# david-jk/BigGAN-Tensorflow

Measured on AMD Instinct MI355X. Metric: BigGAN-128 train-step images/sec, higher is better.
Workload: dtype bf16; 1 GPU; BigGAN-128 ch=96 bf16 (BASELINE config 3: global batch 256, 32/GPU over 8 GPUs); img_size=128, ch=96, per_gpu_batch=256, global_batch=256, da_policy=full, g_regularization=ortho_cosine, n_labels=0, gan_type=hinge, hip_graph=False, precision=bf16, parallelism=dp1

## Files before the change

### biggan-tensorflow_amd/csrc/elementwise.hip

```cpp
#include <stdlib.h>
#include <mutex>
#include "common.h"

namespace bg {

#define EW_BLOCK 256
#define EW_MAX_BLOCKS 2048

static inline int ew_grid(int64_t work_items) {
    int64_t b = (work_items + EW_BLOCK - 1) / EW_BLOCK;
    if (b > EW_MAX_BLOCKS) b = EW_MAX_BLOCKS;
    if (b < 1) b = 1;
    return (int)b;
}

__device__ __forceinline__ float4 ldg4(const float* p) { return *reinterpret_cast<const float4*>(p); }
__device__ __forceinline__ void stg4(float* p, const float4& v) { *reinterpret_cast<float4*>(p) = v; }

template <int NQ, int VEC, class Fn, class OutT>
__global__ __launch_bounds__(EW_BLOCK) void colreduce_kernel(Fn fn, OutT* out, float* part, int64_t qstride,
                                                             int64_t rows_per_seg, int C, int rows_per_block) {
    __shared__ float red[NQ * EW_BLOCK * VEC];
    const int CV = C / VEC;
    const int tx = CV < EW_BLOCK ? CV : EW_BLOCK;
    const int lanes = EW_BLOCK / tx;
    const int cq = threadIdx.x % tx, rl = threadIdx.x / tx;
    const int seg = blockIdx.y;
    const int64_t r0 = (int64_t)blockIdx.x * rows_per_block;
    int64_t r1 = r0 + rows_per_block;
    if (r1 > rows_per_seg) r1 = rows_per_seg;
    for (int cbase = 0; cbase < CV; cbase += tx) {
        const int cv = cbase + cq;
        float acc[NQ][VEC];
#pragma unroll
        for (int q = 0; q < NQ; ++q)
#pragma unroll
            for (int j = 0; j < VEC; ++j) acc[q][j] = 0.f;
        if (cv < CV && rl < lanes) {
            float acc4[4][NQ][VEC];
#pragma unroll
            for (int u = 0; u < 4; ++u)
#pragma unroll
                for (int q = 0; q < NQ; ++q)
#pragma unroll
                    for (int j = 0; j < VEC; ++j) acc4[u][q][j] = 0.f;
            int64_t r = r0 + rl;
            for (; r + 3 * (int64_t)lanes < r1; r += 4 * (int64_t)lanes) {
#pragma unroll
                for (int u = 0; u < 4; ++u) fn(seg, r + u * (int64_t)lanes, cv * VEC, acc4[u]);
            }
            for (; r < r1; r += lanes) fn(seg, r, cv * VEC, acc4[0]);
#pragma unroll
            for (int q = 0; q < NQ; ++q)
#pragma unroll
                for (int j = 0; j < VEC; ++j)
// ... 325 lines not shown
                                                                  const float* __restrict__ r, const float* __restrict__ cr,
                                                                  const float* __restrict__ c0, float* __restrict__ out,
                                                                  int64_t total, int C) {
    for (int64_t i = (int64_t)blockIdx.x * EW_BLOCK + threadIdx.x; i < total; i += (int64_t)gridDim.x * EW_BLOCK) {
        const int c = (int)(i % C);
        float v = cp[c] * p[i] + cq[c] * q[i] + c0[c];
        if (r) v += cr[c] * r[i];
        out[i] = v;
    }
}

__global__ __launch_bounds__(256) void renorm_coeffs_kernel(const double* __restrict__ sums, double count,
                                                            float* ref_mean, float* ref_scale, int scale_is_var,
                                                            float* weight, float eps, float rmin, float rmax, float dmax,
                                                            float decay, float fade, int update, float* __restrict__ r,
                                                            float* __restrict__ d, int C) {
    const float w = weight ? *weight : 1.f;
    __syncthreads();
    for (int c = threadIdx.x; c < C; c += blockDim.x) {
        const double m64 = sums[c] / count;
        double v64 = sums[C + c] / count - m64 * m64;
        if (v64 < 0) v64 = 0;
        const float m = (float)m64, var = (float)v64;
        const float sigma = sqrtf(var + eps);
        const float rm = ref_mean[c], rs = ref_scale[c];
        const float sigma_ref = scale_is_var ? sqrtf(rs + eps) : fmaxf(rs, sqrtf(eps));
        const float sigma_w = w * sigma_ref + (1.f - w) * sigma;
        const float mean_w = w * rm + (1.f - w) * m;
        r[c] = fminf(fmaxf(sigma / sigma_w, rmin), rmax);
        d[c] = fminf(fmaxf((m - mean_w) / sigma_w, -dmax), dmax);
        if (update) {
            ref_mean[c] = rm * decay + m * (1.f - decay);
            ref_scale[c] = rs * decay + (scale_is_var ? var : sigma) * (1.f - decay);
        }
    }
    if (update && weight && threadIdx.x == 0) *weight = w * fade + 1.0f * (1.f - fade);
}

__global__ __launch_bounds__(EW_BLOCK) void renorm_affine_kernel(const float* __restrict__ g, const float* __restrict__ b,
                                                                 const float* __restrict__ r, const float* __restrict__ d,
                                                                 float* __restrict__ oa, float* __restrict__ ob,
                                                                 int64_t total, int C, int dir) {
    for (int64_t i = (int64_t)blockIdx.x * blockDim.x + threadIdx.x; i < total; i += (int64_t)gridDim.x * blockDim.x) {
        const int c = (int)(i % C);
        if (dir == 0) {
            oa[i] = r[c] * g[i];
            ob[i] = b[i] + d[c] * g[i];
        } else {
            oa[i] = r[c] * g[i] + d[c] * b[i];
        }
    }
}

__device__ __forceinline__ float prelu_f(float v, float a) { return v > 0.f ? v : a * v; }
__device__ __forceinline__ float prelu_d(float v, float a) { return v > 0.f ? 1.f : (v < 0.f ? a : 0.5f * a); }

template <int VEC, class TX, class TY>
__global__ __launch_bounds__(EW_BLOCK) void bn_apply_act_fwd_t_kernel(const TX* __restrict__ x,
                                                                       const float* __restrict__ mean,
                                                                       const float* __restrict__ rstd,
                                                                       const float* __restrict__ gamma,
                                                                       const float* __restrict__ beta, int per_sample,
                                                                       const float* __restrict__ alpha,
                                                                       TY* __restrict__ y, int N, int HW, int C) {
    const int CV = C / VEC;
    const int64_t total = (int64_t)N * HW * CV;
    for (int64_t i = (int64_t)blockIdx.x * EW_BLOCK + threadIdx.x; i < total; i += (int64_t)gridDim.x * EW_BLOCK) {
        const int c = (int)(i % CV) * VEC;
        const int n = (int)(i / ((int64_t)HW * CV));
        const float* gp = gamma + (per_sample ? (int64_t)n * C : 0) + c;
        const float* bp = beta + (per_sample ? (int64_t)n * C : 0) + c;
        float xv[VEC], mu[VEC], rs[VEC], ga[VEC], be[VEC], al[VEC], out[VEC];
        loadv<VEC>(x + i * VEC, xv);
        loadv<VEC>(mean + c, mu);
        loadv<VEC>(rstd + c, rs);
        loadv<VEC>(gp, ga);
        loadv<VEC>(bp, be);
        if (alpha) loadv<VEC>(alpha + c, al);
#pragma unroll
        for (int j = 0; j < VEC; ++j) {
            const float inv = rs[j] * ga[j];
            float v = xv[j] * inv + (be[j] - mu[j] * inv);
            out[j] = alpha ? prelu_f(v, al[j]) : v;
        }
        storev<VEC>(y + i * VEC, out);
    }
}

template <class TX, class TY>
struct BnBwdReduceFnT {
    const TX* x;
    const TY* dy;
    const float *mean, *rstd, *gamma, *beta, *alpha;
    int per_sample, HW, C;
    template <int VEC>
    __device__ __forceinline__ void operator()(int n, int64_t r, int c, float (&acc)[3][VEC]) const {
        const int64_t off = ((int64_t)n * HW + r) * C + c;
        float xv[VEC], dv[VEC], mu[VEC], rs[VEC], ga[VEC], be[VEC], al[VEC];
        loadv<VEC>(x + off, xv);
        loadv<VEC>(dy + off, dv);
        loadv<VEC>(mean + c, mu);
        loadv<VEC>(rstd + c, rs);
        loadv<VEC>(gamma + (per_sample ? (int64_t)n * C : 0) + c, ga);
        loadv<VEC>(beta + (per_sample ? (int64_t)n * C : 0) + c, be);
        if (alpha) loadv<VEC>(alpha + c, al);
#pragma unroll
        for (int j = 0; j < VEC; ++j) {
// ... 179 lines not shown
        bf16x8_load(x + (int64_t)r * C + c, xv);
        bf16x8_load(dy + (int64_t)r * C + c, dv);
#pragma unroll
        for (int j = 0; j < 8; ++j) {
            const float xh = (xv[j] - mu[j]) * rs[j];
            const float pre = xh * ga[j] + be[j];
            const float g = alpha ? dv[j] * prelu_d(pre, al[j]) : dv[j];
            out[j] = rs[j] * (g * ga[j] - m1[j] - xh * m2[j]);
        }
        if (add) {
            float av[8];
            bf16x8_load(add + (int64_t)r * C + c, av);
#pragma unroll
            for (int j = 0; j < 8; ++j) out[j] += av[j];
        }
        bf16x8_store(dx + (int64_t)r * C + c, out);
    }
}

template <bool BWD>
__global__ __launch_bounds__(EW_BLOCK) void prelu_bf16x8_kernel(const __bf16* __restrict__ x, const __bf16* __restrict__ dy,
                                                                 const float* __restrict__ alpha, __bf16* out,
                                                                 const __bf16* add, int rows, int CV) {
    const int gtid = blockIdx.x * EW_BLOCK + threadIdx.x;
    const int c = (gtid % CV) * 8, C = CV * 8;
    const int rstep = (gridDim.x * EW_BLOCK) / CV;
    float al[8];
    f32x8_load(alpha + c, al);
    for (int r = gtid / CV; r < rows; r += rstep) {
        float xv[8], dv[8], o[8];
        bf16x8_load(x + (int64_t)r * C + c, xv);
        if (BWD) bf16x8_load(dy + (int64_t)r * C + c, dv);
#pragma unroll
        for (int j = 0; j < 8; ++j) o[j] = BWD ? dv[j] * prelu_d(xv[j], al[j]) : prelu_f(xv[j], al[j]);
        if (BWD && add) {
            float av[8];
            bf16x8_load(add + (int64_t)r * C + c, av);
#pragma unroll
            for (int j = 0; j < 8; ++j) o[j] += av[j];
        }
        bf16x8_store(out + (int64_t)r * C + c, o);
    }
}

__global__ __launch_bounds__(EW_BLOCK) void lincomb_bf16x8_kernel(const __bf16* __restrict__ a, const float* sa_dev, float sa,
                                                                   const __bf16* __restrict__ b, float sb,
                                                                   __bf16* __restrict__ y, int64_t n8) {
    const float s = sa_dev ? *sa_dev : sa;
    for (int64_t i = (int64_t)blockIdx.x * EW_BLOCK + threadIdx.x; i < n8; i += (int64_t)gridDim.x * EW_BLOCK) {
        float av[8], bv[8], o[8];
        bf16x8_load(a + i * 8, av);
        if (b) {
            bf16x8_load(b + i * 8, bv);
#pragma unroll
            for (int j = 0; j < 8; ++j) o[j] = s * av[j] + sb * bv[j];
        } else {
#pragma unroll
            for (int j = 0; j < 8; ++j) o[j] = s * av[j];
        }
        bf16x8_store(y + i * 8, o);
    }
}

static inline int bn_x8_grid(int64_t rows, int CV) {
    int a = CV, b = EW_BLOCK;
    while (b) { const int t = a % b; a = b; b = t; }
    const int unit = CV / a;
    int64_t want = (rows * CV + EW_BLOCK - 1) / EW_BLOCK;
    if (want > 4096) want = 4096;
    if (want < 1) want = 1;
    return (int)((want + unit - 1) / unit * unit);
}

template <int VEC, class TX, class TY>
__global__ __launch_bounds__(EW_BLOCK) void prelu_fwd_t_kernel(const TX* __restrict__ x, const float* __restrict__ alpha,
                                                                TY* __restrict__ y, int64_t total_v, int C) {
    const int CV = C / VEC;
    for (int64_t i = (int64_t)blockIdx.x * EW_BLOCK + threadIdx.x; i < total_v; i += (int64_t)gridDim.x * EW_BLOCK) {
        const int c = (int)(i % CV) * VEC;
        float xv[VEC], al[VEC], out[VEC];
        loadv<VEC>(x + i * VEC, xv);
        loadv<VEC>(alpha + c, al);
#pragma unroll
        for (int j = 0; j < VEC; ++j) out[j] = prelu_f(xv[j], al[j]);
        storev<VEC>(y + i * VEC, out);
    }
}

template <int VEC, class TX, class TY>
__global__ __launch_bounds__(EW_BLOCK) void prelu_bwd_dx_t_kernel(const TX* __restrict__ x, const TY* __restrict__ dy,
                                                                   const float* __restrict__ alpha, TX* dx, const TX* add,
                                                                   int64_t total_v, int C) {
    const int CV = C / VEC;
    for (int64_t i = (int64_t)blockIdx.x * EW_BLOCK + threadIdx.x; i < total_v; i += (int64_t)gridDim.x * EW_BLOCK) {
        const int c = (int)(i % CV) * VEC;
        float xv[VEC], dv[VEC], al[VEC], out[VEC];
        loadv<VEC>(x + i * VEC, xv);
        loadv<VEC>(dy + i * VEC, dv);
        loadv<VEC>(alpha + c, al);
#pragma unroll
        for (int j = 0; j < VEC; ++j) out[j] = dv[j] * prelu_d(xv[j], al[j]);
        if (add) {
            float av[VEC];
            loadv<VEC>(add + i * VEC, av);
#pragma unroll
            for (int j = 0; j < VEC; ++j) out[j] += av[j];
        }
        storev<VEC>(dx + i * VEC, out);
    }
}

// ... 387 lines not shown
}

__global__ __launch_bounds__(EW_BLOCK) void scale_add_kernel(const float* __restrict__ o,
                                                              const float* __restrict__ gamma,
                                                              const float* __restrict__ x, float* __restrict__ y,
                                                              int64_t n) {
    const float g = *gamma;
    const int64_t n4 = n / 4;
    for (int64_t i = (int64_t)blockIdx.x * EW_BLOCK + threadIdx.x; i < n4; i += (int64_t)gridDim.x * EW_BLOCK) {
        float4 ov = ldg4(o + i * 4), xv = ldg4(x + i * 4);
        stg4(y + i * 4, make_float4(g * ov.x + xv.x, g * ov.y + xv.y, g * ov.z + xv.z, g * ov.w + xv.w));
    }
    for (int64_t i = n4 * 4 + (int64_t)blockIdx.x * EW_BLOCK + threadIdx.x; i < n; i += (int64_t)gridDim.x * EW_BLOCK)
        y[i] = g * o[i] + x[i];
}

__global__ __launch_bounds__(EW_BLOCK) void scale_dev_kernel(const float* __restrict__ x, const float* __restrict__ sp,
                                                              float* __restrict__ y, int64_t n) {
    const float s = *sp;
    for (int64_t i = (int64_t)blockIdx.x * EW_BLOCK + threadIdx.x; i < n; i += (int64_t)gridDim.x * EW_BLOCK)
        y[i] = s * x[i];
}

template <class T>
__global__ __launch_bounds__(EW_BLOCK) void lincomb_t_kernel(const T* __restrict__ a, const float* sa_dev, float sa,
                                                              const T* __restrict__ b, float sb, T* __restrict__ y,
                                                              int64_t n4) {
    const float s = sa_dev ? *sa_dev : sa;
    for (int64_t i = (int64_t)blockIdx.x * EW_BLOCK + threadIdx.x; i < n4; i += (int64_t)gridDim.x * EW_BLOCK) {
        float av[4], bv[4], o[4];
        loadv<4>(a + i * 4, av);
        if (b) {
            loadv<4>(b + i * 4, bv);
#pragma unroll
            for (int j = 0; j < 4; ++j) o[j] = s * av[j] + sb * bv[j];
        } else {
#pragma unroll
            for (int j = 0; j < 4; ++j) o[j] = s * av[j];
        }
        storev<4>(y + i * 4, o);
    }
}

template <class T>
__global__ __launch_bounds__(EW_BLOCK) void dot_t_kernel(float* part, const T* __restrict__ a, const T* __restrict__ b, float* out,
                                                          int64_t n) {
    __shared__ float sh[4];
    float s = 0.f;
    const int64_t n4 = n / 4;
    for (int64_t i = (int64_t)blockIdx.x * EW_BLOCK + threadIdx.x; i < n4; i += (int64_t)gridDim.x * EW_BLOCK) {
        float av[4], bv[4];
        loadv<4>(a + i * 4, av);
        loadv<4>(b + i * 4, bv);
        s += av[0] * bv[0] + av[1] * bv[1] + av[2] * bv[2] + av[3] * bv[3];
    }
    for (int64_t i = n4 * 4 + (int64_t)blockIdx.x * EW_BLOCK + threadIdx.x; i < n; i += (int64_t)gridDim.x * EW_BLOCK)
        s += (float)a[i] * (float)b[i];
    s = block_sum_256(s, sh);
    if (threadIdx.x == 0) {
        if (part)
            part[blockIdx.x] = s;
        else
            *out += s;
    }
}

template <class T>
static int launch_dot(const T* a, const T* b, float* out, int64_t n, hipStream_t s) {
    int grid = ew_grid(n / 4 + 1);
    if (grid > 512) grid = 512;
    float* part = nullptr;
    if (!block_partials(grid, 1, s, &part)) return BG_ERR_LAUNCH;
    hipLaunchKernelGGL((dot_t_kernel<T>), dim3(grid), dim3(EW_BLOCK), 0, s, part, a, b, out, n);
    finalize_block_partials(part, out, grid, 1, s);
    BG_LAUNCH_CHECK();
    return BG_OK;
}

__global__ __launch_bounds__(EW_BLOCK) void tanh_fwd_kernel(const float* __restrict__ x, float* __restrict__ y,
                                                             int64_t n) {
    for (int64_t i = (int64_t)blockIdx.x * EW_BLOCK + threadIdx.x; i < n; i += (int64_t)gridDim.x * EW_BLOCK)
        y[i] = tanhf(x[i]);
}

__global__ __launch_bounds__(EW_BLOCK) void tanh_bwd_kernel(const float* __restrict__ y, const float* __restrict__ dy,
                                                             float* __restrict__ dx, int64_t n) {
    for (int64_t i = (int64_t)blockIdx.x * EW_BLOCK + threadIdx.x; i < n; i += (int64_t)gridDim.x * EW_BLOCK)
        dx[i] = dy[i] * (1.f - y[i] * y[i]);
}

template <class TS, class TD>
__global__ __launch_bounds__(EW_BLOCK) void pad_channels_kernel(const TS* __restrict__ src, TD* __restrict__ dst,
                                                                 int64_t total, int Cs, int Cd, int64_t inner, int mode) {
    for (int64_t idx = (int64_t)blockIdx.x * EW_BLOCK + threadIdx.x; idx < total; idx += (int64_t)gridDim.x * EW_BLOCK) {
        const int64_t i = idx % inner, t = idx / inner;
        const int c = (int)(t % Cd);
        const int64_t o = t / Cd;
        const TS* sp = src + o * Cs * inner + i;
        float v = 0.f;
        if (mode == 3) {
            v = (float)sp[(int64_t)c * inner] + (float)sp[(int64_t)(c + Cd) * inner];
        } else if (c < Cs) {
            v = (float)sp[(int64_t)c * inner];
            if (mode == 1) v = (float)(__bf16)v;
        } else if (mode != 0 && c < 2 * Cs) {
            v = (float)sp[(int64_t)(c - Cs) * inner];
            if (mode == 1) v -= (float)(__bf16)v;
        }
        dst[idx] = (TD)v;
    }
}

__global__ __launch_bounds__(EW_BLOCK) void pad_pixels_to8_kernel(const float* __restrict__ src, __bf16* __restrict__ dst,
                                                                  int64_t pixels, int Cs, int mode) {
    for (int64_t i = (int64_t)blockIdx.x * EW_BLOCK + threadIdx.x; i < pixels; i += (int64_t)gridDim.x * EW_BLOCK) {
        float v[8];
#pragma unroll
        for (int c = 0; c < 8; ++c) v[c] = 0.f;
        const float* sp = src + i * Cs;
#pragma unroll
        for (int c = 0; c < 4; ++c)
            if (c < Cs) {
                const float s = sp[c];
                if (mode == 1) {
                    const float hi = (float)(__bf16)s;
                    v[c] = hi;
// ... 1203 lines not shown
        BG_DISPATCH_T(dtype, hipLaunchKernelGGL((maxpool2_bwd_t_kernel<1, T>), dim3(ew_grid(total)), dim3(EW_BLOCK), 0,
                                                as_stream(stream), (const T*)x, (const T*)dy, (T*)dx, N, H, W, C));
    BG_LAUNCH_CHECK();
    return BG_OK;
}

int bg_sum_pool_fwd_t(const void* x, int x_dtype, float* y, int N, int HW, int C, void* stream) {
    BG_REQUIRE(x && y && N > 0 && HW > 0 && C > 0 && BG_DT_OK(x_dtype), "bg_sum_pool_fwd_t: bad argument");
    if (C % 4 == 0)
        BG_DISPATCH_T(x_dtype, hipLaunchKernelGGL((sum_pool_fwd_t_kernel<4, T>), dim3(ew_grid((int64_t)N * C / 4)),
                                                  dim3(EW_BLOCK), 0, as_stream(stream), (const T*)x, y, N, HW, C));
    else
        BG_DISPATCH_T(x_dtype, hipLaunchKernelGGL((sum_pool_fwd_t_kernel<1, T>), dim3(ew_grid((int64_t)N * C)),
                                                  dim3(EW_BLOCK), 0, as_stream(stream), (const T*)x, y, N, HW, C));
    BG_LAUNCH_CHECK();
    return BG_OK;
}

int bg_sum_pool_bwd_t(const float* dy, void* dx, int x_dtype, int N, int HW, int C, void* stream) {
    BG_REQUIRE(dy && dx && N > 0 && HW > 0 && C > 0 && BG_DT_OK(x_dtype), "bg_sum_pool_bwd_t: bad argument");
    if (C % 4 == 0)
        BG_DISPATCH_T(x_dtype, hipLaunchKernelGGL((sum_pool_bwd_t_kernel<4, T>), dim3(ew_grid((int64_t)N * HW * C / 4)),
                                                  dim3(EW_BLOCK), 0, as_stream(stream), dy, (T*)dx, N, HW, C));
    else
        BG_DISPATCH_T(x_dtype, hipLaunchKernelGGL((sum_pool_bwd_t_kernel<1, T>), dim3(ew_grid((int64_t)N * HW * C)),
                                                  dim3(EW_BLOCK), 0, as_stream(stream), dy, (T*)dx, N, HW, C));
    BG_LAUNCH_CHECK();
    return BG_OK;
}

int bg_lincomb_t(const void* a, const float* sa_dev, float sa, const void* b, float sb, void* y, int dtype, int64_t n,
                 void* stream) {
    BG_REQUIRE(a && y && n > 0 && n % 4 == 0 && BG_DT_OK(dtype), "bg_lincomb_t: bad argument (n %% 4 == 0)");
    if (dtype == BG_BF16 && n % 8 == 0 && ((uintptr_t)a & 15) == 0 && ((uintptr_t)y & 15) == 0 &&
        (!b || ((uintptr_t)b & 15) == 0)) {
        hipLaunchKernelGGL(lincomb_bf16x8_kernel, dim3(ew_grid(n / 8)), dim3(EW_BLOCK), 0, as_stream(stream),
                           (const __bf16*)a, sa_dev, sa, (const __bf16*)b, sb, (__bf16*)y, n / 8);
        BG_LAUNCH_CHECK();
        return BG_OK;
    }
    BG_DISPATCH_T(dtype, hipLaunchKernelGGL((lincomb_t_kernel<T>), dim3(ew_grid(n / 4)), dim3(EW_BLOCK), 0, as_stream(stream),
                                            (const T*)a, sa_dev, sa, (const T*)b, sb, (T*)y, n / 4));
    BG_LAUNCH_CHECK();
    return BG_OK;
}

int bg_dot_t(const void* a, const void* b, int dtype, float* out_accum, int64_t n, void* stream) {
    BG_REQUIRE(a && b && out_accum && n > 0 && n % 4 == 0 && BG_DT_OK(dtype), "bg_dot_t: bad argument (n %% 4 == 0)");
    int rc = BG_OK;
    BG_DISPATCH_T(dtype, rc = launch_dot((const T*)a, (const T*)b, out_accum, n, as_stream(stream)));
    return rc;
}

int bg_bn_stats(const float* x, double* sums, int64_t rows, int C, void* stream) {
    return bg_bn_stats_t(x, BG_F32, sums, rows, C, stream);
}

int bg_bn_apply_act_fwd(const float* x, const float* mean, const float* rstd, const float* gamma, const float* beta,
                        int per_sample, const float* alpha, float* y, int N, int HW, int C, void* stream) {
    return bg_bn_apply_act_fwd_t(x, BG_F32, mean, rstd, gamma, beta, per_sample, alpha, y, BG_F32, N, HW, C, stream);
}

int bg_bn_apply_act_bwd_reduce(const float* x, const float* dy, const float* mean, const float* rstd,
                               const float* gamma, const float* beta, int per_sample, const float* alpha, float* part,
                               int N, int HW, int C, void* stream) {
    return bg_bn_apply_act_bwd_reduce_t(x, BG_F32, dy, BG_F32, mean, rstd, gamma, beta, per_sample, alpha, part, N, HW, C,
                                        stream);
}

int bg_bn_apply_act_bwd_dx(const float* x, const float* dy, const float* mean, const float* rstd, const float* gamma,
                           const float* beta, int per_sample, const float* alpha, const float* cm, float* dx, int N,
                           int HW, int C, void* stream) {
    return bg_bn_apply_act_bwd_dx_t(x, BG_F32, dy, BG_F32, mean, rstd, gamma, beta, per_sample, alpha, cm, dx, NULL, N, HW,
                                    C, stream);
}

int bg_prelu_fwd(const float* x, const float* alpha, float* y, int64_t rows, int C, void* stream) {
    return bg_prelu_fwd_t(x, BG_F32, alpha, y, BG_F32, rows, C, stream);
}

int bg_prelu_bwd(const float* x, const float* dy, const float* alpha, float* dx, float* dalpha, int64_t rows, int C,
                 void* stream) {
    return bg_prelu_bwd_t(x, BG_F32, dy, BG_F32, alpha, dx, dalpha, NULL, rows, C, stream);
}

int bg_bias_grad(const float* dy, float* db, int64_t rows, int C, void* stream) {
    return bg_bias_grad_t(dy, BG_F32, db, rows, C, stream);
}

int bg_maxpool2_fwd(const float* x, float* y, int N, int H, int W, int C, void* stream) {
    return bg_maxpool2_fwd_t(x, y, BG_F32, N, H, W, C, stream);
}

int bg_maxpool2_bwd(const float* x, const float* dy, float* dx, int N, int H, int W, int C, void* stream) {
    return bg_maxpool2_bwd_t(x, dy, dx, BG_F32, N, H, W, C, stream);
}

int bg_sum_pool_fwd(const float* x, float* y, int N, int HW, int C, void* stream) {
    return bg_sum_pool_fwd_t(x, BG_F32, y, N, HW, C, stream);
}

int bg_sum_pool_bwd(const float* dy, float* dx, int N, int HW, int C, void* stream) {
    return bg_sum_pool_bwd_t(dy, dx, BG_F32, N, HW, C, stream);
}

int bg_dot(const float* a, const float* b, float* out_accum, int64_t n, void* stream) {
// ... 7 lines not shown
```

### biggan-tensorflow_amd/csrc/igemm.hip

```cpp
#include <stdlib.h>
#include "common.h"
#include "igemm.h"
#include "igemm_dev.h"
#include "igemm_bf16.h"
#include "igemm16.h"


namespace bg {

typedef float floatx16 __attribute__((ext_vector_type(16)));

#define BKT 16

template <int TM, int TN, int LDA, int LDB>
__device__ __forceinline__ void mma_tile(const float* __restrict__ as, const float* __restrict__ bs, int a_rd, int b_rd,
                                         floatx16 (&acc)[TM][TN]) {
    float a[2][TM], b[2][TN];
#pragma unroll
    for (int i = 0; i < TM; ++i) a[0][i] = as[a_rd + 32 * i];
#pragma unroll
    for (int j = 0; j < TN; ++j) b[0][j] = bs[b_rd + 32 * j];
#pragma unroll
    for (int kk = 0; kk < BKT / 2; ++kk) {
        const int cur = kk & 1, nxt = cur ^ 1;
        if (kk + 1 < BKT / 2) {
#pragma unroll
            for (int i = 0; i < TM; ++i) a[nxt][i] = as[a_rd + 2 * (kk + 1) * LDA + 32 * i];
#pragma unroll
            for (int j = 0; j < TN; ++j) b[nxt][j] = bs[b_rd + 2 * (kk + 1) * LDB + 32 * j];
        }
#pragma unroll
        for (int i = 0; i < TM; ++i)
#pragma unroll
            for (int j = 0; j < TN; ++j)
                acc[i][j] = __builtin_amdgcn_mfma_f32_32x32x2f32(a[cur][i], b[cur][j], acc[i][j], 0, 0, 0);
    }
}

template <int TM, int TN, int WM, int WN, bool BT, int MODE, bool MIRROR, bool VEC>
__global__ __launch_bounds__(256, (TM * TN == 4 && !MIRROR) ? 4 : 1) void nn_kernel(const NNParams p) {
    constexpr int BM = 32 * TM * WM, BN = 32 * TN * WN;
    constexpr int LDA = BM + 2;
    constexpr int LDB = BT ? BN + 2 : BN + 4;
    constexpr int AROWS = BM / 64;
    constexpr int NSRC = MIRROR ? 4 : 1;
    static_assert(WM * WN == 4, "4 waves");
    __shared__ __attribute__((aligned(16))) float As[2][BKT * LDA];
    __shared__ __attribute__((aligned(16))) float Bs[2][BKT * LDB];

    const int t = threadIdx.x;
    const int lane = t & 63, wave = t >> 6;
    const int wm = wave / WN, wn = wave % WN;

// ... 1028 lines not shown
    const int batch = d->batch > 0 ? d->batch : 1;
    Gather g{};
    g.Nb = d->transA ? d->K : d->M; g.Hs = 1; g.Ws = 1; g.Ho = 1; g.Wo = 1; g.Hq = 1; g.Wq = 1; g.pstep = 1;
    g.k = 1; g.stride = 1; g.ld = d->lda;
    if (d->transA) {
        pl.route = TN_F32;
        TNParams& p = pl.tn;
        p.g = g;
        p.Ca = d->M; p.Cb = d->N; p.Mf = d->M; p.b_ld = d->ldb; p.M = d->K;
        p.out_ld = d->ldc; p.batch = batch;
        p.strideA = d->strideA; p.strideB = d->strideB; p.strideC = d->strideC;
        return pl;
    }
    pl.route = F32_TAP;
    NNParams& p = pl.nn;
    p.g = g;
    p.C = d->K; p.M = d->M; p.N = d->N;
    if (d->transB) { p.ldk = 1; p.ldn = d->ldb; } else { p.ldk = d->ldb; p.ldn = 1; }
    p.out_ld = d->ldc; p.batch = batch;
    p.strideA = d->strideA; p.strideB = d->strideB; p.strideC = d->strideC;
    pl.bt = d->transB != 0;
    pl.dense = d->ldc == d->N && batch == 1;
    pl.zdim = batch;
    pl.niter_min = kc_of(d->K);
    pl.out_elems = (int64_t)d->M * d->N;
    return pl;
}

static ConvPlan plan_gram16(int rows, int cols, int ld) {
    ConvPlan pl{};
    pl.route = TN_BF16;
    pl.mode = GATHER_PLAIN;
    TN16Params& p = pl.tn16;
    p.g.ld = ld; p.b_ld = ld;
    p.Ca = cols; p.Cb = cols; p.Mf = cols; p.M = rows; p.out_ld = cols;
    return pl;
}

static size_t plan_workspace_bytes(const ConvPlan& pl) {
    if (pl.route == TN_F32) return tn_workspace_bytes(pl.tn.Mf, pl.tn.Cb, pl.tn.batch, pl.tn.M);
    if (pl.route == TN_BF16) return tn16_workspace_bytes(pl.tn16);
    const size_t slabs = route_f32(pl.route) ? nn_workspace_bytes(pl)
                                             : nn16_workspace_bytes(pl.nn16, pl.mode, pl.zdim, pl.out_elems);
    return pl.grid_bytes ? align256(slabs) + pl.grid_bytes : slabs;
}

static size_t plan_stats_bytes(const BgConvDesc* d, const ConvPlan& pl) {
    if (pl.route != BF16_PLAIN || d->y_dtype != BG_BF16) return 0;
    return (size_t)nn16_stats_rows(pl.nn16, pl.mode, pl.zdim) * 2 * (size_t)d->Cout * sizeof(float);
}

static int run_nn(ConvPlan& pl, const BgConvDesc* d, const char* op, bool deconv, const void* src, const void* w,
                  const float* bias, const float* alpha_dev, void* out, int accumulate, void* ws, size_t ws_bytes,
                  void* stream) {
    hipStream_t s = as_stream(stream);
    Tag tag(op, d);
    void* const grid = ws;
    void* target = out;
    int acc = accumulate;
    if (pl.grid_bytes) {
        BG_REQUIRE(ws && ws_bytes >= pl.grid_bytes, "bg_conv2d_dgrad: workspace too small for the padded gradient");
        target = ws; acc = 0;
        ws = ws_bytes > pl.grid_bytes ? reinterpret_cast<char*>(ws) + pl.grid_bytes : nullptr;
        ws_bytes -= pl.grid_bytes;
    }
    ProfScope prof(s, conv_flops(d, deconv), tag.s, tag.bytes);
    int rc;
    if (route_f32(pl.route)) {
        NNParams& p = pl.nn;
        p.A = (const float*)src; p.B = (const float*)w; p.bias = bias; p.alpha = alpha_dev; p.out = (float*)target;
        p.accumulate = acc;
        const bool vec = (p.C % 4 == 0) && (pl.bt || p.N % 4 == 0) && aligned16(src) && aligned16(w);
        rc = launch_nn(pl, vec, ws, ws_bytes, s, d->compute == BG_COMPUTE_BF16);
    } else {
        NN16Params& r = pl.nn16;
        r.A = src; r.B = w; r.bias = bias; r.alpha = alpha_dev; r.out = target; r.accumulate = acc;
        NN16Params q = r;
        if (pl.route == BF16_THIN_D2S || pl.route == BF16_THIN_D2S_RING)
            rc = launch_nn16h_d2s(r, s);
        else
            rc = launch_nn16(r, pl.mode, pl.zdim, pl.out_elems, ws, ws_bytes, s);
        if (!rc && route_ring(pl.route)) {
            q.ring = 1;
            q.ring_lines = d->stride == 1 ? 2 : 1;
            q.accumulate = 1;
            rc = launch_nn16_ring(q, s);
        }
    }
    if (rc || !pl.grid_bytes) return rc;
    return launch_reflect_fold(grid, out, route_f32(pl.route) ? 1 : pl.nn16.out_f32, d->N, d->H, d->W, d->Cin, pl.nn.g.Ho,
                               pl.nn.g.Wo, d->pad_lo, accumulate, s);
}

static int run_tn(ConvPlan& pl, const BgConvDesc* d, const char* op, bool deconv, const void* a, const void* b, float* dw,
                  void* ws, size_t ws_bytes, void* stream) {
    Tag tag(op, d);
    ProfScope prof(as_stream(stream), conv_flops(d, deconv), tag.s, tag.bytes);
    if (pl.route == TN_BF16) {
        pl.tn16.A = a; pl.tn16.Bv = b;
        return launch_tn16(pl.tn16, pl.mode, dw, ws, ws_bytes, as_stream(stream));
    }
    pl.tn.A = (const float*)a; pl.tn.Bv = (const float*)b;
    const bool vec = (d->Cin % 4 == 0) && (d->Cout % 4 == 0) && aligned16(a) && aligned16(b);
    return launch_tn(pl.tn, pl.mode, vec, dw, ws, ws_bytes, as_stream(stream), d->compute == BG_COMPUTE_BF16);
}

}

using namespace bg;

extern "C" {

size_t bg_conv2d_fwd_workspace_bytes(const BgConvDesc* d) { return d ? plan_workspace_bytes(plan_conv_fwd(d)) : 0; }
size_t bg_conv2d_dgrad_workspace_bytes(const BgConvDesc* d) { return d ? plan_workspace_bytes(plan_conv_dgrad(d)) : 0; }
size_t bg_conv2d_wgrad_workspace_bytes(const BgConvDesc* d) { return d ? plan_workspace_bytes(plan_conv_wgrad(d)) : 0; }
size_t bg_deconv2d_fwd_workspace_bytes(const BgConvDesc* d) { return d ? plan_workspace_bytes(plan_deconv_fwd(d)) : 0; }
size_t bg_deconv2d_dgrad_workspace_bytes(const BgConvDesc* d) { return d ? plan_workspace_bytes(plan_deconv_dgrad(d)) : 0; }
size_t bg_deconv2d_wgrad_workspace_bytes(const BgConvDesc* d) { return d ? plan_workspace_bytes(plan_deconv_wgrad(d)) : 0; }
size_t bg_deconv2d_fwd_stats_workspace_bytes(const BgConvDesc* d) { return d ? plan_stats_bytes(d, plan_deconv_fwd(d)) : 0; }
size_t bg_gemm_workspace_bytes(const BgGemmDesc* d) { return d ? plan_workspace_bytes(plan_gemm(d)) : 0; }
size_t bg_gram16_workspace_bytes(int rows, int cols) {
    return rows > 0 && cols > 0 ? plan_workspace_bytes(plan_gram16(rows, cols, cols)) : 0;
}

int bg_conv2d_fwd(const BgConvDesc* d, const void* x, const void* w, const float* bias, const float* alpha_dev,
                  void* y, int accumulate, void* ws, size_t ws_bytes, void* stream) {
    int rc = check_conv(d);
    if (rc) return rc;
    BG_REQUIRE(x && w && y, "bg_conv2d_fwd: null tensor pointer");
    ConvPlan pl = plan_conv_fwd(d);
    if (pl.route == BF16_PLAIN)
        BG_REQUIRE(d->w_packed, "bg_conv2d_fwd: bf16 input needs the packed bf16 weights (w_packed)");
    else
        BG_REQUIRE(d->y_dtype == BG_F32 && !d->w_packed, "bg_conv2d_fwd: fp32 input needs fp32 weights and output");
    return run_nn(pl, d, "conv2d_fwd", false, x, w, bias, alpha_dev, y, accumulate, ws, ws_bytes, stream);
}

int bg_conv2d_fwd_d2s_supported(const BgConvDesc* d, int block) {
    if (!d) return 0;
    const ConvPlan pl = plan_conv_fwd(d, block);
    if (!pl.nn16.d2s_c || check_conv(d) != BG_OK) return 0;
    return nn16_d2s_ok(pl.nn16, pl.mode, pl.zdim) ? 1 : 0;
}

int bg_conv2d_fwd_d2s(const BgConvDesc* d, const void* x, const void* w, const float* bias, const float* alpha_dev,
                      void* y, int block, void* ws, size_t ws_bytes, void* stream) {
    int rc = check_conv(d);
    if (rc) return rc;
    BG_REQUIRE(x && w && y, "bg_conv2d_fwd_d2s: null tensor pointer");
    ConvPlan pl = plan_conv_fwd(d, block);
    BG_REQUIRE(pl.nn16.d2s_c && nn16_d2s_ok(pl.nn16, pl.mode, pl.zdim),
               "bg_conv2d_fwd_d2s: this launch has no fused depth-to-space store (query bg_conv2d_fwd_d2s_supported)");
    (void)ws; (void)ws_bytes;
    return run_nn(pl, d, "conv2d_fwd_d2s", false, x, w, bias, alpha_dev, y, 0, nullptr, 0, stream);
}

int bg_conv2d_dgrad(const BgConvDesc* d, const void* dy, const void* w, const float* alpha_dev, void* dx,
                    int accumulate, void* ws, size_t ws_bytes, void* stream) {
    int rc = check_conv(d);
    if (rc) return rc;
    BG_REQUIRE(dy && w && dx, "bg_conv2d_dgrad: null tensor pointer");
    BG_REQUIRE(d->H % d->stride == 0 && d->W % d->stride == 0, "conv dgrad: H,W must be multiples of stride");
    ConvPlan pl = plan_conv_dgrad(d);
    if (route_f32(pl.route))
        BG_REQUIRE(d->x_dtype == BG_F32 && d->y_dtype == BG_F32 && !d->w_packed, "bg_conv2d_dgrad: unsupported dtype mix");
    return run_nn(pl, d, "conv2d_dgrad", false, dy, w, nullptr, alpha_dev, dx, accumulate, ws, ws_bytes, stream);
}

int bg_conv2d_wgrad(const BgConvDesc* d, const void* x, const void* dy, float* dw, void* ws, size_t ws_bytes,
                    void* stream) {
    int rc = check_conv(d);
    if (rc) return rc;
    BG_REQUIRE(x && dy && dw, "bg_conv2d_wgrad: null tensor pointer");
    ConvPlan pl = plan_conv_wgrad(d);
    if (pl.route == TN_F32)
        BG_REQUIRE(d->x_dtype == BG_F32 && d->y_dtype == BG_F32, "bg_conv2d_wgrad: x and dy must both be fp32 or both bf16");
    return run_tn(pl, d, "conv2d_wgrad", false, x, dy, dw, ws, ws_bytes, stream);
}

int bg_deconv2d_fwd(const BgConvDesc* d, const void* x, const void* w, const float* bias, const float* alpha_dev,
                    void* y, int accumulate, void* ws, size_t ws_bytes, void* stream) {
    int rc = check_deconv(d);
    if (rc) return rc;
    BG_REQUIRE(x && w && y, "bg_deconv2d_fwd: null tensor pointer");
    ConvPlan pl = plan_deconv_fwd(d);
    if (pl.route == BF16_PLAIN)
        BG_REQUIRE(d->w_packed, "bg_deconv2d_fwd: bf16 input needs the packed bf16 weights (w_packed)");
    else
        BG_REQUIRE(d->y_dtype == BG_F32 && !d->w_packed, "bg_deconv2d_fwd: fp32 input needs fp32 weights and output");
    return run_nn(pl, d, "deconv2d_fwd", true, x, w, bias, alpha_dev, y, accumulate, ws, ws_bytes, stream);
// ... 80 lines not shown
```

### biggan-tensorflow_amd/csrc/igemm16.h

```cpp
#pragma once
#include <stdint.h>

#include "igemm.h"

namespace bg {

struct NN16Params {
    const void* A;
    const void* B;
    const float* bias;
    const float* alpha;
    void* out;
    float* slabs;
    float* stats_part;
    Gather g;
    int32_t C;
    int32_t M, N;
    int64_t tap_stride;
    int32_t out_ld;
    int32_t out_f32;
    int32_t accumulate;
    int32_t splitk;
    int64_t slab_stride;
    int32_t tiles_m, tiles_n;
    int32_t zfold;
    int32_t mfast;
    int32_t pow2;
    int32_t wq_shift, hq_shift;
    int32_t posmajor;
    int32_t ring;
    int32_t ring_lines;
    int32_t d2s_c;
};

struct TN16Params {
    const void* A;
    const void* Bv;
    float* out;
    Gather g;
    int32_t Ca, Cb;
    int32_t Mf;
    int32_t b_ld;
    int32_t M;
    int32_t splitk, rows_per_split;
    int64_t slab_stride;
    int32_t out_ld;
    int32_t tiles_m, tiles_n;
    int32_t pow2;
    int32_t wq_shift, hq_shift;
};

size_t nn16_workspace_bytes(const NN16Params& p, int mode, int zdim, int64_t out_elems);
int launch_nn16(NN16Params& p, int mode, int zdim, int64_t out_elems, void* ws, size_t ws_bytes, hipStream_t s);
int64_t nn16_stats_rows(const NN16Params& p, int mode, int zdim);
int launch_nn16_ring(NN16Params& p, hipStream_t s);
bool nn16_d2s_ok(const NN16Params& p, int mode, int zdim);
bool nn16h_d2s_ok(const NN16Params& p);
int launch_nn16h_d2s(const NN16Params& plain, hipStream_t s);
size_t tn16_workspace_bytes(const TN16Params& p);
int launch_tn16(TN16Params& p, int mode, float* final_out, void* ws, size_t ws_bytes, hipStream_t s);
int launch_reflect_fold(const void* dxp, void* dx, int f32, int N, int H, int W, int C, int Hp, int Wp, int pad_lo,
                        int accumulate, hipStream_t s);

}
```

### biggan-tensorflow_amd/csrc/igemm16.hip

```cpp
#include <stdlib.h>

#include "common.h"
#include "igemm.h"
#include "igemm16.h"
#include <type_traits>
#include "igemm_dev.h"

namespace bg {

typedef float f32x4_t __attribute__((ext_vector_type(4)));
typedef float f32x16_t __attribute__((ext_vector_type(16)));
typedef __bf16 bf16x8_t __attribute__((ext_vector_type(8)));
typedef short s16x4v __attribute__((ext_vector_type(4)));
typedef short s16x8v __attribute__((ext_vector_type(8)));
typedef __attribute__((address_space(3))) void lds_void_t;
typedef __attribute__((address_space(1))) const void gbl_void_t;
typedef __attribute__((address_space(3))) s16x4v lds_s16x4v;

__device__ uint4 g_zero_page[1024];

__device__ __forceinline__ void glds16(const void* src, unsigned char* lds_wave_base) {
    __builtin_amdgcn_global_load_lds((gbl_void_t*)src, (lds_void_t*)lds_wave_base, 16, 0, 0);
}

__device__ __forceinline__ void glds16_asm(const void* src, uint32_t lds_byte_addr) {
    unsigned keep;
    const uint32_t dst = __builtin_amdgcn_readfirstlane(lds_byte_addr);
    asm volatile("s_mov_b32 %0, m0\n\ts_mov_b32 m0, %2\n\ts_nop 0\n\tglobal_load_lds_dwordx4 %1, off\n\ts_mov_b32 m0, %0"
                 : "=&s"(keep)
                 : "v"(src), "s"(dst)
                 : "memory");
}

__device__ __forceinline__ uint32_t pack_bf16x2(float a, float b) {
    typedef __bf16 bf16x2_t __attribute__((ext_vector_type(2)));
    bf16x2_t v;
    v[0] = (__bf16)a;
    v[1] = (__bf16)b;
    return __builtin_bit_cast(uint32_t, v);
}
__device__ __forceinline__ float bf16_lo(uint32_t u) { return __builtin_bit_cast(float, u << 16); }
__device__ __forceinline__ float bf16_hi(uint32_t u) { return __builtin_bit_cast(float, u & 0xffff0000u); }

constexpr int NN16_BM = 128;
constexpr int NN16_TAPS = 4;
constexpr int NN16_RING_TAPS = 8;
constexpr int nn16_lds_bytes(int TN, int TAPS = NN16_TAPS) {
    const int stage = (NN16_BM + 32 * TN) * 128;
    const int epi = NN16_BM * (32 * TN + 4) * 4;
    const int tab = 2 * TAPS * NN16_BM * 4;
    return (2 * stage + tab > epi ? 2 * stage + tab : epi) + NN16_BM * 4 + 16;
}
constexpr int nn16_pipe_lds_bytes(int TN, int WM, int TAPS = NN16_TAPS) {
    const int bm = 64 * WM;
    return 3 * (bm + 32 * TN) * 64 + TAPS * bm * (4 + 2) + bm * 4 + 16;
}
constexpr int nn16x_lds_bytes(int TN) {
    return 2 * (256 + 32 * TN) * 128 + 2 * NN16_TAPS * 256 * 4 + 256 * 4 + 16;
}
constexpr int NN16_NOSRC = -(1 << 30);

template <int MODE>
__device__ __forceinline__ int64_t nn16_src_off(const Gather& g, const RowPos& r, int kh, int kw) {
    int h, w;
    if (MODE == GATHER_CONV) {
        h = conv_src(r.ho, kh, g.stride, g.pad, g.reflect, g.Hs);
        w = conv_src(r.wo, kw, g.stride, g.pad, g.reflect, g.Ws);
    } else {
        h = tconv_src_from_num(r.ho + g.pad - kh, g.stride, g.Hs);
        w = tconv_src_from_num(r.wo + g.pad - kw, g.stride, g.Ws);
    }
    const bool ok = r.valid && h >= 0 && w >= 0;
    const int pix = (r.b * g.Hs + h) * g.Ws + w;
    return ok ? (int64_t)pix * g.ld : (int64_t)-1;
}

constexpr int NN16_NOMIRROR = -(1 << 20);
__device__ __forceinline__ int nn16_mirror_pos(int o, int n, bool hi) {
    return o == 1 ? -1 : ((hi && o == n - 2) ? n : NN16_NOMIRROR);
}

template <int MODE, bool PM, bool RING = false>
__device__ __forceinline__ RowPos nn16_row(const NN16Params& p, int m, int ph, int pw) {
    RowPos r;
    if (PM) {
        r.valid = m < p.M;
        const int pos = m / p.g.Nb;
        r.b = m - pos * p.g.Nb;
        if (RING) {
            const int L = p.ring_lines, first = L * p.g.Wo;
            if (pos < first) {
                const int line = pos / p.g.Wo;
                r.ho = line == 0 ? 1 : p.g.Ho - 2;
                r.wo = pos - line * p.g.Wo;
            } else {
// ... 463 lines not shown
#pragma unroll
                for (int j = 0; j < TN; ++j)
                    acc[i][j] = __builtin_amdgcn_mfma_f32_16x16x32_bf16(b[s2][j], a[s2][i], acc[i][j], 0, 0, 0);
        asm volatile("s_waitcnt vmcnt(0) lgkmcnt(0)" ::: "memory");
        __builtin_amdgcn_s_barrier();
    }
    }

    constexpr int PARTS = PIPE ? WM : (PHASED ? 2 : 1), PR = BM / PARTS;
    constexpr int ELD = BN + 4;
    float* est = reinterpret_cast<float*>(smem);
    const bool partial = p.splitk > 1;
    const float alpha = (!partial && p.alpha) ? *p.alpha : 1.0f;
    constexpr int CPR = BN / 8;
    float* slab = partial ? p.slabs + (int64_t)zs * p.slab_stride : nullptr;
#pragma unroll
    for (int part = 0; part < PARTS; ++part) {
    if (part > 0) __syncthreads();
    if constexpr (PHASED) {
        constexpr int WNX = TN == 8 ? 4 : 2;
        const int wmx = w / WNX, wnx = w % WNX;
#pragma unroll
        for (int i = 0; i < XMI; ++i)
#pragma unroll
            for (int hj = 0; hj < 2 * XNJ; ++hj) {
                const int row = wmx * 16 * XMI + 16 * i + (lane & 15);
                const int col = (BN / 2) * (hj / XNJ) + wnx * 16 * XNJ + 16 * (hj % XNJ) + 4 * (lane >> 4);
                f32x4_t v = accx[part][i][hj / XNJ][hj % XNJ];
                v[0] *= alpha; v[1] *= alpha; v[2] *= alpha; v[3] *= alpha;
                *reinterpret_cast<f32x4_t*>(est + row * ELD + col) = v;
            }
    } else if (!PIPE || wm == part) {
#pragma unroll
        for (int i = 0; i < 4; ++i)
#pragma unroll
            for (int j = 0; j < TN; ++j) {
                const int row = (PIPE ? 0 : wm * 64) + 16 * i + (lane & 15);
                const int col = wn * 16 * TN + 16 * j + 4 * (lane >> 4);
                f32x4_t v = acc[i][j];
                v[0] *= alpha; v[1] *= alpha; v[2] *= alpha; v[3] *= alpha;
                *reinterpret_cast<f32x4_t*>(est + row * ELD + col) = v;
            }
    }
    __syncthreads();
#pragma unroll
    for (int q = 0; q < (PR * CPR + NTHR - 1) / NTHR; ++q) {
        const int idx = t + NTHR * q;
        if ((PR * CPR) % NTHR != 0 && idx >= PR * CPR) continue;
        const int erow = idx / CPR, cc = idx - erow * CPR;
        const int row = part * PR + erow;
        const int m = m0 + row, col = n0 + cc * 8;
        if (m >= p.M || col >= p.N) continue;
        int64_t ooff;
        if (use_tabo) {
            const unsigned op = tabo[row];
            if (op == 0xffffffffu) continue;
            ooff = (int64_t)op * p.out_ld + col;
        } else if (p.d2s_c) {
            int b, ho, wo;
            if (p.pow2) {
                wo = m & (g.Wo - 1);
                const int t2 = m >> p.wq_shift;
                ho = t2 & (g.Ho - 1);
                b = t2 >> p.hq_shift;
            } else {
                const int t2 = m / g.Wo;
                wo = m - t2 * g.Wo;
                b = t2 / g.Ho;
                ho = t2 - b * g.Ho;
            }
            const int sub = col / p.d2s_c, c = col - sub * p.d2s_c;
            ooff = (((int64_t)b * (2 * g.Ho) + 2 * ho + (sub >> 1)) * (2 * g.Wo) + 2 * wo + (sub & 1)) * p.d2s_c + c;
        } else {
            ooff = (int64_t)m * p.out_ld + col;
        }
        f32x4_t v0 = *reinterpret_cast<const f32x4_t*>(est + erow * ELD + cc * 8);
        f32x4_t v1 = *reinterpret_cast<const f32x4_t*>(est + erow * ELD + cc * 8 + 4);
        if (partial) {
            *reinterpret_cast<f32x4_t*>(slab + ooff) = v0;
            *reinterpret_cast<f32x4_t*>(slab + ooff + 4) = v1;
            continue;
        }
        if (p.bias) {
            const f32x4_t b0 = *reinterpret_cast<const f32x4_t*>(p.bias + col);
            const f32x4_t b1 = *reinterpret_cast<const f32x4_t*>(p.bias + col + 4);
            v0 += b0;
            v1 += b1;
        }
        if (p.out_f32) {
            float* o = reinterpret_cast<float*>(p.out) + ooff;
            if (p.accumulate) {
                v0 += *reinterpret_cast<const f32x4_t*>(o);
                v1 += *reinterpret_cast<const f32x4_t*>(o + 4);
            }
            *reinterpret_cast<f32x4_t*>(o) = v0;
            *reinterpret_cast<f32x4_t*>(o + 4) = v1;
        } else {
            __bf16* o = reinterpret_cast<__bf16*>(p.out) + ooff;
            if (p.accumulate) {
                const uint4 r = *reinterpret_cast<const uint4*>(o);
                v0[0] += bf16_lo(r.x); v0[1] += bf16_hi(r.x); v0[2] += bf16_lo(r.y); v0[3] += bf16_hi(r.y);
                v1[0] += bf16_lo(r.z); v1[1] += bf16_hi(r.z); v1[2] += bf16_lo(r.w); v1[3] += bf16_hi(r.w);
            }
            uint4 r;
            r.x = pack_bf16x2(v0[0], v0[1]);
            r.y = pack_bf16x2(v0[2], v0[3]);
            r.z = pack_bf16x2(v1[0], v1[1]);
            r.w = pack_bf16x2(v1[2], v1[3]);
            *reinterpret_cast<uint4*>(o) = r;
        }
    }
    }
}

__global__ __launch_bounds__(256) void nn16_slab_reduce_kernel(const float* __restrict__ slabs, void* __restrict__ out,
                                                               const float* __restrict__ bias,
                                                               const float* __restrict__ alpha_dev, int64_t n8, int N,
                                                               int splitk, int64_t slab_stride, int accumulate,
                                                               int out_f32) {
    const float alpha = alpha_dev ? *alpha_dev : 1.0f;
    for (int64_t i = (int64_t)blockIdx.x * 256 + threadIdx.x; i < n8; i += (int64_t)gridDim.x * 256) {
        f32x4_t s0 = {0.f, 0.f, 0.f, 0.f}, s1 = s0;
        for (int z = 0; z < splitk; ++z) {
            const float* sp = slabs + (int64_t)z * slab_stride + i * 8;
            s0 += *reinterpret_cast<const f32x4_t*>(sp);
            s1 += *reinterpret_cast<const f32x4_t*>(sp + 4);
        }
        s0 *= alpha;
        s1 *= alpha;
        if (bias) {
            const int col = (int)((i * 8) % N);
            s0 += *reinterpret_cast<const f32x4_t*>(bias + col);
            s1 += *reinterpret_cast<const f32x4_t*>(bias + col + 4);
        }
        if (out_f32) {
            float* o = reinterpret_cast<float*>(out) + i * 8;
            if (accumulate) {
                s0 += *reinterpret_cast<const f32x4_t*>(o);
                s1 += *reinterpret_cast<const f32x4_t*>(o + 4);
            }
            *reinterpret_cast<f32x4_t*>(o) = s0;
            *reinterpret_cast<f32x4_t*>(o + 4) = s1;
        } else {
            __bf16* o = reinterpret_cast<__bf16*>(out) + i * 8;
            if (accumulate) {
                const uint4 r = *reinterpret_cast<const uint4*>(o);
                s0[0] += bf16_lo(r.x); s0[1] += bf16_hi(r.x); s0[2] += bf16_lo(r.y); s0[3] += bf16_hi(r.y);
                s1[0] += bf16_lo(r.z); s1[1] += bf16_hi(r.z); s1[2] += bf16_lo(r.w); s1[3] += bf16_hi(r.w);
            }
            uint4 r;
            r.x = pack_bf16x2(s0[0], s0[1]);
            r.y = pack_bf16x2(s0[2], s0[3]);
            r.z = pack_bf16x2(s1[0], s1[1]);
            r.w = pack_bf16x2(s1[2], s1[3]);
            *reinterpret_cast<uint4*>(o) = r;
        }
    }
}

constexpr int NH_T = 16;
constexpr int NH_LDS_MAX = 81920;
template <int NT> struct NHGeom {
// ... 33 lines not shown
    for (int half = 0; half < 2; ++half) {
        if ((wm >> 1) == half) {
#pragma unroll
            for (int i = 0; i < 4; ++i)
#pragma unroll
                for (int j = 0; j < NF; ++j) {
                    const int row = ((wm & 1) * 4 + i) * 16 + px;
                    const int col = wn * 16 * NF + 16 * j + 4 * kb;
                    f32x4_t v = acc[i][j];
                    v[0] *= alpha; v[1] *= alpha; v[2] *= alpha; v[3] *= alpha;
                    *reinterpret_cast<f32x4_t*>(est + row * ELD + col) = v;
                }
        }
        __syncthreads();
        for (int idx = t; idx < 128 * CPR; idx += 512) {
            const int row = idx / CPR, cc = idx - row * CPR;
            const int gy = y0 + 8 * half + (row >> 4), gx = x0 + (row & 15);
            const int col = THIN == 1 ? 0 : n0 + cc * 8;
            const int oy = THIN == 1 ? 2 * gy + (cc >> 1) : gy * g.pstep + ph;
            const int ox = THIN == 1 ? 2 * gx + (cc & 1) : gx * g.pstep + pw;
            f32x4_t v0 = *reinterpret_cast<const f32x4_t*>(est + row * ELD + cc * 8);
            f32x4_t v1 = *reinterpret_cast<const f32x4_t*>(est + row * ELD + cc * 8 + 4);
            const bool live = gy < g.Hq && gx < g.Wq && col < p.N && oy < g.Ho && ox < g.Wo;
            if (live) {
                int64_t ooff = ((int64_t)(b * g.Ho + oy) * g.Wo + ox) * p.out_ld + col;
                if (THIN == 0 && p.d2s_c) {
                    const int sub = col / p.d2s_c, c = col - sub * p.d2s_c;
                    ooff = (((int64_t)b * (2 * g.Ho) + 2 * oy + (sub >> 1)) * (2 * g.Wo) + 2 * ox + (sub & 1)) * p.d2s_c + c;
                }
                if (p.bias) {
                    v0 += *reinterpret_cast<const f32x4_t*>(p.bias + col);
                    v1 += *reinterpret_cast<const f32x4_t*>(p.bias + col + 4);
                }
                if (p.out_f32) {
                    float* o = reinterpret_cast<float*>(p.out) + ooff;
                    if (p.accumulate) {
                        v0 += *reinterpret_cast<const f32x4_t*>(o);
                        v1 += *reinterpret_cast<const f32x4_t*>(o + 4);
                    }
                    *reinterpret_cast<f32x4_t*>(o) = v0;
                    *reinterpret_cast<f32x4_t*>(o + 4) = v1;
                } else {
                    __bf16* o = reinterpret_cast<__bf16*>(p.out) + ooff;
                    if (p.accumulate) {
                        const uint4 rr = *reinterpret_cast<const uint4*>(o);
                        v0[0] += bf16_lo(rr.x); v0[1] += bf16_hi(rr.x); v0[2] += bf16_lo(rr.y); v0[3] += bf16_hi(rr.y);
                        v1[0] += bf16_lo(rr.z); v1[1] += bf16_hi(rr.z); v1[2] += bf16_lo(rr.w); v1[3] += bf16_hi(rr.w);
                    }
                    uint4 rr;
                    rr.x = pack_bf16x2(v0[0], v0[1]);
                    rr.y = pack_bf16x2(v0[2], v0[3]);
                    rr.z = pack_bf16x2(v1[0], v1[1]);
                    rr.w = pack_bf16x2(v1[2], v1[3]);
                    *reinterpret_cast<uint4*>(o) = rr;
                    if (p.stats_part) {
                        v0[0] = bf16_lo(rr.x); v0[1] = bf16_hi(rr.x); v0[2] = bf16_lo(rr.y); v0[3] = bf16_hi(rr.y);
                        v1[0] = bf16_lo(rr.z); v1[1] = bf16_hi(rr.z); v1[2] = bf16_lo(rr.w); v1[3] = bf16_hi(rr.w);
                    }
                }
            } else if (p.stats_part) {
                v0 = f32x4_t{0.f, 0.f, 0.f, 0.f};
                v1 = v0;
            }
            if (p.stats_part) {
                *reinterpret_cast<f32x4_t*>(est + row * ELD + cc * 8) = v0;
                *reinterpret_cast<f32x4_t*>(est + row * ELD + cc * 8 + 4) = v1;
            }
        }
        __syncthreads();
        if (p.stats_part) {
            float st_s = 0.f, st_q = 0.f;
            if (t < RG * BN) {
                const int colr = t % BN;
                for (int row = t / BN; row < 128; row += RG) {
                    const float v = est[row * ELD + colr];
                    st_s += v;
                    st_q = fmaf(v, v, st_q);
                }
            }
            __syncthreads();
            if (t < RG * BN) {
                est[t] = st_s;
                est[RG * BN + t] = st_q;
            }
            __syncthreads();
            if (t < BN && n0 + t < p.N) {
                float s = 0.f, q = 0.f;
#pragma unroll
                for (int r2 = 0; r2 < RG; ++r2) {
                    s += est[r2 * BN + t];
                    q += est[RG * BN + r2 * BN + t];
                }
                const int64_t prow = 2 * ((((int64_t)b * tiles_y + ty) * tiles_x + tx) * nph + phase) + half;
                p.stats_part[prow * (2 * (int64_t)p.N) + n0 + t] = s;
                p.stats_part[prow * (2 * (int64_t)p.N) + p.N + n0 + t] = q;
            }
            __syncthreads();
        }
    }
}

template <int NT, int NF, int MODE, int THIN = 0>
__global__ __launch_bounds__(512, 4) void nn16h_kernel(const NN16Params p) {
    using G = NHGeom<NT>;
    constexpr int WW = G::HW, NPIX = G::NPIX, A_ROUNDS = G::A_ROUNDS, A_INSTR = G::A_INSTR, A_BYTES = G::A_BYTES;
    constexpr int BN = 32 * NF, W_ROUNDS = nh_w_rounds(NF), W_INSTR = nh_w_instr(NF), W_BYTES = W_ROUNDS * 1024;
    constexpr int NTAPS = NT * NT;
// ... 1084 lines not shown
    p.N = 32;
    p.splitk = 1; p.mfast = 0; p.ring = 0;
    const int64_t blocks = (int64_t)g.Nb * (g.Hq / NH_T) * (g.Wq / NH_T);
    BG_REQUIRE(blocks > 0 && blocks < (int64_t(1) << 31), "nn16h: grid out of range");
    if (const int rc = launch_nn16h_inst<2, 1, GATHER_CONV, 1>(p, (int)blocks, s)) return rc;
    BG_LAUNCH_CHECK();
    return BG_OK;
}

static int nn16_mfast(const NN16Params& p, int tiles_m, int tiles_n) {
    const char* e = getenv("BG_NN16_MFAST");
    if (!e) return 0;
    if (strcmp(e, "auto") != 0) return atoi(e) != 0;
    const double l2 = 3.0e6;
    const double a_bytes = 2.0 * p.g.Nb * (double)p.g.Hs * p.g.Ws * p.g.ld;
    const double w_bytes = 2.0 * p.g.k * p.g.k * (double)p.N * p.C;
    const double nfast = a_bytes + (w_bytes > l2 ? w_bytes * tiles_m : w_bytes);
    const double mfast = w_bytes + (a_bytes > l2 ? a_bytes * tiles_n : a_bytes);
    return mfast < nfast;
}

static int launch_nn16h(NN16Params& p, int mode, int ntaps, hipStream_t s) {
    int nf = 4, best = 1 << 30;
    for (int c = 4; c >= 1; --c) {
        const int padded = (p.N + 32 * c - 1) / (32 * c) * (32 * c);
        if (padded < best) { best = padded; nf = c; }
    }
    const Gather& g = p.g;
    const int64_t blocks = (int64_t)g.Nb * (g.Hq / NH_T) * (g.Wq / NH_T) * ((p.N + 32 * nf - 1) / (32 * nf)) *
                           (g.pstep * g.pstep);
    BG_REQUIRE(blocks > 0 && blocks < (int64_t(1) << 31), "nn16h: grid out of range");
    p.splitk = 1;
    p.mfast = nn16_mfast(p, g.Nb * (g.Hq / NH_T) * (g.Wq / NH_T), (p.N + 32 * nf - 1) / (32 * nf));
    int rc;
    if (mode == GATHER_CONV) rc = launch_nn16h_nf<3, GATHER_CONV>(p, nf, (int)blocks, s);
    else if (ntaps == 3) rc = launch_nn16h_nf<3, GATHER_TCONV>(p, nf, (int)blocks, s);
    else rc = launch_nn16h_nf<2, GATHER_TCONV>(p, nf, (int)blocks, s);
    if (rc) return rc;
    BG_LAUNCH_CHECK();
    return BG_OK;
}

bool nn16_d2s_ok(const NN16Params& p, int mode, int zdim) {
    const Gather& g = p.g;
    if (p.d2s_c <= 0 || p.d2s_c % 8 || p.N != 4 * p.d2s_c || p.C % 8 || mode != GATHER_CONV || zdim != 1 || g.stride != 1 ||
        g.pstep != 1 || g.Hq != g.Ho || g.Wq != g.Wo || p.stats_part || p.ring)
        return false;
    if ((int64_t)g.Nb * g.Ho * g.Wo * 4 >= (int64_t(1) << 31)) return false;
    if (nn16h_taps(p, mode, zdim)) return true;
    if (nn16_posmajor_fraction(p, mode) < 1.0) return false;
    return plan_nn16(p, mode, zdim, true).splitk == 1;
}

int64_t nn16_stats_rows(const NN16Params& p, int mode, int zdim) {
    if (p.C % 8 || p.N % 8 || !nn16h_taps(p, mode, zdim)) return 0;
    return 2 * (int64_t)p.g.Nb * (p.g.Hq / NH_T) * (p.g.Wq / NH_T) * (p.g.pstep * p.g.pstep);
}

int launch_nn16(NN16Params& p, int mode, int zdim, int64_t out_elems, void* ws, size_t ws_bytes, hipStream_t s) {
    BG_REQUIRE(p.C % 8 == 0 && p.N % 8 == 0 && p.g.ld % 8 == 0 && p.out_ld % 8 == 0,
               "bf16-resident conv: channel counts must be multiples of 8 (C=%d N=%d)", p.C, p.N);
    BG_REQUIRE((reinterpret_cast<uintptr_t>(p.A) & 15) == 0 && (reinterpret_cast<uintptr_t>(p.B) & 15) == 0 &&
                   (reinterpret_cast<uintptr_t>(p.out) & 15) == 0,
               "bf16-resident conv: tensors must be 16-byte aligned");
    BG_REQUIRE(p.g.k >= 1 && p.g.k <= NN16_TAPS && p.C <= 8192 && p.g.stride >= 1 && p.g.stride <= 2,
               "bf16-resident conv: kernel size %d / stride %d / %d channels not supported", p.g.k, p.g.stride, p.C);
    BG_REQUIRE((int64_t)p.g.Nb * p.g.Hs * p.g.Ws < (int64_t(1) << 30) && (int64_t)p.g.Nb * p.g.Ho * p.g.Wo < (int64_t(1) << 31),
               "bf16-resident conv: more than 2^30 source / 2^31 output pixels");
    BG_REQUIRE(p.d2s_c == 0 || (nn16_d2s_ok(p, mode, zdim) && ws == nullptr),
               "bf16-resident conv: this launch has no depth-to-space store (bg_conv2d_fwd_d2s_supported)");
    if (const int ntaps = nn16h_taps(p, mode, zdim)) return launch_nn16h(p, mode, ntaps, s);
    BG_REQUIRE(p.stats_part == nullptr, "bf16-resident conv: fused statistics need the halo-tile form (nn16_stats_rows)");
    NN16Plan pl = plan_nn16(p, mode, zdim, ws != nullptr);
    if (pl.splitk > 1 && ws_bytes < (size_t)pl.splitk * out_elems * sizeof(float)) pl.splitk = 1;
    p.splitk = pl.splitk;
    p.slabs = reinterpret_cast<float*>(ws);
    p.slab_stride = out_elems;
    p.posmajor = nn16_posmajor_fraction(p, mode) < 1.0;
    int xtn;
    const int form = nn16_form(p, pl.tn, (int64_t)((p.M + 255) / 256) * zdim * pl.splitk,
                               zdim == 1 || p.g.k % p.g.stride == 0, false, &xtn);
    const int ltn = form == NN16_FORM_PHASED ? xtn : pl.tn;
    const int bn = 32 * ltn;
    p.tiles_n = (p.N + bn - 1) / bn;
    const int bm = (form == NN16_FORM_WIDE || form == NN16_FORM_PHASED) ? 256 : NN16_BM;
    p.tiles_m = (p.M + bm - 1) / bm;
    p.pow2 = 0;
    if (p.g.Wq > 0 && p.g.Hq > 0 && (p.g.Wq & (p.g.Wq - 1)) == 0 && (p.g.Hq & (p.g.Hq - 1)) == 0) {
        p.pow2 = 1;
        p.wq_shift = __builtin_ctz(p.g.Wq);
        p.hq_shift = __builtin_ctz(p.g.Hq);
    }
    p.mfast = nn16_mfast(p, p.tiles_m, p.tiles_n);
    dim3 grid(p.tiles_m * p.tiles_n, 1, zdim * p.splitk);
    p.zfold = 0;
    if (mode == GATHER_TCONV && zdim > 1 && p.splitk == 1 && p.g.k % p.g.stride == 0) {
        p.zfold = zdim;
        grid = dim3(p.tiles_m * p.tiles_n * zdim, 1, 1);
    }
    int rc;
    if (mode == GATHER_CONV)
        rc = launch_nn16_mode<GATHER_CONV>(p, ltn, form, grid, s);
    else
        rc = launch_nn16_mode<GATHER_TCONV>(p, ltn, form, grid, s);
    if (rc) return rc;
    BG_LAUNCH_CHECK();
    if (pl.splitk > 1) {
        const int64_t n8 = out_elems / 8;
        int blocks = (int)((n8 + 255) / 256);
        if (blocks > 2048) blocks = 2048;
        hipLaunchKernelGGL(nn16_slab_reduce_kernel, dim3(blocks), dim3(256), 0, s, p.slabs, p.out, p.bias, p.alpha, n8,
                           p.N, pl.splitk, out_elems, p.accumulate, p.out_f32);
        BG_LAUNCH_CHECK();
    }
    return BG_OK;
}

static void plan_tn16(TN16Params& p) {
    const int64_t tiles = (int64_t)((p.Mf + 127) / 128) * ((p.Cb + 127) / 128);
    static const int want = getenv("BG_TN16_WANT") ? atoi(getenv("BG_TN16_WANT")) : 1024;
    int sk = (int)(want / tiles);
    const int max_sk = (p.M + 4 * TN16_BK - 1) / (4 * TN16_BK);
    if (sk > max_sk) sk = max_sk;
// ... 187 lines not shown
```

### biggan-tensorflow_amd/functional.py

```python
import math
import os

import torch
from torch.autograd import Function

from . import hip
from .hip import f32, i32, act, dt, stream, check, lib, workspace

BF16 = torch.bfloat16


class Precision:
    compute = hip.COMPUTE_F32
    gemm_bf16 = False
    resident = False
    name = "fp32"


def set_precision(mode):
    if mode in (None, "", "fp32", "f32"):
        Precision.compute, Precision.gemm_bf16, Precision.resident, Precision.name = hip.COMPUTE_F32, False, False, "fp32"
    elif mode == "bf16-staged":
        Precision.compute, Precision.gemm_bf16, Precision.resident, Precision.name = hip.COMPUTE_BF16, True, False, mode
    elif mode == "bf16":
        Precision.compute, Precision.gemm_bf16, Precision.resident, Precision.name = hip.COMPUTE_BF16, True, True, mode
    else:
        raise ValueError("precision %r: expected fp32, bf16-staged or bf16" % (mode,))


class precision_scope:

    def __init__(self, mode):
        self.mode = mode

    def __enter__(self):
        self.prev = Precision.name
        set_precision(self.mode)

    def __exit__(self, *exc):
        set_precision(self.prev)


def cast(x, dtype):
    if x.dtype == dtype:
        return x
    x = _c(x)
    y = torch.empty(x.shape, dtype=dtype, device=x.device)
    check(lib().bg_cast(act(x), dt(x), act(y), dt(y), x.numel(), stream()))
    return y


def image_tiles_u8(x, grid, gh, gw, tile0=0):
# ... 518 lines not shown

def new_run_stamp():
    _run_stamp[0] = object()
    return _run_stamp[0]


def current_run_stamp():
    return _run_stamp[0]



def set_zero_pool(pool):
    global _pool
    _pool = pool


def zeros(n, dtype, device):
    if _pool is not None and _pool.device == device and os.environ.get("BG_ZERO_POOL", "1") != "0":
        return _pool.zeros(n, dtype)
    return torch.zeros(n, dtype=dtype, device=device)


def _bias_grad(dy2d, out):
    check(lib().bg_bias_grad_t(act(dy2d), dt(dy2d), f32(out), dy2d.shape[0], dy2d.shape[1], stream()))


def _resident_ok(x, cin, cout, k=1):
    return x.dtype == BF16 and cin % 8 == 0 and cout % 8 == 0 and k <= 4


def pad_channels(x, C, dtype, axis=-1, mode=hip.PAD_ZERO_FILL):
    x = _c(x)
    axis = axis % x.dim()
    shape = list(x.shape)
    outer = int(math.prod(shape[:axis])) if axis else 1
    inner = int(math.prod(shape[axis + 1:])) if axis + 1 < len(shape) else 1
    Cs = shape[axis]
    shape[axis] = C
    y = torch.empty(shape, dtype=dtype, device=x.device)
    check(lib().bg_pad_channels(act(x), dt(x), act(y), dt(y), outer, Cs, C, inner, mode, stream()))
    return y


def _thin_plan(x, cin, cout):
    if not Precision.resident or x.dtype not in (BF16, torch.float32) or os.environ.get("BG_IMAGE_LAYERS", "") == "fp32":
        return None
    if cin <= 4 and cout % 8 == 0:
        return "in"
    if cout <= 4 and cin % 8 == 0 and x.dtype == BF16:
        return "out"
    return None


class Conv2dFn(Function):

    @staticmethod
    def forward(ctx, x, w, bias, stride, pad_lo, Ho, Wo, pad_mode, out_dtype=None, accumulate_into=None):
        ctx.fork = getattr(x, "bg_fork", None)
        x = _c(x)
        N, H, W_, Cin = x.shape
        k, _, cin2, Cout = w.shape
        assert cin2 == Cin, (x.shape, w.shape)
        L = lib()
        ctx.resident = _resident_ok(x, Cin, Cout, k)
        ctx.in_dtype = x.dtype
        ctx.pad8 = None if ctx.resident or k > 4 else _thin_plan(x, Cin, Cout)
        ctx.acc = accumulate_into is not None
        if ctx.acc:
            assert ctx.pad8 is None and tuple(accumulate_into.shape) == (N, Ho, Wo, Cout), "accumulate_into: shape"
        if ctx.pad8 == "in":
            x8 = pad_channels(x, 8, BF16, mode=hip.PAD_SPLIT)
            ydt = out_dtype or BF16
            d = hip.conv_desc(N, H, W_, 8, Ho, Wo, Cout, k, stride, pad_lo, pad_mode, hip.COMPUTE_BF16, hip.BF16,
                              hip.BF16 if ydt == BF16 else hip.F32, 1)
            y = torch.empty((N, Ho, Wo, Cout), dtype=ydt, device=x.device)
            ws, nb = hip.scratch(L.bg_conv2d_fwd_workspace_bytes, d, x.device)
            pt = weight_packs(pad_channels(w, 8, torch.float32, axis=2, mode=hip.PAD_DUP))[1]
            check(L.bg_conv2d_fwd(d, act(x8), act(pt), f32(bias), None, act(y), 0, f32(ws), nb, stream()))
            ctx.desc, ctx.rgb = d, False
            ctx.x, ctx.w, ctx.bias = x8, w, bias
            return y
        if ctx.pad8 == "out":
            b8 = None if bias is None else pad_channels(bias, 8, torch.float32)
            ydt = out_dtype or torch.float32
            d = hip.conv_desc(N, H, W_, Cin, Ho, Wo, 8, k, stride, pad_lo, pad_mode, hip.COMPUTE_BF16, hip.BF16,
                              hip.F32, 1)
            y8 = torch.empty((N, Ho, Wo, 8), dtype=torch.float32, device=x.device)
            ws, nb = hip.scratch(L.bg_conv2d_fwd_workspace_bytes, d, x.device)
            pt = weight_packs(pad_channels(w, 8, torch.float32, axis=3, mode=hip.PAD_SPLIT))[1]
            check(L.bg_conv2d_fwd(d, act(x), act(pt), f32(b8), None, act(y8), 0, f32(ws), nb, stream()))
            ctx.desc, ctx.rgb = d, False
            ctx.x, ctx.w, ctx.bias = x, w, bias
            return pad_channels(y8, Cout, ydt, mode=hip.PAD_FOLD)
        if x.dtype == BF16 and not ctx.resident:
            x = cast(x, torch.float32)
        if ctx.resident:
            ydt = out_dtype or BF16
            d = hip.conv_desc(N, H, W_, Cin, Ho, Wo, Cout, k, stride, pad_lo, pad_mode, hip.COMPUTE_BF16, hip.BF16,
                              hip.BF16 if ydt == BF16 else hip.F32, 1)
            if ctx.acc:
                y = accumulate_into
                assert y.dtype == ydt and y.is_contiguous(), (y.dtype, ydt)
                ctx.mark_dirty(y)
            else:
                y = torch.empty((N, Ho, Wo, Cout), dtype=ydt, device=x.device)
            ws, nb = hip.scratch(L.bg_conv2d_fwd_workspace_bytes, d, x.device)
            check(L.bg_conv2d_fwd(d, act(x), act(weight_packs(w)[1]), f32(bias), None, act(y), int(ctx.acc), f32(ws), nb,
                                  stream()))
            ctx.desc, ctx.rgb = d, False
            ctx.x, ctx.w, ctx.bias = x, w, bias
            return y
        w = _c(w)
        d = hip.conv_desc(N, H, W_, Cin, Ho, Wo, Cout, k, stride, pad_lo, pad_mode, Precision.compute)
        if ctx.acc:
            y = accumulate_into
            assert y.dtype == torch.float32 and y.is_contiguous()
            ctx.mark_dirty(y)
        else:
            y = torch.empty((N, Ho, Wo, Cout), dtype=torch.float32, device=x.device)
        ctx.rgb = bool(L.bg_rgbconv_supported(d))
        if ctx.rgb:
            check(L.bg_rgbconv_fwd(d, f32(x), f32(w), f32(bias), f32(y), int(ctx.acc), stream()))
        else:
            ws, nb = hip.scratch(L.bg_conv2d_fwd_workspace_bytes, d, x.device)
            check(L.bg_conv2d_fwd(d, f32(x), f32(w), f32(bias), None, f32(y), int(ctx.acc), f32(ws), nb, stream()))
        ctx.desc = d
        ctx.x, ctx.w, ctx.bias = x, w, bias
        return y

    @staticmethod
    def backward(ctx, dy):
        dy = _c(dy)
        d, x, w, bias = ctx.desc, ctx.x, ctx.w, ctx.bias
        L = lib()
        dx = None
        db = None
        if ctx.pad8:
            Cin, Cout = w.shape[2], w.shape[3]
            thin_in = ctx.pad8 == "in"
            if bias is not None:
                db = param_grad(bias, ctx.needs_input_grad[2], lambda out: _bias_grad(dy.view(-1, Cout), out))
            dy8 = cast(dy, BF16) if thin_in else pad_channels(dy, 8, BF16, mode=hip.PAD_SPLIT)
            db16 = hip.conv_desc(d.N, d.H, d.W, d.Cin, d.Ho, d.Wo, d.Cout, d.k, d.stride, d.pad_lo, d.pad_mode,
                                 hip.COMPUTE_BF16, hip.BF16, hip.BF16, 1)
            if ctx.needs_input_grad[0]:
                if thin_in:
                    pp = weight_packs(pad_channels(w, 8, torch.float32, axis=2, mode=hip.PAD_SPLIT))[0]
                    dd = hip.conv_desc(d.N, d.H, d.W, d.Cin, d.Ho, d.Wo, d.Cout, d.k, d.stride, d.pad_lo, d.pad_mode,
                                       hip.COMPUTE_BF16, hip.F32, hip.BF16, 1)
                    dx8 = torch.empty(x.shape, dtype=torch.float32, device=x.device)
                else:
                    pp = weight_packs(pad_channels(w, 8, torch.float32, axis=3, mode=hip.PAD_DUP))[0]
                    dd = db16
                    dx8 = torch.empty_like(x)
                ws, nb = hip.scratch(L.bg_conv2d_dgrad_workspace_bytes, dd, x.device)
                check(L.bg_conv2d_dgrad(dd, act(dy8), act(pp), None, act(dx8), 0, f32(ws), nb, stream()))
                dx = pad_channels(dx8, Cin, ctx.in_dtype, mode=hip.PAD_FOLD) if thin_in else dx8

            def wg8(out):
                nb = L.bg_conv2d_wgrad_workspace_bytes(db16)
                ws = workspace(nb, x.device)
                dw8 = torch.empty((d.k, d.k, d.Cin, d.Cout), dtype=torch.float32, device=x.device)
                check(L.bg_conv2d_wgrad(db16, act(x), act(dy8), f32(dw8), f32(ws), nb, stream()))
                if thin_in:
                    check(L.bg_pad_channels(act(dw8), hip.F32, act(out), hip.F32, d.k * d.k, 8, Cin, d.Cout,
                                            hip.PAD_FOLD, stream()))
                else:
                    check(L.bg_pad_channels(act(dw8), hip.F32, act(out), hip.F32, d.k * d.k * d.Cin, 8, Cout, 1,
                                            hip.PAD_FOLD, stream()))
            dw = param_grad(w, ctx.needs_input_grad[1], wg8)
            ctx.x = ctx.w = ctx.bias = None
            return dx, dw, db, None, None, None, None, None, None, None
        if bias is not None:
            db = param_grad(bias, ctx.needs_input_grad[2], lambda out: _bias_grad(dy.view(-1, d.Cout), out))
        if ctx.resident:
            dyb = cast(dy, BF16)
            db16 = hip.conv_desc(d.N, d.H, d.W, d.Cin, d.Ho, d.Wo, d.Cout, d.k, d.stride, d.pad_lo, d.pad_mode,
                                 hip.COMPUTE_BF16, hip.BF16, hip.BF16, 1)
            if ctx.needs_input_grad[0]:
                dx, add = _fork_target(ctx.fork, x)
                ws, nb = hip.scratch(L.bg_conv2d_dgrad_workspace_bytes, db16, x.device)
                check(L.bg_conv2d_dgrad(db16, act(dyb), act(weight_packs(w)[0]), None, act(dx), int(add), f32(ws), nb,
                                        stream()))
                _fork_done(ctx.fork, dx)

            def wg16(out):
                nb = L.bg_conv2d_wgrad_workspace_bytes(db16)
                ws = workspace(nb, x.device)
                check(L.bg_conv2d_wgrad(db16, act(x), act(dyb), f32(out), f32(ws), nb, stream()))
            dw = param_grad(w, ctx.needs_input_grad[1], wg16)
            ctx.x = ctx.w = ctx.bias = None
            return dx, dw, db, None, None, None, None, None, None, (dy if ctx.acc else None)
        if ctx.needs_input_grad[0]:
            dx = torch.empty_like(x)
            if ctx.rgb:
                check(L.bg_rgbconv_dgrad(d, f32(dy), f32(w), f32(dx), 0, stream()))
            else:
                ws, nb = hip.scratch(L.bg_conv2d_dgrad_workspace_bytes, d, x.device)
                check(L.bg_conv2d_dgrad(d, f32(dy), f32(w), None, f32(dx), 0, f32(ws), nb, stream()))

        def wg(out):
            if ctx.rgb:
                nb = L.bg_rgbconv_wgrad_workspace_bytes(d)
                ws = workspace(nb, x.device)
                check(L.bg_rgbconv_wgrad(d, f32(x), f32(dy), f32(out), f32(ws), nb, stream()))
                return
            nb = L.bg_conv2d_wgrad_workspace_bytes(d)
            ws = workspace(nb, x.device)
            check(L.bg_conv2d_wgrad(d, f32(x), f32(dy), f32(out), f32(ws), nb, stream()))
        dw = param_grad(w, ctx.needs_input_grad[1], wg)
        ctx.x = ctx.w = ctx.bias = None
        if dx is not None:
            dx = cast(dx, ctx.in_dtype)
        return dx, dw, db, None, None, None, None, None, None, (dy if ctx.acc else None)


def _shuffle_ok(t, C):
    return C % (8 if t.dtype == BF16 else 4) == 0


def depth_to_space(x, r=2):
    x = _c(x)
    N, H, W_, C4 = x.shape
    C = C4 // (r * r)
    assert C * r * r == C4, (x.shape, r)
    if not _shuffle_ok(x, C):
        raise NotImplementedError("depth_to_space: %d channels of %s are not a multiple of 16 bytes" % (C, x.dtype))
    y = torch.empty((N, H * r, W_ * r, C), dtype=x.dtype, device=x.device)
    check(lib().bg_depth_to_space(act(x), act(y), dt(x), N, H, W_, C, r, stream()))
    return y


def space_to_depth(y, r=2):
    y = _c(y)
    N, Hr, Wr, C = y.shape
    assert Hr % r == 0 and Wr % r == 0, (y.shape, r)
    if not _shuffle_ok(y, C):
        raise NotImplementedError("space_to_depth: %d channels of %s are not a multiple of 16 bytes" % (C, y.dtype))
    x = torch.empty((N, Hr // r, Wr // r, r * r * C), dtype=y.dtype, device=y.device)
    check(lib().bg_space_to_depth(act(y), act(x), dt(y), N, Hr // r, Wr // r, C, r, stream()))
    return x


def _fuse_d2s():
    return os.environ.get("BG_FUSE_D2S", "1") != "0"


class SubpixelConvFn(Function):

    @staticmethod
    def forward(ctx, x, w, bias, pad_lo, pad_mode, r=2, out_dtype=None):
        N, H, W_, Cin = x.shape
        k, _, cin2, C4 = w.shape
        assert cin2 == Cin and C4 % (r * r) == 0, (x.shape, w.shape, r)
        C = C4 // (r * r)
        ctx.r = r
        L = lib()
        if _fuse_d2s() and r == 2 and out_dtype is None and _resident_ok(x, Cin, C4) and C % 8 == 0:
            d = hip.conv_desc(N, H, W_, Cin, H, W_, C4, k, 1, pad_lo, pad_mode, hip.COMPUTE_BF16, hip.BF16, hip.BF16, 1)
            if L.bg_conv2d_fwd_d2s_supported(d, r):
                ctx.fork = getattr(x, "bg_fork", None)
                x = _c(x)
                ctx.resident, ctx.in_dtype, ctx.pad8, ctx.acc, ctx.rgb = True, x.dtype, None, False, False
                y = torch.empty((N, H * r, W_ * r, C), dtype=BF16, device=x.device)
                check(L.bg_conv2d_fwd_d2s(d, act(x), act(weight_packs(w)[1]), f32(bias), None, act(y), r, None, 0,
                                          stream()))
                ctx.desc = d
# ... 805 lines not shown
        x, mean, rstd = ctx.x, ctx.mean, ctx.rstd
        gamma, beta, alpha = ctx.gamma, ctx.beta, ctx.alpha
        N, H, W_, C = x.shape
        HW = H * W_
        L = lib()
        dev = x.device
        ps = ctx.per_sample
        part = torch.empty((3, N, C), dtype=torch.float32, device=dev)
        check(L.bg_bn_apply_act_bwd_reduce_t(act(x), dt(x), act(dy), dt(dy), f32(mean), f32(rstd), f32(ctx.gamma_c),
                                             f32(ctx.beta_c), ps, f32(alpha), f32(part), N, HW, C, stream()))
        gshape = (N, C) if ps else (C,)
        dgamma = torch.empty(gshape, dtype=torch.float32, device=dev)
        dbeta = torch.empty(gshape, dtype=torch.float32, device=dev)
        dalpha = torch.empty(C, dtype=torch.float32, device=dev) if alpha is not None else None
        cm = torch.empty(2 * C, dtype=torch.float32, device=dev)
        check(L.bg_bn_bwd_finalize(f32(part), f32(ctx.gamma_c), ps, ctx.count, f32(dgamma), f32(dbeta), f32(dalpha),
                                   f32(cm), N, C, stream()))
        if ctx.renorm_rd is not None:
            r_, d_ = ctx.renorm_rd
            dg_eff = dgamma
            dgamma = torch.empty_like(dg_eff)
            check(L.bg_renorm_affine_bwd(f32(dg_eff), f32(dbeta), f32(r_), f32(d_), f32(dgamma), dg_eff.numel() // C, C,
                                         stream()))
        if not ctx.is_training:
            cm.zero_()
        elif ctx.reduce_fn is not None:
            ctx.reduce_fn(cm)
        dx = None
        if ctx.needs_input_grad[0]:
            fork = _fused_fork(ctx.fork, x, dy)
            dx, add = _fork_target(fork, x)
            check(L.bg_bn_apply_act_bwd_dx_t(act(x), dt(x), act(dy), dt(dy), f32(mean), f32(rstd), f32(ctx.gamma_c),
                                             f32(ctx.beta_c), ps, f32(alpha), f32(cm), act(dx), act(dx) if add else None,
                                             N, HW, C, stream()))
            _fork_done(fork, dx)

        def deliver(t, needed, g):
            if not needed:
                return None
            if is_variable(t):
                emit_grad(t, lambda out: out.copy_(g))
                return None
            return g
        dg = deliver(gamma, ctx.needs_input_grad[1], dgamma)
        db = deliver(beta, ctx.needs_input_grad[2], dbeta)
        da = deliver(alpha, ctx.needs_input_grad[3], dalpha) if alpha is not None else None
        ctx.x = None
        return dx, dg, db, da, None, None, None, None, None, None, None, None, None, None


class PReluFn(Function):

    @staticmethod
    def forward(ctx, x, alpha):
        ctx.fork = getattr(x, "bg_fork", None)
        x = _c(x)
        C = x.shape[-1]
        if KinkProbe.sites is not None:
            KinkProbe.sites.append((getattr(alpha, "bg_name", None), "act", x.detach().float().clone()))
        y = torch.empty_like(x)
        check(lib().bg_prelu_fwd_t(act(x), dt(x), f32(alpha), act(y), dt(y), x.numel() // C, C, stream()))
        ctx.x, ctx.alpha = x, alpha
        return y

    @staticmethod
    def backward(ctx, dy):
        dy = _c(dy)
        x, alpha = ctx.x, ctx.alpha
        C = x.shape[-1]
        rows = x.numel() // C
        L = lib()
        dx = None
        if ctx.needs_input_grad[0]:
            fork = _fused_fork(ctx.fork, x, dy)
            dx, add = _fork_target(fork, x)
            check(L.bg_prelu_bwd_t(act(x), dt(x), act(dy), dt(dy), f32(alpha), act(dx), None, act(dx) if add else None,
                                   rows, C, stream()))
            _fork_done(fork, dx)

        def prod(out):
            out.zero_()
            check(L.bg_prelu_bwd_t(act(x), dt(x), act(dy), dt(dy), f32(alpha), None, f32(out), None, rows, C, stream()))
        da = param_grad(alpha, ctx.needs_input_grad[1], prod)
        ctx.x = None
        return dx, da


class MaxPool2Fn(Function):
    @staticmethod
    def forward(ctx, x):
        x = _c(x)
        N, H, W_, C = x.shape
        y = torch.empty((N, H // 2, W_ // 2, C), dtype=x.dtype, device=x.device)
        check(lib().bg_maxpool2_fwd_t(act(x), act(y), dt(x), N, H, W_, C, stream()))
        ctx.x = x
        return y

    @staticmethod
    def backward(ctx, dy):
        dy = _c(dy)
        x = ctx.x
        N, H, W_, C = x.shape
        dx = torch.empty_like(x)
        check(lib().bg_maxpool2_bwd_t(act(x), act(cast(dy, x.dtype)), act(dx), dt(x), N, H, W_, C, stream()))
        ctx.x = None
        return dx


class AvgPool2Fn(Function):

    @staticmethod
    def forward(ctx, x):
        x = _c(x)
        N, H, W_, C = x.shape
        y = torch.empty((N, H // 2, W_ // 2, C), dtype=torch.float32, device=x.device)
        check(lib().bg_box2_down(f32(x), f32(y), N, H, W_, C, 0.25, stream()))
        ctx.shape = (N, H, W_, C)
        return y

    @staticmethod
    def backward(ctx, dy):
        dy = _c(dy)
        N, H, W_, C = ctx.shape
        dx = torch.empty(ctx.shape, dtype=torch.float32, device=dy.device)
        check(lib().bg_box2_up(f32(dy), f32(dx), N, H // 2, W_ // 2, C, 0.25, stream()))
        return dx


class UpSample2Fn(Function):

    @staticmethod
    def forward(ctx, x):
        x = _c(x)
        N, H, W_, C = x.shape
        y = torch.empty((N, 2 * H, 2 * W_, C), dtype=x.dtype, device=x.device)
        if x.dtype == torch.float32:
            check(lib().bg_box2_up(f32(x), f32(y), N, H, W_, C, 1.0, stream()))
        else:
# ... 318 lines not shown
class GradMarkFn(Function):

    @staticmethod
    def forward(ctx, x, callback, tag):
        ctx.cb, ctx.tag = callback, tag
        return x.view_as(x)

    @staticmethod
    def backward(ctx, dy):
        ctx.cb(ctx.tag)
        return dy, None, None


class CastFn(Function):

    @staticmethod
    def forward(ctx, x, dtype):
        ctx.src = x.dtype
        return cast(x, dtype)

    @staticmethod
    def backward(ctx, dy):
        return cast(_c(dy), ctx.src), None


class ForkFn(Function):

    @staticmethod
    def forward(ctx, x, n, state=None):
        ctx.state = state
        return tuple(x.detach().view_as(x) for _ in range(n))

    @staticmethod
    def backward(ctx, *gs):
        if ctx.state is not None:
            ctx.state.buf = None
        uniq = []
        for g in gs:
            if g is not None and not any(g.data_ptr() == u.data_ptr() and g.shape == u.shape for u in uniq):
                uniq.append(_c(g))
        if not uniq:
            return None, None, None
        if len(uniq) == 1:
            return uniq[0], None, None
        out = add(uniq[0], uniq[1])
        for g in uniq[2:]:
            out = add(out, g, out=out)
        return out, None, None


class ScaleAddFn(Function):

    @staticmethod
    def forward(ctx, o, gamma, x):
        ctx.fork = getattr(x, "bg_fork", None)
        o, x = _c(o), _c(x)
        ctx.o_dtype = o.dtype
        if o.dtype != x.dtype:
            o = cast(o, x.dtype)
        y = torch.empty_like(x)
        if x.dtype == torch.float32:
            check(lib().bg_scale_add(f32(o), f32(gamma), f32(x), f32(y), x.numel(), stream()))
        else:
            check(lib().bg_lincomb_t(act(o), f32(gamma), 0.0, act(x), 1.0, act(y), dt(x), x.numel(), stream()))
        ctx.o, ctx.gamma = o, gamma
        return y

    @staticmethod
    def backward(ctx, dy):
        dy = _c(dy)
        o, gamma = ctx.o, ctx.gamma
        L = lib()
        do = None
        if ctx.needs_input_grad[0]:
            do = torch.empty_like(o)
            if dy.dtype == torch.float32:
                check(L.bg_scale_dev(f32(dy), f32(gamma), f32(do), dy.numel(), stream()))
            else:
                check(L.bg_lincomb_t(act(dy), f32(gamma), 0.0, None, 0.0, act(do), dt(dy), dy.numel(), stream()))

        def prod(out):
            out.zero_()
            if dy.numel() % 4:
                check(L.bg_dot(f32(dy), f32(o), f32(out), dy.numel(), stream()))
            else:
                check(L.bg_dot_t(act(dy), act(o), dt(dy), f32(out), dy.numel(), stream()))
        dg = param_grad(gamma, ctx.needs_input_grad[1], prod)
        ctx.o = None
        if do is not None:
            do = cast(do, ctx.o_dtype)
        if ctx.needs_input_grad[2] and dy.dtype == ctx.o_dtype:
            _fork_done(ctx.fork, dy)
        return do, dg, dy


class BnTangentFn(Function):

    @staticmethod
    def forward(ctx, xdot, x, gamma, mean, rstd, count, reduce_fn):
        xdot, x = _c(xdot), _c(x)
        C = x.shape[-1]
        rows = x.numel() // C
        L = lib()
        dev = x.device
        sums = torch.empty(3 * C, dtype=torch.float64, device=dev)
        check(L.bg_chan_dots3(f32(xdot), f32(x), None, hip.ptr(sums), rows, C, stream()))
        if reduce_fn is not None:
            reduce_fn(sums)
        cf = torch.empty(3 * C, dtype=torch.float32, device=dev)
        m12 = torch.empty(2 * C, dtype=torch.float32, device=dev)
        check(L.bg_bn_tangent_fwd_coefs(hip.ptr(sums), float(count), f32(mean), f32(rstd), f32(gamma), f32(cf), f32(m12), C,
                                        stream()))
        y = torch.empty_like(x)
        check(L.bg_chan_lincomb3(f32(xdot), f32(cf[:C]), f32(x), f32(cf[C:2 * C]), None, None, f32(cf[2 * C:]), f32(y),
                                 rows, C, stream()))
        ctx.saved = (xdot, x, gamma, mean, rstd, m12, float(count), reduce_fn)
        return y

    @staticmethod
    def backward(ctx, s_):
        s_ = _c(s_)
        xdot, x, gamma, mean, rstd, m12, count, reduce_fn = ctx.saved
        C = x.shape[-1]
        rows = x.numel() // C
        L = lib()
        dev = x.device
        sums = torch.empty(3 * C, dtype=torch.float64, device=dev)
        check(L.bg_chan_dots3(f32(s_), f32(x), f32(xdot), hip.ptr(sums), rows, C, stream()))
        if reduce_fn is not None:
            reduce_fn(sums)
        cd = torch.empty(3 * C, dtype=torch.float32, device=dev)
        cx = torch.empty(4 * C, dtype=torch.float32, device=dev)
        dg = torch.empty(C, dtype=torch.float32, device=dev)
        check(L.bg_bn_tangent_bwd_coefs(hip.ptr(sums), count, f32(mean), f32(rstd), f32(gamma), f32(m12), f32(cd), f32(cx),
                                        f32(dg), C, stream()))
        dxdot = dx = None
        if ctx.needs_input_grad[0]:
            dxdot = torch.empty_like(x)
            check(L.bg_chan_lincomb3(f32(s_), f32(cd[:C]), f32(x), f32(cd[C:2 * C]), None, None, f32(cd[2 * C:]),
                                     f32(dxdot), rows, C, stream()))
        if ctx.needs_input_grad[1]:
            dx = torch.empty_like(x)
            check(L.bg_chan_lincomb3(f32(s_), f32(cx[:C]), f32(x), f32(cx[C:2 * C]), f32(xdot), f32(cx[2 * C:3 * C]),
                                     f32(cx[3 * C:]), f32(dx), rows, C, stream()))
        dgam = param_grad(gamma, ctx.needs_input_grad[2], lambda out: out.copy_(dg))
        ctx.saved = None
# ... 465 lines not shown
```

### biggan-tensorflow_amd/hip.py

```python
import ctypes
import os
from ctypes import (POINTER, Structure, byref, c_char_p, c_double, c_float, c_int, c_int32, c_int64, c_size_t, c_uint16,
                    c_uint32, c_void_p)

import torch

_LIB = None
LIB_NAME = "libbiggan_hip.so"
ABI_VERSION = 10
LIB_PATH = os.path.join(os.path.dirname(os.path.abspath(__file__)), LIB_NAME)

PAD_REFLECT, PAD_ZERO = 0, 1
PAD_ZERO_FILL, PAD_SPLIT, PAD_DUP, PAD_FOLD = 0, 1, 2, 3
F32, BF16 = 0, 1
COMPUTE_F32, COMPUTE_BF16 = 0, 1
SN_ALL, SN_POWER, SN_NORMALIZE = 0, 1, 2


class BgConvDesc(Structure):
    _fields_ = [(n, c_int32) for n in
                ("N", "H", "W", "Cin", "Ho", "Wo", "Cout", "k", "stride", "pad_lo", "pad_mode",
                 "compute", "x_dtype", "y_dtype", "w_packed")]


class BgGemmDesc(Structure):
    _fields_ = [("M", c_int32), ("N", c_int32), ("K", c_int32), ("transA", c_int32), ("transB", c_int32),
                ("lda", c_int32), ("ldb", c_int32), ("ldc", c_int32), ("batch", c_int32),
                ("strideA", c_int64), ("strideB", c_int64), ("strideC", c_int64),
                ("compute", c_int32), ("reserved", c_int32)]


class BgSnItem(Structure):
    _fields_ = [("w", c_void_p), ("u", c_void_p), ("v", c_void_p), ("sigma", c_void_p), ("w_norm", c_void_p),
                ("g_wnorm", c_void_p), ("dw", c_void_p), ("ws_offset", c_int64), ("rows", c_int32), ("cols", c_int32),
                ("pack_p", c_void_p), ("pack_t", c_void_p), ("taps", c_int32), ("pack_p_ld", c_int32)]


class BgDenseItem(Structure):
    _fields_ = [("x", c_void_p), ("ldx", c_int64), ("w", c_void_p), ("bias", c_void_p), ("y", c_void_p), ("dw", c_void_p),
                ("db", c_void_p), ("K", c_int32), ("N", c_int32), ("acc_w", c_int32), ("acc_b", c_int32)]


DENSE_GROUP_MAX = 8


class BgLatentTarget(Structure):
    _fields_ = [("dst", c_void_p), ("ldd", c_int64), ("width", c_int32), ("accumulate", c_int32)]


class BgLatentSeg(Structure):
    _fields_ = [("src", c_void_p), ("lds", c_int64), ("src_col", c_int32), ("dst_col", c_int32), ("width", c_int32),
                ("target", c_int32)]


LATENT_MAX_TARGETS = 8
LATENT_MAX_SEGS = 48


class BgMixBranch(Structure):
    _fields_ = [("c_off", c_int32), ("cb", c_int32), ("k", c_int32), ("dil", c_int32), ("lo", c_int32),
                ("pad_mode", c_int32), ("transposed", c_int32), ("acc_w", c_int32),
                ("w", c_void_p), ("bias", c_void_p), ("dw", c_void_p)]


MIX_MAX_BRANCHES = 8


class BgAttn16Desc(Structure):
    _fields_ = [(n, c_int32) for n in ("B", "N", "Nk", "d", "dv", "reserved")] + \
               [(n, c_int64) for n in ("ldq", "sq", "ldk", "sk", "ldv", "sv", "ldo", "so",
                                       "ldg", "sg", "lddq", "sdq", "lddk", "sdk", "lddv", "sdv")]


class BgHistItem(Structure):
    _fields_ = [("x", c_void_p), ("n", c_int64)]


class BgPlaceEntry(Structure):
    _fields_ = [("offset", c_int64), ("pitch", c_int32), ("skip", c_int32)]


class BgJpegInfo(Structure):
    _fields_ = [(n, c_int32) for n in ("width", "height", "ncomp", "hs", "vs", "restart")] + \
               [("bw", c_int32 * 3), ("bh", c_int32 * 3), ("blocks", c_int64), ("q", (c_uint16 * 64) * 3)]


_P = c_void_p
_AD = POINTER(BgAttn16Desc)
_CD = POINTER(BgConvDesc)
_GD = POINTER(BgGemmDesc)

SIGNATURES = {
    "bg_abi_version": (c_int, []),
    "bg_last_error": (c_char_p, []),
    "bg_target_arch": (c_char_p, []),
    "bg_png_unfilter": (c_int, [c_char_p, c_int, c_int, c_int, _P]),
    "bg_jpeg_info": (c_int, [c_char_p, c_size_t, _P]),
    "bg_jpeg_coefficients": (c_int, [c_char_p, c_size_t, _P, c_size_t]),
    "bg_conv2d_fwd_workspace_bytes": (c_size_t, [_CD]),
    "bg_conv2d_fwd": (c_int, [_CD, _P, _P, _P, _P, _P, c_int, _P, c_size_t, _P]),
    "bg_conv2d_fwd_d2s_supported": (c_int, [_CD, c_int]),
    "bg_conv2d_fwd_d2s": (c_int, [_CD, _P, _P, _P, _P, _P, c_int, _P, c_size_t, _P]),
    "bg_conv2d_dgrad_workspace_bytes": (c_size_t, [_CD]),
    "bg_conv2d_dgrad": (c_int, [_CD, _P, _P, _P, _P, c_int, _P, c_size_t, _P]),
    "bg_conv2d_wgrad_workspace_bytes": (c_size_t, [_CD]),
    "bg_conv2d_wgrad": (c_int, [_CD, _P, _P, _P, _P, c_size_t, _P]),
    "bg_deconv2d_fwd_workspace_bytes": (c_size_t, [_CD]),
    "bg_deconv2d_fwd": (c_int, [_CD, _P, _P, _P, _P, _P, c_int, _P, c_size_t, _P]),
    "bg_deconv2d_fwd_stats_workspace_bytes": (c_size_t, [_CD]),
    "bg_deconv2d_fwd_stats": (c_int, [_CD, _P, _P, _P, _P, _P, c_int, _P, _P, c_size_t, _P, c_size_t, _P]),
    "bg_deconv2d_dgrad_workspace_bytes": (c_size_t, [_CD]),
    "bg_deconv2d_dgrad": (c_int, [_CD, _P, _P, _P, _P, c_int, _P, c_size_t, _P]),
    "bg_deconv2d_wgrad_workspace_bytes": (c_size_t, [_CD]),
    "bg_deconv2d_wgrad": (c_int, [_CD, _P, _P, _P, _P, c_size_t, _P]),
    "bg_rgbconv_supported": (c_int, [_CD]),
    "bg_rgbconv_fwd": (c_int, [_CD, _P, _P, _P, _P, c_int, _P]),
    "bg_rgbconv_dgrad": (c_int, [_CD, _P, _P, _P, c_int, _P]),
    "bg_rgbconv_wgrad_workspace_bytes": (c_size_t, [_CD]),
    "bg_rgbconv_wgrad": (c_int, [_CD, _P, _P, _P, _P, c_size_t, _P]),
    "bg_dense_group_fwd": (c_int, [POINTER(BgDenseItem), c_int, c_int, _P]),
    "bg_dense_group_wgrad": (c_int, [POINTER(BgDenseItem), c_int, c_int, _P]),
    "bg_dense_group_dgrad": (c_int, [POINTER(BgDenseItem), c_int, c_int, _P, c_int, c_int, _P]),
    "bg_latent_fanout": (c_int, [_P, c_int, _P, c_int, c_int, _P]),
    "bg_latent_fanin": (c_int, [_P, c_int, _P, c_int, c_int, _P]),
    "bg_mixconv_fwd": (c_int, [_CD, _P, c_int, _P, _P, c_int, _P]),
    "bg_mixconv_dgrad": (c_int, [_CD, _P, c_int, _P, c_int, _P, c_int, _P]),
    "bg_mixconv_wgrad_workspace_bytes": (c_size_t, [_CD, _P, c_int]),
    "bg_mixconv_wgrad": (c_int, [_CD, _P, c_int, _P, _P, c_int, _P, c_size_t, _P]),
    "bg_gemm_workspace_bytes": (c_size_t, [_GD]),
    "bg_gemm": (c_int, [_GD, _P, _P, _P, _P, _P, c_int, _P, c_size_t, _P]),
    "bg_attention2_supported": (c_int, [c_int, c_int, c_int, c_int]),
    "bg_attention2_fwd": (c_int, [_P, _P, _P, _P, _P, c_int, c_int, c_int, c_int, c_int, _P]),
    "bg_attention2_bwd": (c_int, [_P, _P, _P, _P, _P, _P, _P, _P, _P, _P, c_int, c_int, c_int, c_int, c_int, _P]),
    "bg_attention16_supported": (c_int, [c_int, c_int, c_int, c_int]),
    "bg_attention16_fwd": (c_int, [_AD, _P, _P, _P, _P, _P, _P]),
    "bg_attention16_bwd": (c_int, [_AD, _P, _P, _P, _P, _P, _P, _P, _P, _P, _P, _P]),
    "bg_spectral_norm_workspace_bytes": (c_size_t, [c_int, c_int]),
    "bg_spectral_norm_fwd": (c_int, [_P, _P, _P, _P, _P, _P, c_int, c_int, _P, c_size_t, _P]),
    "bg_spectral_norm_bwd": (c_int, [_P, _P, _P, _P, _P, _P, c_int, c_int, _P, c_size_t, _P]),
    "bg_spectral_norm_batch_fwd": (c_int, [_P, c_int, _P, c_size_t, _P]),
    "bg_spectral_norm_batch_phase": (c_int, [_P, c_int, _P, c_size_t, c_int, _P]),
    "bg_spectral_norm_batch_bwd": (c_int, [_P, c_int, _P, _P, _P, c_size_t, _P]),
    "bg_bn_stats": (c_int, [_P, _P, c_int64, c_int, _P]),
    "bg_bn_finalize": (c_int, [_P, c_double, c_float, c_float, c_int, _P, _P, _P, _P, c_int, _P]),
    "bg_bn_apply_act_fwd": (c_int, [_P, _P, _P, _P, _P, c_int, _P, _P, c_int, c_int, c_int, _P]),
    "bg_bn_apply_act_bwd_reduce": (c_int, [_P, _P, _P, _P, _P, _P, c_int, _P, _P, c_int, c_int, c_int, _P]),
    "bg_bn_apply_act_bwd_dx": (c_int, [_P, _P, _P, _P, _P, _P, c_int, _P, _P, _P, c_int, c_int, c_int, _P]),
    "bg_bn_bwd_finalize": (c_int, [_P, _P, c_int, c_double, _P, _P, _P, _P, c_int, c_int, _P]),
    "bg_bn_population": (c_int, [_P, _P, c_float, _P, _P, c_int, _P]),
    "bg_renorm_coeffs": (c_int, [_P, c_double, _P, _P, c_int, _P, c_float, c_float, c_float, c_float, c_float, c_float,
                                 c_int, _P, _P, c_int, _P]),
    "bg_renorm_affine_fwd": (c_int, [_P, _P, _P, _P, _P, _P, c_int64, c_int, _P]),
    "bg_renorm_affine_bwd": (c_int, [_P, _P, _P, _P, _P, c_int64, c_int, _P]),
    "bg_symmetrize": (c_int, [_P, _P, c_int, _P]),
    "bg_gp_interpolate": (c_int, [_P, _P, _P, _P, c_double, _P, c_int, c_int64, _P]),
# ... 23 lines not shown
    "bg_alpha_head_bwd": (c_int, [_P, _P, _P, _P, _P, c_int64, _P]),
    "bg_alpha_mask_fwd": (c_int, [_P, _P, c_int64, _P]),
    "bg_alpha_mask_bwd": (c_int, [_P, _P, _P, c_int64, _P]),
    "bg_alpha_mask_tangent": (c_int, [_P, _P, _P, c_int64, _P]),
    "bg_diffaugment_fwd": (c_int, [_P, _P, _P, _P, _P, _P, _P, _P, _P, c_int, c_int, c_int, c_int, _P, _P]),
    "bg_diffaugment_bwd": (c_int, [_P, _P, _P, _P, _P, _P, _P, _P, c_int, c_int, c_int, c_int, _P, _P]),
    "bg_hinge_d_sums": (c_int, [_P, _P, _P, c_int, _P]),
    "bg_hinge_d_grad": (c_int, [_P, _P, _P, c_double, c_float, _P, _P, _P, c_int, _P]),
    "bg_hinge_g_sums": (c_int, [_P, _P, c_int, _P]),
    "bg_hinge_g_grad": (c_int, [_P, c_double, c_float, _P, _P, c_int, _P]),
    "bg_gan_loss_means": (c_int, [_P, _P, _P, c_int, c_int, _P]),
    "bg_gan_loss_terms": (c_int, [c_int, c_int, _P, _P, _P, c_double, c_double, _P, c_int, c_int, _P]),
    "bg_gan_loss_grad": (c_int, [c_int, c_int, _P, _P, _P, _P, c_double, c_double, c_float, _P, _P, _P, c_int, c_int,
                                 _P]),
    "bg_sigmoid_ce": (c_int, [_P, _P, _P, c_float, _P, _P, c_int, c_int, _P]),
    "bg_label_loss_sums": (c_int, [_P, _P, _P, _P, _P, _P, c_int, c_int, c_int, _P]),
    "bg_label_loss_finish": (c_int, [_P, _P, _P, _P, _P, _P, c_double, c_float, _P, _P, c_int, c_int, c_int, _P]),
    "bg_gather_rows": (c_int, [_P, _P, _P, c_int, c_int, c_int, _P]),
    "bg_ortho_cosine_fwd_bwd": (c_int, [_P, c_float, _P, _P, c_int, _P]),
    "bg_ortho_identity_fwd_bwd": (c_int, [_P, c_float, _P, _P, c_int, _P]),
    "bg_gemv_rows": (c_int, [_P, _P, _P, c_int, c_int, _P]),
    "bg_ortho_lowrank_cols": (c_int, [_P, _P, _P, c_float, _P, _P, _P, c_int, c_int, _P]),
    "bg_ortho_lowrank_finish": (c_int, [_P, _P, _P, _P, _P, c_int, c_int, _P]),
    "bg_adam_tf_ema_step": (c_int, [_P, _P, _P, _P, _P, c_float, c_float, c_float, c_float, c_float, c_float,
                                    c_int64, _P]),
    "bg_adam_tf_ema_step_dev": (c_int, [_P, _P, _P, _P, _P, _P, c_float, c_float, c_float, c_float, c_float, c_int64,
                                        _P]),
    "bg_chan_dots3": (c_int, [_P, _P, _P, _P, c_int64, c_int, _P]),
    "bg_bn_tangent_fwd_coefs": (c_int, [_P, c_double, _P, _P, _P, _P, _P, c_int, _P]),
    "bg_bn_tangent_bwd_coefs": (c_int, [_P, c_double, _P, _P, _P, _P, _P, _P, _P, c_int, _P]),
    "bg_chan_lincomb3": (c_int, [_P, _P, _P, _P, _P, _P, _P, _P, c_int64, c_int, _P]),
    "bg_gram16_workspace_bytes": (c_size_t, [c_int, c_int]),
    "bg_gram16": (c_int, [_P, c_int, c_int, c_int, _P, _P, c_size_t, _P]),
    "bg_cast": (c_int, [_P, c_int, _P, c_int, c_int64, _P]),
    "bg_depth_to_space": (c_int, [_P, _P, c_int, c_int, c_int, c_int, c_int, c_int, _P]),
    "bg_space_to_depth": (c_int, [_P, _P, c_int, c_int, c_int, c_int, c_int, c_int, _P]),
    "bg_pad_channels": (c_int, [_P, c_int, _P, c_int, c_int64, c_int, c_int, c_int64, c_int, _P]),
    "bg_weight_pack": (c_int, [_P, c_int, c_int, c_int, _P, _P, _P]),
    "bg_bn_stats_t": (c_int, [_P, c_int, _P, c_int64, c_int, _P]),
    "bg_bn_apply_act_fwd_t": (c_int, [_P, c_int, _P, _P, _P, _P, c_int, _P, _P, c_int, c_int, c_int, c_int, _P]),
    "bg_bn_apply_act_bwd_reduce_t": (c_int, [_P, c_int, _P, c_int, _P, _P, _P, _P, c_int, _P, _P, c_int, c_int, c_int,
                                             _P]),
    "bg_bn_apply_act_bwd_dx_t": (c_int, [_P, c_int, _P, c_int, _P, _P, _P, _P, c_int, _P, _P, _P, _P, c_int, c_int, c_int,
                                         _P]),
    "bg_prelu_fwd_t": (c_int, [_P, c_int, _P, _P, c_int, c_int64, c_int, _P]),
    "bg_prelu_bwd_t": (c_int, [_P, c_int, _P, c_int, _P, _P, _P, _P, c_int64, c_int, _P]),
    "bg_bias_grad_t": (c_int, [_P, c_int, _P, c_int64, c_int, _P]),
    "bg_maxpool2_fwd_t": (c_int, [_P, _P, c_int, c_int, c_int, c_int, c_int, _P]),
    "bg_maxpool2_bwd_t": (c_int, [_P, _P, _P, c_int, c_int, c_int, c_int, c_int, _P]),
    "bg_sum_pool_fwd_t": (c_int, [_P, c_int, _P, c_int, c_int, c_int, _P]),
    "bg_sum_pool_bwd_t": (c_int, [_P, _P, c_int, c_int, c_int, c_int, _P]),
    "bg_lincomb_t": (c_int, [_P, _P, c_float, _P, c_float, _P, c_int, c_int64, _P]),
    "bg_dot_t": (c_int, [_P, _P, c_int, _P, c_int64, _P]),
    "bg_bn_glu_fwd": (c_int, [_P, _P, _P, _P, _P, _P, c_int, c_int64, c_int, _P]),
    "bg_bn_glu_bwd_reduce": (c_int, [_P, _P, _P, _P, _P, _P, _P, c_int, c_int64, c_int, c_int, _P]),
    "bg_bn_glu_bwd_dx": (c_int, [_P, _P, _P, _P, _P, _P, _P, _P, c_int, c_int64, c_int, _P]),
    "bg_glu_fwd": (c_int, [_P, _P, c_int, c_int64, c_int, _P]),
    "bg_glu_bwd": (c_int, [_P, _P, _P, c_int, c_int64, c_int, _P]),
    "bg_upsample2_fwd_t": (c_int, [_P, _P, c_int, c_int, c_int, c_int, c_int, _P]),
    "bg_upsample2_bwd_t": (c_int, [_P, _P, c_int, c_int, c_int, c_int, c_int, _P]),
    "bg_crop_at_fwd": (c_int, [_P, _P, c_int, _P, _P, c_int, c_int, c_int, c_int, c_int, _P]),
    "bg_crop_at_bwd": (c_int, [_P, _P, c_int, _P, _P, c_int, c_int, c_int, c_int, c_int, _P]),
    "bg_recon_loss_sums": (c_int, [_P, _P, _P, _P, _P, c_int, c_int, _P, c_int, c_int, c_int, c_int, c_int, _P]),
    "bg_recon_loss_finalize": (c_int, [_P, c_double, _P, _P]),
    "bg_recon_loss_bwd": (c_int, [_P, _P, _P, _P, c_int, c_int, _P, c_double, _P, _P, c_int, c_int, c_int, c_int, c_int,
                                  _P]),
    "bg_image_tiles_u8": (c_int, [_P, c_int, c_int, c_int, c_int, c_int, _P, c_int, c_int, c_int, _P]),
    "bg_image_place_u8": (c_int, [_P, c_int, c_int, c_int, c_int, c_int, _P, _P, c_int64, _P]),
    "bg_deflate_bound": (c_size_t, [c_int]),
    "bg_png_filter": (c_int, [_P, c_int64, _P, c_int, c_int, c_int, _P, c_int64, _P]),
    "bg_deflate_segments": (c_int, [_P, c_int64, _P, c_int, c_int, _P, c_int64, _P, _P]),
    "bg_deflate_compact": (c_int, [_P, c_int64, _P, _P, c_int, _P, c_int64, _P, _P, c_int, _P]),
    "bg_image_batch_u8": (c_int, [_P, c_int64, _P, c_int, c_int, c_int, _P, _P]),
    "bg_jpeg_batch_workspace_bytes": (c_size_t, [c_int, c_int64]),
    "bg_jpeg_batch_u8": (c_int, [_P, c_int64, _P, c_int, c_int64, c_int, _P, c_int64, _P, c_int, _P, c_size_t, _P]),
    "bg_dataset_store": (c_int, [_P, c_int64, _P, c_int, _P, c_int64, _P]),
    "bg_dataset_batch": (c_int, [_P, c_int64, _P, c_int, _P, c_int, c_int, c_int, _P, _P]),
    "bg_crc32c": (c_uint32, [c_char_p, c_size_t, c_uint32]),
    "bg_var_hist_plan_chunks": (c_int, [_P, c_int, _P]),
    "bg_var_hist_plan_bytes": (c_size_t, [c_int, c_int]),
    "bg_var_hist_plan": (c_int, [_P, c_int, _P, c_size_t]),
    "bg_var_hist_workspace_bytes": (c_size_t, [c_int, c_int]),
    "bg_var_hist": (c_int, [_P, c_int, c_int, _P, c_int, _P, _P, _P, c_size_t, _P]),
    "bg_swd_pyr_down": (c_int, [_P, c_int, _P, c_int, c_int, c_int, _P]),
    "bg_swd_pyr_lap": (c_int, [_P, c_int, _P, _P, c_int, c_int, c_int, _P]),
    "bg_swd_stats_workspace_bytes": (c_size_t, [c_int, c_int]),
    "bg_swd_descriptors": (c_int, [_P, _P, c_int, c_int, c_int, _P, c_int64, c_int64, _P, c_size_t, _P]),
    "bg_swd_stats_finish": (c_int, [_P, c_size_t, c_int, c_int, _P, _P]),
    "bg_swd_project": (c_int, [_P, _P, _P, _P, _P, _P, c_int64, c_int, c_int, _P]),
    "bg_swd_sort_tile": (c_size_t, []),
    "bg_swd_sort_segments": (c_int, [_P, c_int, c_int, _P]),
    "bg_swd_l1_workspace_bytes": (c_size_t, [c_int64, c_int]),
    "bg_swd_l1": (c_int, [_P, _P, c_int64, c_int, _P, _P, c_size_t, _P]),
    "bg_nn_pack": (c_int, [_P, c_int, c_int, c_int, c_int, c_int, c_int, _P, _P]),
    "bg_nn_distances": (c_int, [_P, _P, c_int, c_int64, c_int, _P, _P]),
    "bg_nn_topk_workspace_bytes": (c_size_t, [c_int, c_int64, c_int]),
    "bg_nn_topk": (c_int, [_P, c_int, c_int64, c_int, _P, _P, _P, c_size_t, _P]),
    "bg_msssim_workspace_bytes": (c_size_t, [c_int, c_int, c_int]),
    "bg_msssim_level": (c_int, [_P, _P, c_int, c_int64, c_int, c_int, c_int, c_int, _P, _P, _P, c_size_t, _P]),
    "bg_msssim_finish": (c_int, [_P, c_size_t, c_int, c_int, c_int, _P, c_int64, c_int64, _P]),
    "bg_prof_enable": (None, [c_int]),
    "bg_prof_reset": (None, []),
    "bg_prof_collect": (c_int, [POINTER(c_double), POINTER(c_double), POINTER(c_int64)]),
    "bg_prof_dump": (c_int, [c_char_p]),
}

# ... 88 lines not shown
```

### biggan-tensorflow_amd/ops.py

```python
import os

import torch

from . import functional as Fn
from . import hip
from . import scope as S
from .scope import variable_scope, get_variable
from .utils import round_up

weight_init = S.truncated_normal_initializer(mean=0.0, stddev=0.02)
gan_dtype = torch.float32


class _Run:
    def __init__(self):
        self.sn_cache = {}
        self.sn_prefetched = set()
        self.reg_losses = []
        self.reg_seen = set()
        self.reduce_fn = None
        self.world = 1
        self.rank = 0
        self.reg_owner = None
        self.dense_cache = {}
# ... 85 lines not shown
    c4 = channels * r * r
    with variable_scope(scope) as full_scope:
        N, H, W, Cin = x.shape
        pad = (kernel - 1) / 2.0
        pad_mode, pad_lo, pad_hi = hip.PAD_REFLECT, 0, 0
        if pad > 0:
            pad_type = opt.get("conv", {}).get("padding_type", 'reflect')
            tot = pad * 2
            pad_lo = int(tot // 2)
            pad_hi = int(tot - pad_lo)
            if pad_type == 'zero':
                pad_mode = hip.PAD_ZERO
            elif pad_type != 'reflect':
                raise ValueError("Unsupported padding type: " + str(pad_type))
        if pad_lo + pad_hi != kernel - 1:
            raise NotImplementedError("subpixel_conv: kernel %d does not keep the map size" % kernel)
        sn = opt.get("conv", {}).get("sn", True)
        reg = opt.get("conv", {}).get("regularizer", None) if 'generator' in full_scope else None
        w = get_variable("kernel", shape=[kernel, kernel, Cin, c4], initializer=weight_init, regularizer=reg)
        _regularize(w, reg)
        wk = spectral_norm(w, _shape_only=_is_meta(x)) if sn else w
        bias = get_variable("bias", [c4], initializer=S.constant_initializer(0.0)) if use_bias else None
        if _is_meta(x):
            return _meta((N, H * r, W * r, channels))
        if pad_mode == hip.PAD_REFLECT and max(pad_lo, pad_hi) > min(H, W) - 1:
            raise ValueError("tf.pad REFLECT: padding %d does not fit a %dx%d map" % (max(pad_lo, pad_hi), H, W))
        return _resident_out(Fn.SubpixelConvFn.apply(x, wk, bias, pad_lo, pad_mode, r))


def decode_kernel_sizes(str):
    entries = [tuple(int(v) for v in item.split('x')) for item in str.split(',')]
    slices = [{"size": width, "kernel": k} for width, k in entries]
    return {"slices": slices, "total_channels": sum(width for width, _ in entries)}


def encode_kernel_sizes(slices, ch_mul=1.0):
    return ",".join("%dx%d" % (int(float(sl["size"]) * ch_mul + 1e-8), sl["kernel"]) for sl in slices)


def _to(x, dtype):
    if _is_meta(x) or x.dtype == dtype:
        return x
    return Fn.CastFn.apply(x, dtype)


def _resident_out(y):
    if _is_meta(y):
        return y
    if Fn.Precision.resident and y.dtype == torch.float32 and y.dim() == 4 and y.shape[-1] % 8 == 0:
        return Fn.CastFn.apply(y, torch.bfloat16)
    return y


def conv(x, channels, opt, kernel=4, stride=2, pad=0, dilation=1, use_bias=True, scope='conv_0', _out_dtype=None,
         _accumulate_into=None):
    with variable_scope(scope) as full_scope:
        if isinstance(kernel, str):
            slices = decode_kernel_sizes(kernel)["slices"]
            branches = [_MixBranch('conv' + str(sl["kernel"]) + "_slice", False, sl["size"], sl["kernel"],
                                   (sl["kernel"] - 1) // 2, dilation) for sl in slices]
            y = _mixconv(x, branches, opt, stride, use_bias)
            return _mix_epilogue(y, _out_dtype, _accumulate_into)
        if dilation != 1:
            y = _mixconv(x, [_MixBranch(None, False, channels, kernel, pad, dilation)], opt, stride, use_bias)
            return _mix_epilogue(y, _out_dtype, _accumulate_into)
        N, H, W, Cin = x.shape
        pad_mode = hip.PAD_REFLECT
        pad_lo = pad_hi = 0
        if pad > 0:
            pad_type = opt.get("conv", {}).get("padding_type", 'reflect')
            if H % stride == 0:
                tot = pad * 2
            else:
                tot = max(kernel - (H % stride), 0)
            pad_lo = int(tot // 2)
            pad_hi = int(tot - pad_lo)
            if pad_type == 'zero':
                pad_mode = hip.PAD_ZERO
                out = -(-H // stride)
                tot = max((out - 1) * stride + kernel - H, 0)
                pad_lo, pad_hi = tot // 2, tot - tot // 2
            elif pad_type == 'reflect':
                pad_mode = hip.PAD_REFLECT
            else:
                raise ValueError("Unsupported padding type: " + str(pad_type))
        Ho = (H + pad_lo + pad_hi - kernel) // stride + 1
        Wo = (W + pad_lo + pad_hi - kernel) // stride + 1

        sn = opt.get("conv", {}).get("sn", True)
        reg = opt.get("conv", {}).get("regularizer", None) if 'generator' in full_scope else None
        w = get_variable("kernel", shape=[kernel, kernel, Cin, channels], initializer=weight_init, regularizer=reg)
        _regularize(w, reg)
        bias = None
        if sn:
            wk = spectral_norm(w, _shape_only=_is_meta(x))
            if use_bias:
                bias = get_variable("bias", [channels], initializer=S.constant_initializer(0.0))
        else:
            wk = w
            if use_bias:
                bias = get_variable("bias", [channels], initializer=S.constant_initializer(0.0))
        if _is_meta(x):
            return _meta((N, Ho, Wo, channels))
        if _is_dual(x):
            y = Dual(Fn.Conv2dFn.apply(x.p, wk, bias, stride, pad_lo, Ho, Wo, pad_mode),
                     Fn.Conv2dFn.apply(x.t, wk, None, stride, pad_lo, Ho, Wo, pad_mode))
            return y if _accumulate_into is None else _add(y, _accumulate_into)
        acc = _accumulate_into
        if acc is not None and os.environ.get("BG_FUSE_RESIDUAL", "1") == "0":
            y = Fn.Conv2dFn.apply(x, wk, bias, stride, pad_lo, Ho, Wo, pad_mode, _out_dtype)
            return _add(y if _out_dtype is not None else _resident_out(y), acc)
        if acc is not None:
            want = (_out_dtype or (torch.bfloat16 if Fn._resident_ok(x, Cin, channels, kernel) else torch.float32))
            if (acc.dtype != want or not acc.is_contiguous() or Fn._thin_plan(x, Cin, channels) is not None
                    or (x.dtype == torch.bfloat16 and not Fn._resident_ok(x, Cin, channels, kernel))):
                y = Fn.Conv2dFn.apply(x, wk, bias, stride, pad_lo, Ho, Wo, pad_mode, _out_dtype)
                return _add(y if _out_dtype is not None else _resident_out(y), acc)
        y = Fn.Conv2dFn.apply(x, wk, bias, stride, pad_lo, Ho, Wo, pad_mode, _out_dtype, acc)
        return y if _out_dtype is not None else _resident_out(y)


def deconv(x, channels, opt, kernel=4, stride=2, padding='SAME', use_bias=True, scope='deconv_0', _accumulate_into=None,
           _stats=False):
    with variable_scope(scope):
        N, H, W, Cin = x.shape
        if padding != 'SAME':
            raise NotImplementedError("deconv padding != 'SAME'")
        tot = max((H - 1) * stride + kernel - stride * H, 0)
        pad_lo = tot // 2
        reg = opt.get("conv", {}).get("regularizer", None)
        w = get_variable("kernel", shape=[kernel, kernel, channels, Cin], initializer=weight_init, regularizer=reg)
        _regularize(w, reg)
        wk = spectral_norm(w, _shape_only=_is_meta(x)) if opt.get("conv", {}).get("sn", True) else w
        bias = None
        if use_bias:
            bias = get_variable("bias", [channels], initializer=S.constant_initializer(0.0))
        if _is_meta(x):
            return _meta((N, H * stride, W * stride, channels))
        if _accumulate_into is not None and _accumulate_into.dtype != x.dtype and x.dtype == torch.bfloat16:
            _accumulate_into = _to(_accumulate_into, x.dtype)
        box = [None] if (_stats and opt.get("is_training", True) and x.dtype == torch.bfloat16
                         and os.environ.get("BG_FUSE_BNSTATS", "1") != "0") else None
        y = _resident_out(Fn.Deconv2dFn.apply(x, wk, bias, stride, pad_lo, _accumulate_into, box))
        if box is not None and box[0] is not None:
            y.bg_bn_sums = box[0]
        return y


def get_variable_with_custom_lr(name, shape, regularizer, lrmul):
    if lrmul != 1.0:
        raise NotImplementedError("lrmul != 1.0")
    return get_variable(name, shape, initializer=S.truncated_normal_initializer(mean=0.0, stddev=0.02 / lrmul),
                        regularizer=regularizer)


def fully_connected(x, units, opt, use_bias=True, lrmul=1.0, scope='fully_0'):
    with variable_scope(scope) as full_scope:
        x = flatten(x)
        channels = x.shape[-1]
        reg = opt.get("fc_regularizer") if 'generator' in full_scope else None
        w = get_variable_with_custom_lr("kernel", shape=[channels, units], regularizer=reg, lrmul=lrmul)
        _regularize(w, reg)
        bias = get_variable("bias", [units], initializer=S.constant_initializer(0.0)) if use_bias else None
        wk = spectral_norm(w, _shape_only=_is_meta(x)) if opt.get("conv", {}).get("sn", True) else w
        if _is_meta(x):
            return _meta((x.shape[0], units))
        if _is_dual(x):
            return Dual(Fn.DenseFn.apply(x.p, wk, bias), Fn.DenseFn.apply(x.t, wk, None))
        hit = _run.dense_cache.pop(w.bg_name, None)
        if hit is not None and hit[0].data_ptr() == x.data_ptr() and hit[0].shape == x.shape and hit[0].stride() == x.stride():
            return hit[1]
        return Fn.DenseFn.apply(x, wk, bias)


def flatten(x):
    if _is_dual(x):
        return Dual(flatten(x.p), flatten(x.t))
    if x.dim() == 2:
        return x
    if x.dim() == 4 and x.shape[1] == 1 and x.shape[2] == 1:
        return x[:, 0, 0, :]
    return x.reshape(x.shape[0], -1)


def hw_flatten(x):
    return x.reshape(x.shape[0], -1, x.shape[-1])


def _add(a, b):
    if _is_meta(a):
        return _meta(a.shape)
    if _is_dual(a):
        return Dual(Fn.AddFn.apply(a.p, b.p), Fn.AddFn.apply(a.t, b.t))
    return Fn.AddFn.apply(a, b)


def _fork(x, n=2):
    if _is_dual(x):
        return tuple(Dual(a, b) for a, b in zip(_fork(x.p, n), _fork(x.t, n)))
    if _is_meta(x) or not (torch.is_grad_enabled() and x.requires_grad):
        return (x,) * n
    state = Fn.ForkState()
    outs = Fn.ForkFn.apply(x, n, state)
    sums = getattr(x, "bg_bn_sums", None)
    for t in outs:
        t.bg_fork = state
        if sums is not None:
            t.bg_bn_sums = sums
    return outs


def resblock(x_init, channels, opt, use_bias=True, scope='resblock'):
    with variable_scope(scope):
        x_main, x_skip = _fork(x_init)
        with variable_scope('res1'):
            x = conv(x_main, channels, kernel=3, stride=1, pad=1, use_bias=use_bias, opt=opt)
            if opt["bn_in_d"]:
                x = bn(x, opt=opt)
            x = opt["act"](x)
        with variable_scope('res2'):
            x = conv(x, channels, kernel=3, stride=1, pad=1, use_bias=use_bias, opt=opt)
            if opt["bn_in_d"]:
                x = bn(x, opt=opt)
        return _add(x, x_skip)


def upconv(x, channels, opt, use_bias=True, _accumulate_into=None, _stats=False):
    m = opt["upsampling_method"]
    if m == 'deconv3':
        return deconv(x, channels, kernel=3, stride=2, use_bias=use_bias, opt=opt, _accumulate_into=_accumulate_into,
                      _stats=_stats)
    elif m == 'deconv4':
        return deconv(x, channels, kernel=4, stride=2, use_bias=use_bias, opt=opt, _accumulate_into=_accumulate_into,
                      _stats=_stats)
    elif m == 'deconv6':
        return deconv(x, channels, kernel=6, stride=2, use_bias=use_bias, opt=opt, _accumulate_into=_accumulate_into,
                      _stats=_stats)
    elif m == 'resize_conv':
        x = up_sample(x, 2)
        y = conv(x, channels, kernel=3, stride=1, pad=1, use_bias=use_bias, opt=opt)
        return y if _accumulate_into is None else _add(y, _accumulate_into)
    elif m == 'nn':
        y = up_sample(x, 2)
        return y if _accumulate_into is None else _add(y, _accumulate_into)
    elif m == 'subpixel2':
        y = subpixel_conv(x, channels, kernel=2, scale=2, use_bias=use_bias, opt=opt)
        return y if _accumulate_into is None else _add(y, _accumulate_into)
    elif m == 'subpixel3':
        y = subpixel_conv(x, channels, kernel=3, scale=2, use_bias=use_bias, opt=opt)
        return y if _accumulate_into is None else _add(y, _accumulate_into)
    else:
        raise ValueError("Invalid upsampling method specified: " + str(m))


def g_conv(x, channels, opt, use_bias=True, _accumulate_into=None, _stats=False):
    m = opt["g_conv"]
    if m == 'deconv3':
        return deconv(x, channels, kernel=3, stride=1, use_bias=use_bias, opt=opt, _accumulate_into=_accumulate_into,
                      _stats=_stats)
    elif m == 'deconv4':
        return deconv(x, channels, kernel=4, stride=1, use_bias=use_bias, opt=opt, _accumulate_into=_accumulate_into,
                      _stats=_stats)
    elif m == 'conv3':
        y = conv(x, channels, kernel=3, stride=1, pad=1, use_bias=use_bias, opt=opt)
        return y if _accumulate_into is None else _add(y, _accumulate_into)
    elif m == 'conv5':
        y = conv(x, channels, kernel=5, stride=1, pad=2, use_bias=use_bias, opt=opt)
        return y if _accumulate_into is None else _add(y, _accumulate_into)
    else:
        raise ValueError("Invalid generator convolution type specified: " + str(m))


# ... 16 lines not shown
    args, names = [], []
    for sub in subscopes:
        for which in ('beta', 'gamma'):
            name = "%s/%s/%s/%s" % (base, sub, bscope, which)
            w, b = store.vars.get(name + "/kernel"), store.vars.get(name + "/bias")
            if w is None or w.shape[0] != x.shape[1]:
                return
            wk = w
            if sn:
                cached = _run.sn_cache.get(w.bg_name)
                if cached is None or cached[1] != (torch.is_grad_enabled() and w.requires_grad):
                    return
                wk = cached[0]
            args += [x, wk, b]
            names.append(w.bg_name)
    if not names or len(names) > hip.DENSE_GROUP_MAX:
        return
    ys = Fn.GroupedDenseFn.apply(len(names), *args)
    for nm, y in zip(names, ys):
        _run.dense_cache[nm] = (x, y)


def resblock_up(x_init, channels, opt, use_bias=True, scope='resblock_up'):
    with variable_scope(scope):
        x_main, x_skip = _fork(x_init)
        with variable_scope('res1'):
            x = _bn_act(x_main, None, opt)
            x = upconv(x, channels, use_bias=use_bias, opt=opt)
        with variable_scope('res2'):
            x = _bn_act(x, None, opt)
        with variable_scope('skip'):
            skip = upconv(x_skip, channels, use_bias=use_bias, opt=opt)
        with variable_scope('res2'):
            x = g_conv(x, channels, use_bias=use_bias, opt=opt, _accumulate_into=skip)
    return x


def resblock_up_condition(x_init, z, channels, opt, use_bias=True, scope='resblock_up'):
    with variable_scope(scope):
        _cbn_prefetch(z, ('res1', 'res2'), opt)
        x_main, x_skip = _fork(x_init)
        with variable_scope('res1'):
            x = _bn_act(x_main, z, opt)
            x = upconv(x, channels, use_bias=use_bias, opt=opt, _stats=True)
        with variable_scope('res2'):
            x = _bn_act(x, z, opt)
        with variable_scope('skip'):
            skip = upconv(x_skip, channels, use_bias=use_bias, opt=opt)
        with variable_scope('res2'):
            x = g_conv(x, channels, use_bias=use_bias, opt=opt, _accumulate_into=skip, _stats=True)
    return x


def downconv(x, channels, opt, use_bias=True, method=None):
    if method is None:
        method = opt["downsampling_method"]
    if method == 'strided_conv3':
        return conv(x, channels, kernel=3, stride=2, pad=1, use_bias=use_bias, opt=opt)
    elif method == 'resize_conv1':
        x = conv(x, channels, kernel=1, stride=1, pad=0, use_bias=use_bias, opt=opt)
        return avg_pooling(x)
    elif method == 'resize_conv3':
        x = conv(x, channels, kernel=3, stride=1, pad=1, use_bias=use_bias, opt=opt)
        return avg_pooling(x)
    elif method == 'pool_only':
        return avg_pooling(x)
    elif method == 'max_pool_only':
        return max_pooling(x)
    elif method == 'resize_conv35':
        channels5 = int(channels * 0.333333333334)
        channels3 = channels - channels5
        x = _conv35(x, channels3, channels5, use_bias, opt)
        return avg_pooling(x)
    else:
        raise ValueError("Invalid downsampling method specified: " + str(method))


def _conv35(x, channels3, channels5, use_bias, opt):
    kernel = "%dx3,%dx5" % (channels3, channels5)
    if _is_meta(x) or _is_dual(x) or not (Fn.Precision.resident and x.shape[-1] % 8):
        return conv(x, channels3 + channels5, kernel=kernel, stride=1, pad=1, use_bias=use_bias, opt=opt)
    x3, x5 = _fork(_to(x, torch.float32))
    with variable_scope('conv_0'), Fn.precision_scope("bf16-staged"):
        y3 = conv(x3, channels3, kernel=3, stride=1, pad=1, use_bias=use_bias, opt=opt, scope='conv3_slice')
        y5 = conv(x5, channels5, kernel=5, stride=1, pad=2, use_bias=use_bias, opt=opt, scope='conv5_slice')
    return _channel_concat(y3, y5)


def resblock_down(x_init, channels, opt, use_bias=True, scope='resblock_down'):
    with variable_scope(scope):
        x_main, x_init = _fork(x_init)
        with variable_scope('res1'):
            if opt["bn_in_d"]:
                x = bn(x_main, opt=opt)
            else:
                x = x_main
            x = opt["act"](x)
            res_method = opt["downsampling_method"]
            if res_method != 'strided_conv3':
                res_method = 'resize_conv3'
            x = downconv(x, channels, use_bias=use_bias, opt=opt, method=res_method)
        with variable_scope('res2'):
            if opt["bn_in_d"]:
                x = bn(x, opt=opt)
            x = opt["act"](x)
        with variable_scope('skip'):
            x_init = downconv(x_init, channels, use_bias=use_bias, opt=opt, method=opt["downsampling_method"])
        with variable_scope('res2'):
            x = conv(x, channels, kernel=3, stride=1, pad=1, use_bias=use_bias, opt=opt,
                     _accumulate_into=None if _is_meta(x) else x_init)
    return x


def _channel_slice(x, lo, hi):
    if _is_meta(x):
        return _meta(tuple(x.shape[:-1]) + (hi - lo,))
    return x[..., lo:hi]


def _channel_concat(a, b):
    if _is_meta(a):
        return _meta(tuple(a.shape[:-1]) + (a.shape[-1] + b.shape[-1],))
    return torch.cat([a, b], dim=-1)


def resblock_up_cond_deep(x_init, z, channels_out, opt, upscale=True, use_bias=True, scope='deep_resblock'):
    channels_in = int(x_init.shape[-1])
    inner_channels = round_up((channels_in + channels_out) // 6, 8)
    with variable_scope(scope):
        x_main, x_skip = _fork(x_init)
        with variable_scope('bottleneck'):
            x = _bn_act(x_main, z, opt)
            x = conv(x, inner_channels, kernel=1, stride=1, use_bias=False, opt=opt)
        with variable_scope('upscale'):
            x = _bn_act(x, z, opt)
            if upscale:
                x = upconv(x, inner_channels, use_bias=False, opt=opt)
        with variable_scope('inner1'):
            x = g_conv(x, inner_channels, use_bias=False, opt=opt)
            x = _bn_act(x, z, opt)
        with variable_scope('inner2'):
            x = g_conv(x, inner_channels, use_bias=False, opt=opt)
            x = _bn_act(x, None, opt)
        with variable_scope('proj'):
            x = conv(x, channels_out, kernel=1, stride=1, use_bias=use_bias, opt=opt)
        with variable_scope('skip'):
            if upscale:
                kept = _channel_slice(x_skip, 0, channels_out) if channels_in != channels_out else x_skip
                x_skip = upconv(kept, channels_out, use_bias=use_bias, opt=opt)
    return _add(x, x_skip)


def resblock_down_deep(x_init, channels_out, opt, downscale=True, use_bias=True, scope='deep_resblock'):
    channels_in = int(x_init.shape[-1])
    inner_channels = round_up((channels_in + channels_out) // 6, 8)
    with variable_scope(scope):
        x_main, x_skip = _fork(x_init)
        with variable_scope('bottleneck'):
# ... 114 lines not shown
    conv5_ch = split_ch
    no_deconv2 = opt.get("mixed_conv_no_deconv2", False)
    if no_deconv2:
        deconv4_ch += half_split_ch
        conv5_ch += other_half_split_ch
    with variable_scope(scope):
        branches = [_MixBranch("deconv4", True, deconv4_ch, 4), _MixBranch("deconv3", True, split_ch * 2, 3)]
        if not no_deconv2:
            branches.append(_MixBranch("deconv2", True, split_ch, 2))
        branches += [_MixBranch("conv3", False, split_ch, 3, pad=1), _MixBranch("conv5", False, conv5_ch, 5, pad=2),
                     _MixBranch("dilconv5", False, split_ch, 5, pad=4, dilation=2)]
        concat = _mixconv(x, branches, opt, 1, use_bias)
        return _bn_act(concat, z, dict(opt, act=prelu))


def mixed_resblock(x, inner_channels, out_channels, opt, use_bias=False, z=None, scope='res_mixed'):
    with variable_scope(scope):
        x_main, x_skip = _fork(x)
        res = clown_conv(x_main, inner_channels, scope="clown", opt=opt, z=z)
        if _is_meta(x) or torch.is_grad_enabled():
            res = conv(res, channels=out_channels, kernel=1, stride=1, pad=0, use_bias=False, opt=opt, scope='proj')
            return _add(res, x_skip)
        return conv(res, channels=out_channels, kernel=1, stride=1, pad=0, use_bias=False, opt=opt, scope='proj',
                    _accumulate_into=x_skip)


def self_attention(x, channels, opt, scope='self_attention'):
    raise NotImplementedError("self_attention (ops.py:445) is never called by the reference; use self_attention_2")


def _conv1x1_vars(name, cin, cout, opt, use_bias):
    with variable_scope(name) as full_scope:
        reg = opt.get("conv", {}).get("regularizer", None) if 'generator' in full_scope else None
        w = get_variable("kernel", shape=[1, 1, cin, cout], initializer=weight_init, regularizer=reg)
        _regularize(w, reg)
        wk = spectral_norm(w) if opt.get("conv", {}).get("sn", True) else w
        bias = get_variable("bias", [cout], initializer=S.constant_initializer(0.0)) if use_bias else None
    return wk, bias


def self_attention_2(x, channels, opt, scope='self_attention'):
    with variable_scope(scope):
        use_bias = opt.get("self_attention_bias", False)
        if (Fn.Precision.resident and not _is_meta(x) and not _is_dual(x) and x.dtype == torch.bfloat16
                and channels % 8 == 0 and (channels // 2) % 8 == 0):
            C = x.shape[-1]
            wf, b_f = _conv1x1_vars('f_conv', C, channels // 8, opt, use_bias)
            wg, b_g = _conv1x1_vars('g_conv', C, channels // 8, opt, use_bias)
            wh, b_h = _conv1x1_vars('h_conv', C, channels // 2, opt, use_bias)
            if Fn.SaFrontFn.supported(x, wf, wg, wh):
                x_qkv, x_res = _fork(x, 2)
                gamma = get_variable("gamma", [1], initializer=S.constant_initializer(0.0))
                o = Fn.SaFrontFn.apply(x_qkv, wf, wg, wh, b_f, b_g, b_h)
                o = conv(o, channels, kernel=1, stride=1, opt=opt, scope='attn_conv', use_bias=use_bias)
                return Fn.ScaleAddFn.apply(o, gamma, x_res)
        x_f, x_g, x_h, x = _fork(x, 4)
        f32o = None if _is_meta(x) or _is_dual(x) or x.dtype == torch.float32 else torch.float32
        f = conv(x_f, channels // 8, kernel=1, stride=1, opt=opt, scope='f_conv', use_bias=use_bias, _out_dtype=f32o)
        f = max_pooling(f)
        g = conv(x_g, channels // 8, kernel=1, stride=1, opt=opt, scope='g_conv', use_bias=use_bias, _out_dtype=f32o)
        h = conv(x_h, channels // 2, kernel=1, stride=1, opt=opt, scope='h_conv', use_bias=use_bias, _out_dtype=f32o)
        h = max_pooling(h)
        gamma = get_variable("gamma", [1], initializer=S.constant_initializer(0.0))
        if _is_meta(x):
            o = _meta((x.shape[0], x.shape[1], x.shape[2], channels // 2))
        elif _is_dual(x):
            o = _attention_dual(hw_flatten(g), hw_flatten(f), hw_flatten(h))
            o = o.reshape(x.shape[0], x.shape[1], x.shape[2], channels // 2)
        else:
            o = Fn.AttentionFn.apply(hw_flatten(_to(g, torch.float32)), hw_flatten(_to(f, torch.float32)),
                                     hw_flatten(_to(h, torch.float32)))
            o = o.reshape(x.shape[0], x.shape[1], x.shape[2], channels // 2)
            if x.dtype == torch.bfloat16 and (channels // 2) % 8 == 0 and channels % 8 == 0:
                o = _to(o, torch.bfloat16)
        o = conv(o, channels, kernel=1, stride=1, opt=opt, scope='attn_conv', use_bias=use_bias)
        if _is_meta(x):
            return _meta(x.shape)
        if _is_dual(x):
            return Dual(Fn.ScaleAddFn.apply(o.p, gamma, x.p), Fn.ScaleAddFn.apply(o.t, gamma, x.t))
        return Fn.ScaleAddFn.apply(o, gamma, x)


def _attention_dual(q, k, v):
    q1, q2 = _fork(q.p)
    k1, k2 = _fork(k.p)
    v1, v2 = _fork(v.p)
    p = Fn.SoftmaxFn.apply(Fn.BmmFn.apply(q1, k1, True))
    p1, p2, p3 = _fork(p, 3)
    o = Fn.BmmFn.apply(p1, v1, False)
    sdot = Fn.AddFn.apply(Fn.BmmFn.apply(q.t, k2, True), Fn.BmmFn.apply(q2, k.t, True))
    pdot = Fn.SoftmaxTangentFn.apply(p2, sdot)
    odot = Fn.AddFn.apply(Fn.BmmFn.apply(pdot, v2, False), Fn.BmmFn.apply(p3, v.t, False))
    return Dual(o, odot)


def global_avg_pooling(x):
    if _is_meta(x):
        return _meta((x.shape[0], x.shape[-1]))
    inv = 1.0 / float(x.shape[1] * x.shape[2])
    if _is_dual(x):
        return Dual(Fn.ScaleFn.apply(Fn.SumPoolFn.apply(x.p), inv), Fn.ScaleFn.apply(Fn.SumPoolFn.apply(x.t), inv))
    return Fn.ScaleFn.apply(Fn.SumPoolFn.apply(x), inv)


def global_sum_pooling(x):
    if _is_meta(x):
        return _meta((x.shape[0], x.shape[-1]))
    if _is_dual(x):
# ... 328 lines not shown
```

### include/biggan_hip.h

```cpp
#ifndef BIGGAN_HIP_H
#define BIGGAN_HIP_H

#include <stddef.h>
#include <stdint.h>

#ifdef __cplusplus
extern "C" {
#endif

#define BG_ABI_VERSION 10

enum { BG_OK = 0, BG_ERR_ARG = 1, BG_ERR_LAUNCH = 2, BG_ERR_UNSUPPORTED = 3 };
enum { BG_PAD_REFLECT = 0, BG_PAD_ZERO = 1 };
enum { BG_F32 = 0, BG_BF16 = 1 };
enum { BG_COMPUTE_F32 = 0, BG_COMPUTE_BF16 = 1 };

int         bg_abi_version(void);
const char* bg_last_error(void);
const char* bg_target_arch(void);

int bg_png_unfilter(const unsigned char* raw, int h, int stride, int bpp, unsigned char* out);

typedef struct BgJpegInfo {
    int32_t  width, height, ncomp, hs, vs, restart;
    int32_t  bw[3], bh[3];
    int64_t  blocks;
    uint16_t q[3][64];
} BgJpegInfo;
int bg_jpeg_info(const unsigned char* data, size_t n, BgJpegInfo* info);
int bg_jpeg_coefficients(const unsigned char* data, size_t n, int16_t* coef, size_t coef_count);

uint32_t bg_crc32c(const void* data, size_t n, uint32_t crc);

typedef struct BgConvDesc {
    int32_t N, H, W, Cin;
    int32_t Ho, Wo, Cout;
    int32_t k, stride;
    int32_t pad_lo;
    int32_t pad_mode;
    int32_t compute;
    int32_t x_dtype;
    int32_t y_dtype;
    int32_t w_packed;
} BgConvDesc;



size_t bg_conv2d_fwd_workspace_bytes(const BgConvDesc*);
int bg_conv2d_fwd  (const BgConvDesc*, const void* x, const void* w, const float* bias,
                    const float* alpha_dev, void* y, int accumulate,
                    void* ws, size_t ws_bytes, void* stream);
int bg_conv2d_fwd_d2s_supported(const BgConvDesc*, int block);
int bg_conv2d_fwd_d2s(const BgConvDesc*, const void* x, const void* w, const float* bias, const float* alpha_dev,
                      void* y, int block, void* ws, size_t ws_bytes, void* stream);
size_t bg_conv2d_dgrad_workspace_bytes(const BgConvDesc*);
int bg_conv2d_dgrad(const BgConvDesc*, const void* dy, const void* w, const float* alpha_dev,
                    void* dx, int accumulate, void* ws, size_t ws_bytes, void* stream);
size_t bg_conv2d_wgrad_workspace_bytes(const BgConvDesc*);
int bg_conv2d_wgrad(const BgConvDesc*, const void* x, const void* dy, float* dw,
                    void* ws, size_t ws_bytes, void* stream);

size_t bg_deconv2d_fwd_workspace_bytes(const BgConvDesc*);
int bg_deconv2d_fwd  (const BgConvDesc*, const void* x, const void* w, const float* bias,
                      const float* alpha_dev, void* y, int accumulate,
                      void* ws, size_t ws_bytes, void* stream);
size_t bg_deconv2d_fwd_stats_workspace_bytes(const BgConvDesc*);
int bg_deconv2d_fwd_stats(const BgConvDesc*, const void* x, const void* w, const float* bias, const float* alpha_dev,
                          void* y, int accumulate, double* sums, void* stats_ws, size_t stats_ws_bytes, void* ws,
                          size_t ws_bytes, void* stream);
size_t bg_deconv2d_dgrad_workspace_bytes(const BgConvDesc*);
int bg_deconv2d_dgrad(const BgConvDesc*, const void* dy, const void* w, const float* alpha_dev,
                      void* dx, int accumulate, void* ws, size_t ws_bytes, void* stream);
size_t bg_deconv2d_wgrad_workspace_bytes(const BgConvDesc*);
int bg_deconv2d_wgrad(const BgConvDesc*, const void* x, const void* dy, float* dw,
                      void* ws, size_t ws_bytes, void* stream);

int bg_rgbconv_supported(const BgConvDesc*);
int bg_rgbconv_fwd  (const BgConvDesc*, const float* x, const float* w, const float* bias, float* y,
                     int accumulate, void* stream);
int bg_rgbconv_dgrad(const BgConvDesc*, const float* dy, const float* w, float* dx, int accumulate, void* stream);
size_t bg_rgbconv_wgrad_workspace_bytes(const BgConvDesc*);
int bg_rgbconv_wgrad(const BgConvDesc*, const float* x, const float* dy, float* dw,
                     void* ws, size_t ws_bytes, void* stream);

typedef struct BgGemmDesc {
    int32_t M, N, K;
    int32_t transA, transB;
    int32_t lda, ldb, ldc;
    int32_t batch;
    int64_t strideA, strideB, strideC;
    int32_t compute;
    int32_t reserved;
} BgGemmDesc;
size_t bg_gemm_workspace_bytes(const BgGemmDesc*);
int bg_gemm(const BgGemmDesc*, const float* A, const float* B, const float* bias,
            const float* alpha_dev, float* C, int accumulate, void* ws, size_t ws_bytes, void* stream);

#define BG_DENSE_GROUP_MAX 8
typedef struct BgDenseItem {
    const float* x;
    int64_t ldx;
    const float* w;
    const float* bias;
    float* y;
    float* dw;
    float* db;
    int32_t K, N;
// ... 139 lines not shown

int bg_softmax_fwd(const float* s, float* p, int64_t rows, int cols, void* stream);
int bg_softmax_bwd(const float* p, const float* dp, float* ds, int64_t rows, int cols, void* stream);

int bg_sum_pool_fwd(const float* x, float* y, int N, int HW, int C, void* stream);
int bg_sum_pool_bwd(const float* dy, float* dx, int N, int HW, int C, void* stream);

int bg_axpby(const float* x, float a, float* y, float b, int64_t n, void* stream);
int bg_add(const float* a, const float* b, float* y, int64_t n, void* stream);
int bg_scale_add(const float* o, const float* gamma_dev, const float* x, float* y, int64_t n, void* stream);
int bg_dot(const float* a, const float* b, float* out_accum, int64_t n, void* stream);
int bg_scale_dev(const float* x, const float* s_dev, float* y, int64_t n, void* stream);
int bg_tanh_fwd(const float* x, float* y, int64_t n, void* stream);
int bg_tanh_bwd(const float* y, const float* dy, float* dx, int64_t n, void* stream);
int bg_bias_grad(const float* dy, float* db, int64_t rows, int C, void* stream);

int bg_alpha_head_fwd(const float* x, const float* w, float* y, int64_t rows, void* stream);
int bg_alpha_head_bwd(const float* x, const float* w, const float* dy, float* dx, float* dw_accum, int64_t rows,
                      void* stream);
int bg_alpha_mask_fwd(const float* x, float* y, int64_t rows, void* stream);
int bg_alpha_mask_bwd(const float* x, const float* dy, float* dx, int64_t rows, void* stream);
int bg_alpha_mask_tangent(const float* x, const float* xdot, float* ydot, int64_t rows, void* stream);

int bg_cast(const void* x, int x_dtype, void* y, int y_dtype, int64_t n, void* stream);
int bg_depth_to_space(const void* x, void* y, int dtype, int N, int H, int W, int C, int r, void* stream);
int bg_space_to_depth(const void* x, void* y, int dtype, int N, int H, int W, int C, int r, void* stream);
enum { BG_PAD_ZERO_FILL = 0, BG_PAD_SPLIT = 1, BG_PAD_DUP = 2, BG_PAD_FOLD = 3 };
int bg_pad_channels(const void* src, int src_dtype, void* dst, int dst_dtype, int64_t outer, int Cs, int Cd,
                    int64_t inner, int mode, void* stream);
int bg_weight_pack(const float* w, int taps, int rows_per_tap, int cols, void* pack_p, void* pack_t, void* stream);
int bg_bn_stats_t(const void* x, int x_dtype, double* sums, int64_t rows, int C, void* stream);
int bg_bn_apply_act_fwd_t(const void* x, int x_dtype, const float* mean, const float* rstd, const float* gamma,
                          const float* beta, int per_sample, const float* alpha, void* y, int y_dtype,
                          int N, int HW, int C, void* stream);
int bg_bn_apply_act_bwd_reduce_t(const void* x, int x_dtype, const void* dy, int y_dtype, const float* mean,
                                 const float* rstd, const float* gamma, const float* beta, int per_sample,
                                 const float* alpha, float* part, int N, int HW, int C, void* stream);
int bg_bn_apply_act_bwd_dx_t(const void* x, int x_dtype, const void* dy, int y_dtype, const float* mean,
                             const float* rstd, const float* gamma, const float* beta, int per_sample,
                             const float* alpha, const float* cm, void* dx, const void* dx_add, int N, int HW, int C,
                             void* stream);
int bg_prelu_fwd_t(const void* x, int x_dtype, const float* alpha, void* y, int y_dtype, int64_t rows, int C,
                   void* stream);
int bg_prelu_bwd_t(const void* x, int x_dtype, const void* dy, int y_dtype, const float* alpha, void* dx,
                   float* dalpha, const void* dx_add, int64_t rows, int C, void* stream);
int bg_bias_grad_t(const void* dy, int dtype, float* db, int64_t rows, int C, void* stream);
int bg_maxpool2_fwd_t(const void* x, void* y, int dtype, int N, int H, int W, int C, void* stream);
int bg_maxpool2_bwd_t(const void* x, const void* dy, void* dx, int dtype, int N, int H, int W, int C, void* stream);
int bg_sum_pool_fwd_t(const void* x, int x_dtype, float* y, int N, int HW, int C, void* stream);
int bg_sum_pool_bwd_t(const float* dy, void* dx, int x_dtype, int N, int HW, int C, void* stream);
int bg_lincomb_t(const void* a, const float* sa_dev, float sa, const void* b, float sb, void* y, int dtype,
                 int64_t n, void* stream);
int bg_dot_t(const void* a, const void* b, int dtype, float* out_accum, int64_t n, void* stream);

int bg_diffaugment_fwd(const float* x, float* y, const float* u_b, const float* u_s, const float* u_c,
                       const int32_t* t_x, const int32_t* t_y, const int32_t* o_x, const int32_t* o_y,
                       int N, int S, int C, int policy, double* mean_ws, void* stream);
int bg_diffaugment_bwd(const float* dy, float* dx, const float* u_s, const float* u_c,
                       const int32_t* t_x, const int32_t* t_y, const int32_t* o_x, const int32_t* o_y,
                       int N, int S, int C, int policy, double* mean_ws, void* stream);

int bg_hinge_d_sums(const float* real, const float* fake, float* sums, int n, void* stream);
int bg_hinge_d_grad(const float* real, const float* fake, const float* sums, double n_global, float flood,
                    float* d_real, float* d_fake, float* loss_out, int n, void* stream);
int bg_hinge_g_sums(const float* fake, float* sums, int n, void* stream);
int bg_hinge_g_grad(const float* sums, double n_global, float flood, float* d_fake, float* loss_out,
                    int n, void* stream);

int bg_gan_loss_means(const float* real, const float* fake, float* sums, int nr, int nf, void* stream);
int bg_gan_loss_terms(int kind, int generator, const float* real, const float* fake, const float* sums,
                      double n_real_global, double n_fake_global, float* tsums, int nr, int nf, void* stream);
int bg_gan_loss_grad(int kind, int generator, const float* real, const float* fake, const float* sums,
                     const float* tsums, double n_real_global, double n_fake_global, float flood, float* d_real,
                     float* d_fake, float* loss_out, int nr, int nf, void* stream);

int bg_gp_interpolate(const float* real, const float* other, const float* alpha, const double* sums, double count,
                      float* out, int N, int64_t per, void* stream);
int bg_gp_penalty(const float* g, int N, int64_t per, double count_global, float ld, int lp, double* ws, float* loss,
                  float* v, void* stream);
int bg_maxpool2_gather(const float* x, const float* t, float* y, int N, int H, int W, int C, void* stream);
int bg_prelu_tangent_dalpha(const float* x, const float* xdot, const float* dy, float* dalpha, int64_t rows, int C,
                            void* stream);
int bg_softmax_tangent_bwd(const float* p, const float* sdot, const float* g, float* dp, float* dsdot, int64_t rows,
                           int cols, void* stream);

int bg_sigmoid_ce(const float* logits, const float* truth, const float* weights, float scale, float* loss_out,
                  float* dlogits, int B, int n, void* stream);

int bg_label_loss_sums(const float* logits, const float* truth, const float* weights, const int32_t* slices,
                       const int32_t* col_slice, double* sums, int B, int n, int n_slices, void* stream);
int bg_label_loss_finish(const float* logits, const float* truth, const float* weights, const int32_t* slices,
                         const int32_t* col_slice, const double* sums, double rows_global, float loss_weight,
                         float* loss_out, float* dlogits, int B, int n, int n_slices, void* stream);
int bg_gather_rows(const float* table, const int64_t* idx, float* out, int rows, int n, int B, void* stream);

int bg_ortho_cosine_fwd_bwd(const float* A, float scale, float* loss_accum, float* dA, int c, void* stream);
int bg_symmetrize(const float* A, float* S, int c, void* stream);
int bg_ortho_identity_fwd_bwd(const float* A, float scale, float* loss_accum, float* dA, int c, void* stream);
int bg_gemv_rows(const float* w, const float* v, float* out, int rows, int cols, void* stream);
int bg_ortho_lowrank_cols(const float* W, const float* P, const float* s, float scale, float* alpha_beta,
                          float* Wb, float* loss_accum, int rows, int c, void* stream);
int bg_ortho_lowrank_finish(float* dW, const float* P, const float* s, const float* Walpha,
                            const float* alpha_beta, int rows, int c, void* stream);

int bg_adam_tf_ema_step(float* p, const float* g, float* m, float* v, float* ema,
                        float lr_t, float b1, float b2, float eps, float ema_decay, float grad_scale,
// ... 143 lines not shown
```

Baseline: 2858 images/sec.

## Fuse PReLU and attention scale-add post-ops into bf16 conv epilogue

Adds a post-op path to the bf16 implicit-GEMM conv epilogue, so the conv can write a PReLU/ReLU-activated output or a gamma*o + residual output directly. The model uses it for the first conv of resblocks and down-resblocks and for the attention output conv, which removes separate elementwise kernels and one activation round-trip through memory. It also adds a fused scale-and-dot backward kernel for ScaleAdd. The cost is extra epilogue work and register pressure in the conv kernel, plus a second output write when the pre-activation tensor is kept for backward.

Result: no change. 2854 images/sec (-0.1%).

```diff
diff --git a/biggan-tensorflow_amd/csrc/elementwise.hip b/biggan-tensorflow_amd/csrc/elementwise.hip
--- a/biggan-tensorflow_amd/csrc/elementwise.hip
+++ b/biggan-tensorflow_amd/csrc/elementwise.hip
@@ -1,6 +1,7 @@
 #include <stdlib.h>
 #include <mutex>
 #include "common.h"
+#include "postop.h"
 
 namespace bg {
 
@@ -432,7 +433,6 @@
     }
 }
 
-__device__ __forceinline__ float prelu_f(float v, float a) { return v > 0.f ? v : a * v; }
 __device__ __forceinline__ float prelu_d(float v, float a) { return v > 0.f ? 1.f : (v < 0.f ? a : 0.5f * a); }
 
 template <int VEC, class TX, class TY>
@@ -718,11 +718,9 @@
         bf16x8_load(a + i * 8, av);
         if (b) {
             bf16x8_load(b + i * 8, bv);
-#pragma unroll
-            for (int j = 0; j < 8; ++j) o[j] = s * av[j] + sb * bv[j];
+            lincomb8(s, av, sb, bv, o);
         } else {
-#pragma unroll
-            for (int j = 0; j < 8; ++j) o[j] = s * av[j];
+            scale_v<8>(s, av, o);
         }
         bf16x8_store(y + i * 8, o);
     }
@@ -1216,7 +1214,7 @@
         float av[4], bv[4];
         loadv<4>(a + i * 4, av);
         loadv<4>(b + i * 4, bv);
-        s += av[0] * bv[0] + av[1] * bv[1] + av[2] * bv[2] + av[3] * bv[3];
+        s += dot4(av, bv);
     }
     for (int64_t i = n4 * 4 + (int64_t)blockIdx.x * EW_BLOCK + threadIdx.x; i < n; i += (int64_t)gridDim.x * EW_BLOCK)
         s += (float)a[i] * (float)b[i];
@@ -1236,6 +1234,43 @@
     float* part = nullptr;
     if (!block_partials(grid, 1, s, &part)) return BG_ERR_LAUNCH;
     hipLaunchKernelGGL((dot_t_kernel<T>), dim3(grid), dim3(EW_BLOCK), 0, s, part, a, b, out, n);
+    finalize_block_partials(part, out, grid, 1, s);
+    BG_LAUNCH_CHECK();
+    return BG_OK;
+}
+
+template <class T>
+__global__ __launch_bounds__(EW_BLOCK) void scale_dot_t_kernel(float* part, const T* __restrict__ a, const T* __restrict__ b,
+                                                                const float* __restrict__ s_dev, T* __restrict__ y, float* out,
+                                                                int64_t n4) {
+    __shared__ float sh[4];
+    const float g = *s_dev;
+    float s = 0.f;
+    for (int64_t i = (int64_t)blockIdx.x * EW_BLOCK + threadIdx.x; i < n4; i += (int64_t)gridDim.x * EW_BLOCK) {
+        float av[4], bv[4], o[4];
+        loadv<4>(a + i * 4, av);
+        loadv<4>(b + i * 4, bv);
+        s += dot4(av, bv);
+        scale_v<4>(g, av, o);
+        storev<4>(y + i * 4, o);
+    }
+    s = block_sum_256(s, sh);
+    if (threadIdx.x == 0) {
+        if (part)
+            part[blockIdx.x] = s;
+        else
+            *out += s;
+    }
+}
+
+template <class T>
+static int launch_scale_dot(const T* a, const T* b, const float* s_dev, T* y, float* out, int64_t n, hipStream_t s) {
+    int grid = ew_grid(n / 4 + 1);
+    if (grid > 512) grid = 512;
+    float* part = nullptr;
+    if (!block_partials(grid, 1, s, &part)) return BG_ERR_LAUNCH;
+    hipLaunchKernelGGL((scale_dot_t_kernel<T>), dim3(grid), dim3(EW_BLOCK), 0, s, part, a, b, s_dev, y, out,
+                       n / 4);
     finalize_block_partials(part, out, grid, 1, s);
     BG_LAUNCH_CHECK();
     return BG_OK;
@@ -2545,6 +2580,15 @@
     return rc;
 }
 
+int bg_scale_dot_t(const void* dy, const void* o, const float* gamma, void* d_o, float* dot_accum, int64_t n, int dtype,
+                   void* stream) {
+    BG_REQUIRE(dy && o && gamma && d_o && dot_accum && n > 0 && n % 4 == 0 && BG_DT_OK(dtype),
+               "bg_scale_dot_t: bad argument (n %% 4 == 0)");
+    int rc = BG_OK;
+    BG_DISPATCH_T(dtype, rc = launch_scale_dot((const T*)dy, (const T*)o, gamma, (T*)d_o, dot_accum, n, as_stream(stream)));
+    return rc;
+}
+
 int bg_bn_stats(const float* x, double* sums, int64_t rows, int C, void* stream) {
     return bg_bn_stats_t(x, BG_F32, sums, rows, C, stream);
 }
diff --git a/biggan-tensorflow_amd/csrc/igemm.hip b/biggan-tensorflow_amd/csrc/igemm.hip
--- a/biggan-tensorflow_amd/csrc/igemm.hip
+++ b/biggan-tensorflow_amd/csrc/igemm.hip
@@ -1,4 +1,5 @@
 #include <stdlib.h>
+#include <optional>
 #include "common.h"
 #include "igemm.h"
 #include "igemm_dev.h"
@@ -1133,7 +1134,7 @@
 
 static int run_nn(ConvPlan& pl, const BgConvDesc* d, const char* op, bool deconv, const void* src, const void* w,
                   const float* bias, const float* alpha_dev, void* out, int accumulate, void* ws, size_t ws_bytes,
-                  void* stream) {
+                  void* stream, bool profiled = true) {
     hipStream_t s = as_stream(stream);
     Tag tag(op, d);
     void* const grid = ws;
@@ -1145,7 +1146,8 @@
         ws = ws_bytes > pl.grid_bytes ? reinterpret_cast<char*>(ws) + pl.grid_bytes : nullptr;
         ws_bytes -= pl.grid_bytes;
     }
-    ProfScope prof(s, conv_flops(d, deconv), tag.s, tag.bytes);
+    std::optional<ProfScope> prof;
+    if (profiled) prof.emplace(s, conv_flops(d, deconv), tag.s, tag.bytes);
     int rc;
     if (route_f32(pl.route)) {
         NNParams& p = pl.nn;
@@ -1217,6 +1219,42 @@
     return run_nn(pl, d, "conv2d_fwd", false, x, w, bias, alpha_dev, y, accumulate, ws, ws_bytes, stream);
 }
 
+static ConvPlan plan_conv_fwd_post(const BgConvDesc* d, int kind) {
+    ConvPlan pl = plan_conv_fwd(d);
+    if (pl.route == BF16_PLAIN) pl.nn16.post_kind = kind;
+    return pl;
+}
+
+int bg_conv2d_fwd_post_supported(const BgConvDesc* d, int kind) {
+    if (!d || (kind != BG_POST_PRELU && kind != BG_POST_SCALE_ADD) || check_conv(d) != BG_OK) return 0;
+    const ConvPlan pl = plan_conv_fwd_post(d, kind);
+    if (pl.route != BF16_PLAIN || !d->w_packed) return 0;
+    return nn16_post_ok(pl.nn16, pl.mode, pl.zdim) ? 1 : 0;
+}
+
+int bg_conv2d_fwd_post(const BgConvDesc* d, const void* x, const void* w, const float* bias, const float* alpha_dev,
+                       void* y, int accumulate, const BgConvPost* post, void* ws, size_t ws_bytes, void* stream) {
+    if (!post || post->kind == BG_POST_NONE)
+        return bg_conv2d_fwd(d, x, w, bias, alpha_dev, y, accumulate, ws, ws_bytes, stream);
+    int rc = check_conv(d);
+    if (rc) return rc;
+    BG_REQUIRE(x && w && y, "bg_conv2d_fwd_post: null tensor pointer");
+    BG_REQUIRE((post->kind == BG_POST_PRELU || post->kind == BG_POST_SCALE_ADD) && post->y2 && post->coef &&
+                   post->y2_ld >= d->Cout && post->y2_ld % 8 == 0 && post->y2_ld < (int64_t(1) << 31),
+               "bg_conv2d_fwd_post: bad post-op description");
+    ConvPlan pl = plan_conv_fwd_post(d, post->kind);
+    BG_REQUIRE(pl.route == BF16_PLAIN && d->w_packed && !accumulate && nn16_post_ok(pl.nn16, pl.mode, pl.zdim),
+               "bg_conv2d_fwd_post: this launch cannot carry a post-op (query bg_conv2d_fwd_post_supported)");
+    NN16Params& r = pl.nn16;
+    r.post_keep_out = post->keep_out != 0;
+    r.out2 = post->y2;
+    r.out2_ld = (int32_t)post->y2_ld;
+    r.post_coef = post->coef;
+    r.post_res = post->res;
+    (void)ws; (void)ws_bytes;
+    return run_nn(pl, d, "conv2d_fwd_post", false, x, w, bias, alpha_dev, y, 0, nullptr, 0, stream, false);
+}
+
 int bg_conv2d_fwd_d2s_supported(const BgConvDesc* d, int block) {
     if (!d) return 0;
     const ConvPlan pl = plan_conv_fwd(d, block);
diff --git a/biggan-tensorflow_amd/csrc/igemm16.h b/biggan-tensorflow_amd/csrc/igemm16.h
--- a/biggan-tensorflow_amd/csrc/igemm16.h
+++ b/biggan-tensorflow_amd/csrc/igemm16.h
@@ -31,7 +31,14 @@
     int32_t ring;
     int32_t ring_lines;
     int32_t d2s_c;
+    int32_t post_kind;
+    int32_t post_keep_out;
+    int32_t out2_ld;
+    void* out2;
+    const float* post_coef;
+    const void* post_res;
 };
+enum { NN16_POST_NONE = 0, NN16_POST_PRELU = 1, NN16_POST_SCALE_ADD = 2 };
 
 struct TN16Params {
     const void* A;
@@ -55,6 +62,7 @@
 int64_t nn16_stats_rows(const NN16Params& p, int mode, int zdim);
 int launch_nn16_ring(NN16Params& p, hipStream_t s);
 bool nn16_d2s_ok(const NN16Params& p, int mode, int zdim);
+bool nn16_post_ok(const NN16Params& p, int mode, int zdim);
 bool nn16h_d2s_ok(const NN16Params& p);
 int launch_nn16h_d2s(const NN16Params& plain, hipStream_t s);
 size_t tn16_workspace_bytes(const TN16Params& p);
diff --git a/biggan-tensorflow_amd/csrc/igemm16.hip b/biggan-tensorflow_amd/csrc/igemm16.hip
--- a/biggan-tensorflow_amd/csrc/igemm16.hip
+++ b/biggan-tensorflow_amd/csrc/igemm16.hip
@@ -5,6 +5,7 @@
 #include "igemm16.h"
 #include <type_traits>
 #include "igemm_dev.h"
+#include "postop.h"
 
 namespace bg {
 
@@ -41,6 +42,33 @@
 }
 __device__ __forceinline__ float bf16_lo(uint32_t u) { return __builtin_bit_cast(float, u << 16); }
 __device__ __forceinline__ float bf16_hi(uint32_t u) { return __builtin_bit_cast(float, u & 0xffff0000u); }
+
+__device__ __forceinline__ void nn16_post_store(const NN16Params& p, const uint4 rr, int64_t off2, int col) {
+    const float xv[8] = {bf16_lo(rr.x), bf16_hi(rr.x), bf16_lo(rr.y), bf16_hi(rr.y),
+                         bf16_lo(rr.z), bf16_hi(rr.z), bf16_lo(rr.w), bf16_hi(rr.w)};
+    float o[8];
+    if (p.post_kind == NN16_POST_PRELU) {
+        const f32x4_t a0 = *reinterpret_cast<const f32x4_t*>(p.post_coef + col);
+        const f32x4_t a1 = *reinterpret_cast<const f32x4_t*>(p.post_coef + col + 4);
+#pragma unroll
+        for (int j = 0; j < 4; ++j) {
+            o[j] = prelu_f(xv[j], a0[j]);
+            o[4 + j] = prelu_f(xv[4 + j], a1[j]);
+        }
+    } else {
+        const float s = *p.post_coef;
+        const uint4 xr = *reinterpret_cast<const uint4*>(reinterpret_cast<const __bf16*>(p.post_res) + off2);
+        const float bv[8] = {bf16_lo(xr.x), bf16_hi(xr.x), bf16_lo(xr.y), bf16_hi(xr.y),
+                             bf16_lo(xr.z), bf16_hi(xr.z), bf16_lo(xr.w), bf16_hi(xr.w)};
+        lincomb8(s, xv, 1.0f, bv, o);
+    }
+    uint4 r2;
+    r2.x = pack_bf16x2(o[0], o[1]);
+    r2.y = pack_bf16x2(o[2], o[3]);
+    r2.z = pack_bf16x2(o[4], o[5]);
+    r2.w = pack_bf16x2(o[6], o[7]);
+    *reinterpret_cast<uint4*>(reinterpret_cast<__bf16*>(p.out2) + off2) = r2;
+}
 
 constexpr int NN16_BM = 128;
 constexpr int NN16_TAPS = 4;
@@ -610,9 +638,11 @@
         const int m = m0 + row, col = n0 + cc * 8;
         if (m >= p.M || col >= p.N) continue;
         int64_t ooff;
+        int64_t orow = m;
         if (use_tabo) {
             const unsigned op = tabo[row];
             if (op == 0xffffffffu) continue;
+            orow = op;
             ooff = (int64_t)op * p.out_ld + col;
         } else if (p.d2s_c) {
             int b, ho, wo;
@@ -665,7 +695,8 @@
             r.y = pack_bf16x2(v0[2], v0[3]);
             r.z = pack_bf16x2(v1[0], v1[1]);
             r.w = pack_bf16x2(v1[2], v1[3]);
-            *reinterpret_cast<uint4*>(o) = r;
+            if (p.post_kind == NN16_POST_NONE || p.post_keep_out) *reinterpret_cast<uint4*>(o) = r;
+            if (p.post_kind != NN16_POST_NONE) nn16_post_store(p, r, orow * p.out2_ld + col, col);
         }
     }
     }
@@ -805,7 +836,9 @@
                     rr.y = pack_bf16x2(v0[2], v0[3]);
                     rr.z = pack_bf16x2(v1[0], v1[1]);
                     rr.w = pack_bf16x2(v1[2], v1[3]);
-                    *reinterpret_cast<uint4*>(o) = rr;
+                    if (THIN || p.post_kind == NN16_POST_NONE || p.post_keep_out) *reinterpret_cast<uint4*>(o) = rr;
+                    if (THIN == 0 && p.post_kind != NN16_POST_NONE)
+                        nn16_post_store(p, rr, ((int64_t)(b * g.Ho + oy) * g.Wo + ox) * p.out2_ld + col, col);
                     if (p.stats_part) {
                         v0[0] = bf16_lo(rr.x); v0[1] = bf16_hi(rr.x); v0[2] = bf16_lo(rr.y); v0[3] = bf16_hi(rr.y);
                         v1[0] = bf16_lo(rr.z); v1[1] = bf16_hi(rr.z); v1[2] = bf16_lo(rr.w); v1[3] = bf16_hi(rr.w);
@@ -1996,6 +2029,16 @@
     return plan_nn16(p, mode, zdim, true).splitk == 1;
 }
 
+bool nn16_post_ok(const NN16Params& p, int mode, int zdim) {
+    const Gather& g = p.g;
+    if (p.post_kind != NN16_POST_PRELU && p.post_kind != NN16_POST_SCALE_ADD) return false;
+    if (p.out_f32 || p.d2s_c || p.ring || p.stats_part || p.C % 8 || p.N % 8 || mode != GATHER_CONV || zdim != 1 ||
+        g.pstep != 1 || g.Hq != g.Ho || g.Wq != g.Wo)
+        return false;
+    if (nn16h_taps(p, mode, zdim)) return true;
+    return plan_nn16(p, mode, zdim, true).splitk == 1;
+}
+
 int64_t nn16_stats_rows(const NN16Params& p, int mode, int zdim) {
     if (p.C % 8 || p.N % 8 || !nn16h_taps(p, mode, zdim)) return 0;
     return 2 * (int64_t)p.g.Nb * (p.g.Hq / NH_T) * (p.g.Wq / NH_T) * (p.g.pstep * p.g.pstep);
@@ -2013,6 +2056,16 @@
                "bf16-resident conv: more than 2^30 source / 2^31 output pixels");
     BG_REQUIRE(p.d2s_c == 0 || (nn16_d2s_ok(p, mode, zdim) && ws == nullptr),
                "bf16-resident conv: this launch has no depth-to-space store (bg_conv2d_fwd_d2s_supported)");
+    if (p.post_kind != NN16_POST_NONE) {
+        BG_REQUIRE(nn16_post_ok(p, mode, zdim) && ws == nullptr && !p.accumulate,
+                   "bf16-resident conv: this launch cannot carry a post-op (bg_conv2d_fwd_post_supported)");
+        BG_REQUIRE(p.out2 && p.post_coef && p.out2_ld % 8 == 0 && p.out2_ld >= p.N &&
+                       (reinterpret_cast<uintptr_t>(p.out2) & 15) == 0 &&
+                       (reinterpret_cast<uintptr_t>(p.post_coef) & (p.post_kind == NN16_POST_PRELU ? 15 : 3)) == 0,
+                   "bf16-resident conv post-op: out2 / coef missing or not 16-byte aligned");
+        BG_REQUIRE(p.post_kind != NN16_POST_SCALE_ADD || (p.post_res && (reinterpret_cast<uintptr_t>(p.post_res) & 15) == 0),
+                   "bf16-resident conv post-op: SCALE_ADD needs the 16-byte aligned residual");
+    }
     if (const int ntaps = nn16h_taps(p, mode, zdim)) return launch_nn16h(p, mode, ntaps, s);
     BG_REQUIRE(p.stats_part == nullptr, "bf16-resident conv: fused statistics need the halo-tile form (nn16_stats_rows)");
     NN16Plan pl = plan_nn16(p, mode, zdim, ws != nullptr);
diff --git a/biggan-tensorflow_amd/csrc/postop.h b/biggan-tensorflow_amd/csrc/postop.h
--- /dev/null
+++ b/biggan-tensorflow_amd/csrc/postop.h
@@ -0,0 +1,37 @@
+#pragma once
+#include <hip/hip_runtime.h>
+
+namespace bg {
+
+__device__ __forceinline__ float prelu_f(float v, float a) { return v > 0.f ? v : a * v; }
+
+__device__ __forceinline__ void lincomb8(float s, const float (&a)[8], float sb, const float (&b)[8], float (&o)[8]) {
+#pragma clang fp contract(off)
+#pragma unroll
+    for (int j = 0; j < 6; ++j) {
+        const float t = sb * b[j];
+        o[j] = __builtin_fmaf(s, a[j], t);
+    }
+#pragma unroll
+    for (int j = 6; j < 8; ++j) {
+        const float u = s * a[j], t = sb * b[j];
+        o[j] = u + t;
+    }
+}
+
+template <int VEC>
+__device__ __forceinline__ void scale_v(float s, const float (&a)[VEC], float (&o)[VEC]) {
+#pragma unroll
+    for (int j = 0; j < VEC; ++j) o[j] = s * a[j];
+}
+
+__device__ __forceinline__ float dot4(const float (&a)[4], const float (&b)[4]) {
+#pragma clang fp contract(off)
+    const float p0 = a[0] * b[0], p1 = a[1] * b[1], p2 = a[2] * b[2], p3 = a[3] * b[3];
+    float t = p0 + p1;
+    t = t + p2;
+    t = p3 + t;
+    return t;
+}
+
+}
diff --git a/biggan-tensorflow_amd/functional.py b/biggan-tensorflow_amd/functional.py
--- a/biggan-tensorflow_amd/functional.py
+++ b/biggan-tensorflow_amd/functional.py
@@ -1,3 +1,4 @@
+import ctypes
 import math
 import os
 
@@ -622,10 +623,41 @@
     return None
 
 
+def fuse_post():
+    return os.environ.get("BG_FUSE_POST", "1") != "0"
+
+
+def _conv_post(L, d, x, pt, bias, post):
+    shape = (d.N, d.Ho, d.Wo, d.Cout)
+    y2 = torch.empty(shape, dtype=BF16, device=x.device)
+    if post[0] == "prelu":
+        kind, coef, res, keep = hip.POST_PRELU, post[1], None, True
+    else:
+        kind, coef, res, keep = hip.POST_SCALE_ADD, post[1], _c(post[2]), bool(post[3])
+        assert res.dtype == BF16 and tuple(res.shape) == shape, (res.dtype, res.shape, shape)
+    if fuse_post() and L.bg_conv2d_fwd_post_supported(d, kind):
+        y = torch.empty(shape, dtype=BF16, device=x.device) if keep else None
+        desc = hip.BgConvPost(kind, int(keep), y2.data_ptr(), d.Cout, f32(coef).value,
+                              act(res).value if res is not None else None)
+        check(L.bg_conv2d_fwd_post(d, act(x), act(pt), f32(bias), None, act(y if keep else y2), 0, ctypes.byref(desc), None,
+                                   0, stream()))
+        if y is None:
+            y = torch.empty(1, dtype=BF16, device=x.device).expand(shape)
+        return y, y2
+    y = torch.empty(shape, dtype=BF16, device=x.device)
+    ws, nb = hip.scratch(L.bg_conv2d_fwd_workspace_bytes, d, x.device)
+    check(L.bg_conv2d_fwd(d, act(x), act(pt), f32(bias), None, act(y), 0, f32(ws), nb, stream()))
+    if kind == hip.POST_PRELU:
+        check(L.bg_prelu_fwd_t(act(y), dt(y), f32(coef), act(y2), dt(y2), y.numel() // d.Cout, d.Cout, stream()))
+    else:
+        check(L.bg_lincomb_t(act(y), f32(coef), 0.0, act(res), 1.0, act(y2), dt(y), y.numel(), stream()))
+    return y, y2
+
+
 class Conv2dFn(Function):
 
     @staticmethod
-    def forward(ctx, x, w, bias, stride, pad_lo, Ho, Wo, pad_mode, out_dtype=None, accumulate_into=None):
+    def forward(ctx, x, w, bias, stride, pad_lo, Ho, Wo, pad_mode, out_dtype=None, accumulate_into=None, post=None):
         ctx.fork = getattr(x, "bg_fork", None)
         x = _c(x)
         N, H, W_, Cin = x.shape
@@ -636,6 +668,7 @@
         ctx.in_dtype = x.dtype
         ctx.pad8 = None if ctx.resident or k > 4 else _thin_plan(x, Cin, Cout)
         ctx.acc = accumulate_into is not None
+        assert post is None or (ctx.resident and not ctx.acc and out_dtype is None), "post-op: bf16-resident layers only"
         if ctx.acc:
             assert ctx.pad8 is None and tuple(accumulate_into.shape) == (N, Ho, Wo, Cout), "accumulate_into: shape"
         if ctx.pad8 == "in":
@@ -668,6 +701,13 @@
             ydt = out_dtype or BF16
             d = hip.conv_desc(N, H, W_, Cin, Ho, Wo, Cout, k, stride, pad_lo, pad_mode, hip.COMPUTE_BF16, hip.BF16,
                               hip.BF16 if ydt == BF16 else hip.F32, 1)
+            if post is not None:
+                y, y2 = _conv_post(L, d, x, weight_packs(w)[1], bias, post)
+                ctx.mark_non_differentiable(y2)
+                ctx.set_materialize_grads(False)
+                ctx.desc, ctx.rgb = d, False
+                ctx.x, ctx.w, ctx.bias = x, w, bias
+                return y, y2
             if ctx.acc:
                 y = accumulate_into
                 assert y.dtype == ydt and y.is_contiguous(), (y.dtype, ydt)
@@ -699,7 +739,7 @@
         return y
 
     @staticmethod
-    def backward(ctx, dy):
+    def backward(ctx, dy, _dy2=None):
         dy = _c(dy)
         d, x, w, bias = ctx.desc, ctx.x, ctx.w, ctx.bias
         L = lib()
@@ -740,7 +780,7 @@
                                             hip.PAD_FOLD, stream()))
             dw = param_grad(w, ctx.needs_input_grad[1], wg8)
             ctx.x = ctx.w = ctx.bias = None
-            return dx, dw, db, None, None, None, None, None, None, None
+            return dx, dw, db, None, None, None, None, None, None, None, None
         if bias is not None:
             db = param_grad(bias, ctx.needs_input_grad[2], lambda out: _bias_grad(dy.view(-1, d.Cout), out))
         if ctx.resident:
@@ -760,7 +800,7 @@
                 check(L.bg_conv2d_wgrad(db16, act(x), act(dyb), f32(out), f32(ws), nb, stream()))
             dw = param_grad(w, ctx.needs_input_grad[1], wg16)
             ctx.x = ctx.w = ctx.bias = None
-            return dx, dw, db, None, None, None, None, None, None, (dy if ctx.acc else None)
+            return dx, dw, db, None, None, None, None, None, None, (dy if ctx.acc else None), None
         if ctx.needs_input_grad[0]:
             dx = torch.empty_like(x)
             if ctx.rgb:
@@ -782,7 +822,7 @@
         ctx.x = ctx.w = ctx.bias = None
         if dx is not None:
             dx = cast(dx, ctx.in_dtype)
-        return dx, dw, db, None, None, None, None, None, None, (dy if ctx.acc else None)
+        return dx, dw, db, None, None, None, None, None, None, (dy if ctx.acc else None), None
 
 
 def _shuffle_ok(t, C):
@@ -1694,14 +1734,15 @@
 class PReluFn(Function):
 
     @staticmethod
-    def forward(ctx, x, alpha):
+    def forward(ctx, x, alpha, y=None):
         ctx.fork = getattr(x, "bg_fork", None)
         x = _c(x)
         C = x.shape[-1]
         if KinkProbe.sites is not None:
             KinkProbe.sites.append((getattr(alpha, "bg_name", None), "act", x.detach().float().clone()))
-        y = torch.empty_like(x)
-        check(lib().bg_prelu_fwd_t(act(x), dt(x), f32(alpha), act(y), dt(y), x.numel() // C, C, stream()))
+        if y is None:
+            y = torch.empty_like(x)
+            check(lib().bg_prelu_fwd_t(act(x), dt(x), f32(alpha), act(y), dt(y), x.numel() // C, C, stream()))
         ctx.x, ctx.alpha = x, alpha
         return y
 
@@ -1725,7 +1766,7 @@
             check(L.bg_prelu_bwd_t(act(x), dt(x), act(dy), dt(dy), f32(alpha), None, f32(out), None, rows, C, stream()))
         da = param_grad(alpha, ctx.needs_input_grad[1], prod)
         ctx.x = None
-        return dx, da
+        return dx, da, None
 
 
 class MaxPool2Fn(Function):
@@ -2150,8 +2191,12 @@
 class ScaleAddFn(Function):
 
     @staticmethod
-    def forward(ctx, o, gamma, x):
+    def forward(ctx, o, gamma, x, y=None):
         ctx.fork = getattr(x, "bg_fork", None)
+        if y is not None:
+            ctx.o_dtype = o.dtype
+            ctx.o, ctx.gamma = o, gamma
+            return y
         o, x = _c(o), _c(x)
         ctx.o_dtype = o.dtype
         if o.dtype != x.dtype:
@@ -2169,27 +2214,31 @@
         dy = _c(dy)
         o, gamma = ctx.o, ctx.gamma
         L = lib()
-        do = None
-        if ctx.needs_input_grad[0]:
-            do = torch.empty_like(o)
+        do = torch.empty_like(dy) if ctx.needs_input_grad[0] else None
+        one_pass = do is not None and fuse_post() and dy.numel() % 4 == 0 and o.dtype == dy.dtype and o.is_contiguous()
+        do_written = [False]
+
+        def prod(out):
+            out.zero_()
+            if one_pass:
+                check(L.bg_scale_dot_t(act(dy), act(o), f32(gamma), act(do), f32(out), dy.numel(), dt(dy), stream()))
+                do_written[0] = True
+            elif dy.numel() % 4:
+                check(L.bg_dot(f32(dy), f32(o), f32(out), dy.numel(), stream()))
+            else:
+                check(L.bg_dot_t(act(dy), act(o), dt(dy), f32(out), dy.numel(), stream()))
+        dg = param_grad(gamma, ctx.needs_input_grad[1], prod)
+        if do is not None and not do_written[0]:
             if dy.dtype == torch.float32:
                 check(L.bg_scale_dev(f32(dy), f32(gamma), f32(do), dy.numel(), stream()))
             else:
                 check(L.bg_lincomb_t(act(dy), f32(gamma), 0.0, None, 0.0, act(do), dt(dy), dy.numel(), stream()))
-
-        def prod(out):
-            out.zero_()
-            if dy.numel() % 4:
-                check(L.bg_dot(f32(dy), f32(o), f32(out), dy.numel(), stream()))
-            else:
-                check(L.bg_dot_t(act(dy), act(o), dt(dy), f32(out), dy.numel(), stream()))
-        dg = param_grad(gamma, ctx.needs_input_grad[1], prod)
         ctx.o = None
         if do is not None:
             do = cast(do, ctx.o_dtype)
         if ctx.needs_input_grad[2] and dy.dtype == ctx.o_dtype:
             _fork_done(ctx.fork, dy)
-        return do, dg, dy
+        return do, dg, dy, None
 
 
 class BnTangentFn(Function):
diff --git a/biggan-tensorflow_amd/hip.py b/biggan-tensorflow_amd/hip.py
--- a/biggan-tensorflow_amd/hip.py
+++ b/biggan-tensorflow_amd/hip.py
@@ -55,6 +55,14 @@
 
 LATENT_MAX_TARGETS = 8
 LATENT_MAX_SEGS = 48
+
+
+POST_NONE, POST_PRELU, POST_SCALE_ADD = 0, 1, 2
+
+
+class BgConvPost(Structure):
+    _fields_ = [("kind", c_int32), ("keep_out", c_int32), ("y2", c_void_p), ("y2_ld", c_int64), ("coef", c_void_p),
+                ("res", c_void_p)]
 
 
 class BgMixBranch(Structure):
@@ -101,6 +109,8 @@
     "bg_conv2d_fwd": (c_int, [_CD, _P, _P, _P, _P, _P, c_int, _P, c_size_t, _P]),
     "bg_conv2d_fwd_d2s_supported": (c_int, [_CD, c_int]),
     "bg_conv2d_fwd_d2s": (c_int, [_CD, _P, _P, _P, _P, _P, c_int, _P, c_size_t, _P]),
+    "bg_conv2d_fwd_post_supported": (c_int, [_CD, c_int]),
+    "bg_conv2d_fwd_post": (c_int, [_CD, _P, _P, _P, _P, _P, c_int, _P, _P, c_size_t, _P]),
     "bg_conv2d_dgrad_workspace_bytes": (c_size_t, [_CD]),
     "bg_conv2d_dgrad": (c_int, [_CD, _P, _P, _P, _P, c_int, _P, c_size_t, _P]),
     "bg_conv2d_wgrad_workspace_bytes": (c_size_t, [_CD]),
@@ -230,6 +240,7 @@
     "bg_sum_pool_bwd_t": (c_int, [_P, _P, c_int, c_int, c_int, c_int, _P]),
     "bg_lincomb_t": (c_int, [_P, _P, c_float, _P, c_float, _P, c_int, c_int64, _P]),
     "bg_dot_t": (c_int, [_P, _P, c_int, _P, c_int64, _P]),
+    "bg_scale_dot_t": (c_int, [_P, _P, _P, _P, _P, c_int64, c_int, _P]),
     "bg_bn_glu_fwd": (c_int, [_P, _P, _P, _P, _P, _P, c_int, c_int64, c_int, _P]),
     "bg_bn_glu_bwd_reduce": (c_int, [_P, _P, _P, _P, _P, _P, _P, c_int, c_int64, c_int, c_int, _P]),
     "bg_bn_glu_bwd_dx": (c_int, [_P, _P, _P, _P, _P, _P, _P, _P, c_int, c_int64, c_int, _P]),
diff --git a/biggan-tensorflow_amd/ops.py b/biggan-tensorflow_amd/ops.py
--- a/biggan-tensorflow_amd/ops.py
+++ b/biggan-tensorflow_amd/ops.py
@@ -161,18 +161,26 @@
     return y
 
 
+def _apply_post(y, post):
+    if post is None:
+        return y
+    if post[0] == "prelu":
+        return _prelu_apply(y, post[1])
+    return Fn.ScaleAddFn.apply(y, post[1], post[2])
+
+
 def conv(x, channels, opt, kernel=4, stride=2, pad=0, dilation=1, use_bias=True, scope='conv_0', _out_dtype=None,
-         _accumulate_into=None):
+         _accumulate_into=None, _post=None):
     with variable_scope(scope) as full_scope:
         if isinstance(kernel, str):
             slices = decode_kernel_sizes(kernel)["slices"]
             branches = [_MixBranch('conv' + str(sl["kernel"]) + "_slice", False, sl["size"], sl["kernel"],
                                    (sl["kernel"] - 1) // 2, dilation) for sl in slices]
             y = _mixconv(x, branches, opt, stride, use_bias)
-            return _mix_epilogue(y, _out_dtype, _accumulate_into)
+            return _apply_post(_mix_epilogue(y, _out_dtype, _accumulate_into), _post)
         if dilation != 1:
             y = _mixconv(x, [_MixBranch(None, False, channels, kernel, pad, dilation)], opt, stride, use_bias)
-            return _mix_epilogue(y, _out_dtype, _accumulate_into)
+            return _apply_post(_mix_epilogue(y, _out_dtype, _accumulate_into), _post)
         N, H, W, Cin = x.shape
         pad_mode = hip.PAD_REFLECT
         pad_lo = pad_hi = 0
@@ -215,6 +223,19 @@
             y = Dual(Fn.Conv2dFn.apply(x.p, wk, bias, stride, pad_lo, Ho, Wo, pad_mode),
                      Fn.Conv2dFn.apply(x.t, wk, None, stride, pad_lo, Ho, Wo, pad_mode))
             return y if _accumulate_into is None else _add(y, _accumulate_into)
+        if _post is not None:
+            assert _accumulate_into is None and _out_dtype is None, "_post: not with _accumulate_into / _out_dtype"
+            if not (Fn.fuse_post() and Fn._resident_ok(x, Cin, channels, kernel)):
+                y = Fn.Conv2dFn.apply(x, wk, bias, stride, pad_lo, Ho, Wo, pad_mode)
+                return _apply_post(_resident_out(y), _post)
+            if _post[0] == "prelu":
+                y, y2 = Fn.Conv2dFn.apply(x, wk, bias, stride, pad_lo, Ho, Wo, pad_mode, None, None, _post)
+                return Fn.PReluFn.apply(y, _post[1], y2)
+            gamma, x_res = _post[1], _post[2]
+            keep = torch.is_grad_enabled() and not Fn._Mode.inputs_only and bool(gamma.requires_grad)
+            y, y2 = Fn.Conv2dFn.apply(x, wk, bias, stride, pad_lo, Ho, Wo, pad_mode, None, None,
+                                      ("scale_add", gamma, x_res, keep))
+            return Fn.ScaleAddFn.apply(y, gamma, x_res, y2)
         acc = _accumulate_into
         if acc is not None and os.environ.get("BG_FUSE_RESIDUAL", "1") == "0":
             y = Fn.Conv2dFn.apply(x, wk, bias, stride, pad_lo, Ho, Wo, pad_mode, _out_dtype)
@@ -319,14 +340,28 @@
     return outs
 
 
+def _res1_post(x, channels, opt, act_scope):
+    if (_is_meta(x) or _is_dual(x) or opt["bn_in_d"] or not Fn.fuse_post() or not S.default_store().frozen
+            or x.dtype != torch.bfloat16):
+        return None
+    if opt["act"] is relu:
+        return ("prelu", _constant_alpha(channels, 0.0, x.device))
+    if opt["act"] is prelu:
+        with variable_scope(act_scope), variable_scope(None, default_name="prelu"):
+            return ("prelu", get_variable('alpha', channels, initializer=S.constant_initializer(0.0)))
+    return None
+
+
 def resblock(x_init, channels, opt, use_bias=True, scope='resblock'):
     with variable_scope(scope):
         x_main, x_skip = _fork(x_init)
+        post = _res1_post(x_main, channels, opt, 'res1')
         with variable_scope('res1'):
-            x = conv(x_main, channels, kernel=3, stride=1, pad=1, use_bias=use_bias, opt=opt)
+            x = conv(x_main, channels, kernel=3, stride=1, pad=1, use_bias=use_bias, opt=opt, _post=post)
             if opt["bn_in_d"]:
                 x = bn(x, opt=opt)
-            x = opt["act"](x)
+            if post is None:
+                x = opt["act"](x)
         with variable_scope('res2'):
             x = conv(x, channels, kernel=3, stride=1, pad=1, use_bias=use_bias, opt=opt)
             if opt["bn_in_d"]:
@@ -449,11 +484,12 @@
     return x
 
 
-def downconv(x, channels, opt, use_bias=True, method=None):
+def downconv(x, channels, opt, use_bias=True, method=None, _post=None):
     if method is None:
         method = opt["downsampling_method"]
+    assert _post is None or method == 'strided_conv3'
     if method == 'strided_conv3':
-        return conv(x, channels, kernel=3, stride=2, pad=1, use_bias=use_bias, opt=opt)
+        return conv(x, channels, kernel=3, stride=2, pad=1, use_bias=use_bias, opt=opt, _post=_post)
     elif method == 'resize_conv1':
         x = conv(x, channels, kernel=1, stride=1, pad=0, use_bias=use_bias, opt=opt)
         return avg_pooling(x)
@@ -487,20 +523,22 @@
 def resblock_down(x_init, channels, opt, use_bias=True, scope='resblock_down'):
     with variable_scope(scope):
         x_main, x_init = _fork(x_init)
+        res_method = opt["downsampling_method"]
+        if res_method != 'strided_conv3':
+            res_method = 'resize_conv3'
+        post = _res1_post(x_main, channels, opt, 'res2') if res_method == 'strided_conv3' else None
         with variable_scope('res1'):
             if opt["bn_in_d"]:
                 x = bn(x_main, opt=opt)
             else:
                 x = x_main
             x = opt["act"](x)
-            res_method = opt["downsampling_method"]
-            if res_method != 'strided_conv3':
-                res_method = 'resize_conv3'
-            x = downconv(x, channels, use_bias=use_bias, opt=opt, method=res_method)
+            x = downconv(x, channels, use_bias=use_bias, opt=opt, method=res_method, _post=post)
         with variable_scope('res2'):
             if opt["bn_in_d"]:
                 x = bn(x, opt=opt)
-            x = opt["act"](x)
+            if post is None:
+                x = opt["act"](x)
         with variable_scope('skip'):
             x_init = downconv(x_init, channels, use_bias=use_bias, opt=opt, method=opt["downsampling_method"])
         with variable_scope('res2'):
@@ -721,8 +759,8 @@
                 x_qkv, x_res = _fork(x, 2)
                 gamma = get_variable("gamma", [1], initializer=S.constant_initializer(0.0))
                 o = Fn.SaFrontFn.apply(x_qkv, wf, wg, wh, b_f, b_g, b_h)
-                o = conv(o, channels, kernel=1, stride=1, opt=opt, scope='attn_conv', use_bias=use_bias)
-                return Fn.ScaleAddFn.apply(o, gamma, x_res)
+                return conv(o, channels, kernel=1, stride=1, opt=opt, scope='attn_conv', use_bias=use_bias,
+                            _post=("scale_add", gamma, x_res))
         x_f, x_g, x_h, x = _fork(x, 4)
         f32o = None if _is_meta(x) or _is_dual(x) or x.dtype == torch.float32 else torch.float32
         f = conv(x_f, channels // 8, kernel=1, stride=1, opt=opt, scope='f_conv', use_bias=use_bias, _out_dtype=f32o)
diff --git a/include/biggan_hip.h b/include/biggan_hip.h
--- a/include/biggan_hip.h
+++ b/include/biggan_hip.h
@@ -53,6 +53,18 @@
 int bg_conv2d_fwd_d2s_supported(const BgConvDesc*, int block);
 int bg_conv2d_fwd_d2s(const BgConvDesc*, const void* x, const void* w, const float* bias, const float* alpha_dev,
                       void* y, int block, void* ws, size_t ws_bytes, void* stream);
+enum { BG_POST_NONE = 0, BG_POST_PRELU = 1, BG_POST_SCALE_ADD = 2 };
+typedef struct BgConvPost {
+    int32_t      kind;
+    int32_t      keep_out;
+    void*        y2;
+    int64_t      y2_ld;
+    const float* coef;
+    const void*  res;
+} BgConvPost;
+int bg_conv2d_fwd_post_supported(const BgConvDesc*, int kind);
+int bg_conv2d_fwd_post(const BgConvDesc*, const void* x, const void* w, const float* bias, const float* alpha_dev,
+                       void* y, int accumulate, const BgConvPost* post, void* ws, size_t ws_bytes, void* stream);
 size_t bg_conv2d_dgrad_workspace_bytes(const BgConvDesc*);
 int bg_conv2d_dgrad(const BgConvDesc*, const void* dy, const void* w, const float* alpha_dev,
                     void* dx, int accumulate, void* ws, size_t ws_bytes, void* stream);
@@ -298,6 +310,8 @@
 int bg_lincomb_t(const void* a, const float* sa_dev, float sa, const void* b, float sb, void* y, int dtype,
                  int64_t n, void* stream);
 int bg_dot_t(const void* a, const void* b, int dtype, float* out_accum, int64_t n, void* stream);
+int bg_scale_dot_t(const void* dy, const void* o, const float* gamma, void* d_o, float* dot_accum, int64_t n, int dtype,
+                   void* stream);
 
 int bg_diffaugment_fwd(const float* x, float* y, const float* u_b, const float* u_s, const float* u_c,
                        const int32_t* t_x, const int32_t* t_y, const int32_t* o_x, const int32_t* o_y,
```
